# XunshanMan/Object-oriented-SLAM

Measured on AMD Instinct MI355X. Metric: LM iterations/sec (cams+ellipsoids), higher is better.
Workload: dtype f64

## Files before the change

### include/esl.h

```cpp
#ifndef ESL_H_
#define ESL_H_

#include <stdint.h>

#ifdef __cplusplus
extern "C" {
#endif

#define ESL_ABI_VERSION 5
#define ESL_MAX_TRACE 32

typedef enum {
  ESL_OK = 0,
  ESL_ERR_NO_DEVICE = 1,
  ESL_ERR_INVALID = 2,
  ESL_ERR_HIP = 3,
  ESL_ERR_STATE = 4,
  ESL_ERR_ALLOC = 5
} esl_status;

typedef struct esl_ctx esl_ctx;

typedef struct {
  double fx, fy, cx, cy;
  int32_t n_cams;
  int32_t n_objs;
  const uint8_t* cam_fixed;

  int32_t n_bbox;
  const int32_t* bbox_cam;
  const int32_t* bbox_obj;
  const double* bbox_meas;
  const double* bbox_weight;

  int32_t n_e3d;
  const int32_t* e3d_cam;
  const int32_t* e3d_obj;
  const double* e3d_meas;
  const double* e3d_weight;

  int32_t n_grav;
  const int32_t* grav_obj;
  double grav_normal[4];
  double grav_weight;

  int32_t n_odom;
  const int32_t* odom_i;
  const int32_t* odom_j;
  const double* odom_meas;
  const double* odom_info;

  int32_t check_visibility;
  int32_t image_rows, image_cols;
} esl_graph;

typedef enum {
  ESL_JAC_NUMERIC = 0,
  ESL_JAC_ANALYTIC = 1
} esl_jacobian_mode;

typedef enum {
  ESL_SOLVER_AUTO = 0,
  ESL_SOLVER_REDUCED_CAMERA = 1,
  ESL_SOLVER_REDUCED_ELLIPSOID = 2,
  ESL_SOLVER_CAMERA_CHAIN = 3,
  ESL_SOLVER_PCG = 4
} esl_linear_solver;

typedef enum {
  ESL_BBOX_REPROJECTION = 0,
  ESL_BBOX_TANGENCY = 1
} esl_bbox_residual;

typedef struct {
  int32_t max_iters;
  int32_t max_trials;
  double tau;
  int32_t jacobian_mode;
  double numeric_delta;
  int32_t linear_solver;
  int32_t drop_nan_bbox;
  int32_t bbox_residual;
  int32_t e3d_half_turn;
} esl_lm_params;

typedef struct {
  int32_t iterations;
  int32_t total_trials;
  int32_t n_bbox_valid;
  int32_t n_bbox_dropped;
  int32_t stop_reason;
  double chi2_initial;
  double chi2_final;
  double lambda_final;
  int32_t trace_len;
  double trace_chi2[ESL_MAX_TRACE];
  double trace_lambda[ESL_MAX_TRACE];
  int32_t trace_trials[ESL_MAX_TRACE];
} esl_lm_report;

typedef struct {
  double chi2;
  double max_diag;
  double scale;
  int32_t solve_ok;
  int32_t pad;
} esl_lm_partials;

int esl_abi_version(void);
const char* esl_last_error(void);
int esl_device_count(void);
int esl_ctx_create(int device_id, esl_ctx** out);
int esl_ctx_destroy(esl_ctx* ctx);
int esl_ctx_synchronize(esl_ctx* ctx);
int esl_ctx_trim(esl_ctx* ctx);
void esl_lm_params_default(esl_lm_params* p);

typedef enum { ESL_ROBUST_NONE = 0, ESL_ROBUST_HUBER = 1, ESL_ROBUST_PSEUDO_HUBER = 2, ESL_ROBUST_CAUCHY = 3, ESL_ROBUST_TUKEY = 4 } esl_robust_kind;
typedef enum { ESL_EDGE_BBOX = 0, ESL_EDGE_E3D = 1, ESL_EDGE_GRAVITY = 2, ESL_EDGE_ODOM = 3, ESL_EDGE_CLASSES = 4 } esl_edge_class;
typedef struct {
  int32_t kind[ESL_EDGE_CLASSES];
  double delta[ESL_EDGE_CLASSES];
} esl_robust_params;
int esl_lm_set_robust(esl_ctx* ctx, const esl_robust_params* p);
typedef struct {
  int32_t max_iters;
  int32_t check_every;
  double rel_tol;
} esl_pcg_params;
void esl_pcg_params_default(esl_pcg_params* p);
int esl_lm_set_pcg(esl_ctx* ctx, const esl_pcg_params* p);
#define ESL_PCG_STATS 8
int esl_lm_pcg_stats(esl_ctx* ctx, double stats[ESL_PCG_STATS]);

int esl_edge_chi2(esl_ctx* ctx, int32_t edge_class, double* chi2, double* weight, int64_t count);

int esl_optimize(esl_ctx* ctx, const esl_graph* g, double* cams_io ,
                 double* objs_io , const esl_lm_params* p, esl_lm_report* out);

int esl_graph_upload(esl_ctx* ctx, const esl_graph* g);
int esl_graph_upload_fixed(esl_ctx* ctx, const esl_graph* g, const uint8_t* obj_fixed);
int esl_optimize_fixed(esl_ctx* ctx, const esl_graph* g, const uint8_t* obj_fixed, double* cams_io, double* objs_io,
                       const esl_lm_params* p, esl_lm_report* out);
int esl_graph_obj_fixed(esl_ctx* ctx, uint8_t* flags_out, int32_t count);
int esl_states_upload(esl_ctx* ctx, const double* cams, const double* objs);
int esl_states_download(esl_ctx* ctx, double* cams, double* objs);
int esl_optimize_resident(esl_ctx* ctx, const esl_lm_params* p, esl_lm_report* out);
int esl_states_snapshot(esl_ctx* ctx);
int esl_states_restore(esl_ctx* ctx);

typedef struct {
  int32_t n_new_cams; const double* new_cams;
  int32_t n_new_objs; const double* new_objs;
  int32_t n_bbox; const int32_t* bbox_cam; const int32_t* bbox_obj; const double* bbox_meas; const double* bbox_weight;
  int32_t n_e3d; const int32_t* e3d_cam; const int32_t* e3d_obj; const double* e3d_meas; const double* e3d_weight;
  int32_t n_grav; const int32_t* grav_obj;
  const uint8_t* new_cam_fixed;
  int32_t n_odom; const int32_t* odom_i; const int32_t* odom_j;
  const double* odom_meas;
  const double* odom_info;
} esl_graph_delta;
int esl_graph_append(esl_ctx* ctx, const esl_graph_delta* d);
int esl_graph_sizes(esl_ctx* ctx, int32_t* n_cams, int32_t* n_objs, int32_t* n_bbox, int32_t* n_e3d, int32_t* relayouts);

#define ESL_PROF_KINDS 10
int esl_profile_enable(esl_ctx* ctx, int enable);
int esl_profile_get(esl_ctx* ctx, int64_t count[ESL_PROF_KINDS], double total_ms[ESL_PROF_KINDS]);

int esl_lm_begin(esl_ctx* ctx, const esl_lm_params* p, int32_t* n_valid, int32_t* n_dropped);
int esl_lm_linearize(esl_ctx* ctx, esl_lm_partials* out);
int esl_lm_reduced_system(esl_ctx* ctx, double lambda, void** dev_ptr, int64_t* n, int64_t* lda);
int esl_lm_reduced_residual(esl_ctx* ctx, double* rel_residual_out);
int esl_lm_try_step(esl_ctx* ctx, double lambda, esl_lm_partials* out);
int esl_lm_commit(esl_ctx* ctx, int accept);
int esl_lm_solver_used(esl_ctx* ctx, int32_t* solver_out);
#define ESL_SOLVER_STATS 10
int esl_lm_solver_stats(esl_ctx* ctx, double stats[ESL_SOLVER_STATS]);

int esl_lm_download(esl_ctx* ctx, int32_t which, double* dst, int64_t count);

int esl_comm_unique_id(char out[128]);
int esl_comm_init(esl_ctx* ctx, int32_t n_ranks, int32_t rank, const char id[128]);
typedef int (*esl_host_allreduce_fn)(void* user, double* host_buf, int64_t count);
int esl_comm_init_host(esl_ctx* ctx, int32_t n_ranks, int32_t rank, esl_host_allreduce_fn fn, void* user);
int esl_comm_set_replicated(esl_ctx* ctx, int replicated);
int esl_comm_destroy(esl_ctx* ctx);

int esl_partition_objects(const esl_graph* g, int32_t n_parts, int32_t* part_of_obj);

typedef struct {
  int32_t stride;
  double depth_scale;
  double depth_min, depth_max;
  double voxel_leaf;
  double plane_dist;
  double cluster_tolerance;
  int32_t min_cluster_size;
  double center_dis;
  int32_t symmetry_open;
  double symmetry_grid;
  double symmetry_sigma;
  int32_t symmetry_lm_iters;
} esl_fit_params;

void esl_fit_params_default(esl_fit_params* p);

int esl_fit_frame(esl_ctx* ctx, const uint16_t* depth, int32_t width, int32_t height,
                  const double* bboxes , const int32_t* labels , int32_t n_boxes,
                  const double Twc[7], const double intr[5] ,
                  const double ground[4], const esl_fit_params* p,
                  double* ellipsoids_out , double* prob_out ,
                  int32_t* status_out );

int esl_fit_frame_debug(esl_ctx* ctx, const uint16_t* depth, int32_t width, int32_t height, const double* bboxes,
                        const int32_t* labels, int32_t n_boxes, const double Twc[7], const double intr[5],
                        const double ground[4], const esl_fit_params* p, double* ellipsoids_out, double* prob_out,
                        int32_t* status_out, double* debug_out);

typedef struct {
  int32_t result;
  int32_t symmetry_type;
  double plane[4];
  double plane2[4];
  double prob;
  double center[3];
} esl_fit_symmetry;

int esl_fit_frame_ex(esl_ctx* ctx, const uint16_t* depth, int32_t width, int32_t height, const double* bboxes,
                     const int32_t* labels, int32_t n_boxes, const double Twc[7], const double intr[5],
                     const double ground[4], const esl_fit_params* p, double* ellipsoids_out, double* prob_out,
                     int32_t* status_out, esl_fit_symmetry* symmetry_out, double* debug_out);

typedef struct esl_plane_params {
  int32_t min_size;
  double angle_threshold_deg;
  double distance_threshold;
  int32_t normal_smoothing;
  double max_depth_change_factor;
  int32_t min_inliers;
  int32_t refine;
  double refine_distance;
  double max_curvature;
} esl_plane_params;
void esl_plane_params_default(esl_plane_params* p);
int esl_extract_ground_plane(esl_ctx* ctx, const uint16_t* depth, int32_t width, int32_t height, const double intr[5],
                             const esl_plane_params* p, double plane_out[4], int32_t* ok, int32_t* n_planes, int32_t* n_pixels);

int esl_extract_planes(esl_ctx* ctx, const uint16_t* depth, int32_t width, int32_t height, const double intr[5],
                       const esl_plane_params* p, int32_t max_planes, double* planes_out, int32_t* sizes_out,
                       int32_t* n_planes, int32_t* labels_out);

int esl_init_quadric(esl_ctx* ctx, const double* poses_Twc , const double* bboxes ,
                     int32_t n, const double K[4], int32_t rows, int32_t cols, int32_t faithful,
                     double ellipsoid_out[10], double qstar_out[16], int32_t* ok);

int esl_init_from_qstar(esl_ctx* ctx, const double qstar[16], int32_t faithful, double ellipsoid_out[10], int32_t* ok);
int esl_init_plane_error(esl_ctx* ctx, const double* poses_Twc , const double* bboxes , int32_t n,
                         const double K[4], int32_t rows, int32_t cols, const double ellipsoid[10], double* error_out);

int esl_init_quadrics(esl_ctx* ctx,
                      const double* cams , int32_t F,
                      int32_t N ,
                      const int32_t* obs_cam , const int32_t* obs_obj ,
                      const double* obs_boxes , int64_t n_obs,
                      const double K[4], int32_t rows, int32_t cols, int32_t faithful, int32_t min_observations,
                      double* ellipsoids_out , double* qstar_out ,
                      double* plane_error_out , int32_t* stats_out );

typedef struct {
  int32_t sample_size;
  int32_t n_hypotheses;
  double  inlier_px;
  int32_t min_inliers;
  int32_t refine;
  uint64_t seed;
} esl_init_robust_params;
void esl_init_robust_params_default(esl_init_robust_params* p);

int esl_init_quadrics_robust(esl_ctx* ctx, const double* cams , int32_t F, int32_t N,
                             const int32_t* obs_cam, const int32_t* obs_obj, const double* obs_boxes, int64_t n_obs,
                             const double K[4], int32_t rows, int32_t cols, int32_t faithful, int32_t min_observations,
                             const esl_init_robust_params* p ,
                             double* ellipsoids_out , double* qstar_out , double* plane_error_out ,
                             int32_t* stats_out , int32_t* inlier_out , double* residual_out ,
                             double* hyp_out );

typedef struct {
  double center_tol;
  double height_tol;
  double size_ratio;
  double min_baseline;
  int32_t min_inliers;
  int32_t max_candidates;
  int32_t match_labels;
  int32_t refine;
} esl_reloc_params;
void esl_reloc_params_default(esl_reloc_params* p);

int esl_reloc_set_map(esl_ctx* ctx, const double* objs, const int32_t* labels, int32_t M, const double ground_world[4]);

typedef struct {
  int32_t status;
  int32_t n_candidates;
  int64_t n_hypotheses;
  int64_t best_key;
  int32_t n_inliers;
  int32_t refined;
  double cost;
  double yaw, tx, ty;
  double Twc[7];
} esl_reloc_result;

int esl_relocalize(esl_ctx* ctx, const double* det_objs , const int32_t* det_labels, int32_t D,
                   const double ground_cam[4], const esl_reloc_params* p ,
                   esl_reloc_result* out, int32_t* assoc_out );

typedef struct {
  double min_iou;
  double occl_ratio;
  double min_box_px;
  int32_t match_labels;
  int32_t occlusion;
} esl_assoc_params;
void esl_assoc_params_default(esl_assoc_params* p);

int esl_predict_boxes(esl_ctx* ctx, const double Tcw[7], const double* objs ,
                      int32_t M, const double K[4], int32_t rows, int32_t cols, const esl_assoc_params* p ,
                      double* boxes_out , double* depth_out , int32_t* flags_out );

int esl_associate_boxes(esl_ctx* ctx, const double* cams , int32_t F,
// ... 104 lines not shown
```

### object-oriented-slam_amd/abi.py

```python
import ctypes as C

import numpy as np

ESL_MAX_TRACE = 32

c_double_p = C.POINTER(C.c_double)
c_int32_p = C.POINTER(C.c_int32)
c_uint8_p = C.POINTER(C.c_uint8)


class EslGraph(C.Structure):
    _fields_ = [
        ("fx", C.c_double), ("fy", C.c_double), ("cx", C.c_double), ("cy", C.c_double),
        ("n_cams", C.c_int32), ("n_objs", C.c_int32),
        ("cam_fixed", c_uint8_p),
        ("n_bbox", C.c_int32), ("bbox_cam", c_int32_p), ("bbox_obj", c_int32_p),
        ("bbox_meas", c_double_p), ("bbox_weight", c_double_p),
        ("n_e3d", C.c_int32), ("e3d_cam", c_int32_p), ("e3d_obj", c_int32_p),
        ("e3d_meas", c_double_p), ("e3d_weight", c_double_p),
        ("n_grav", C.c_int32), ("grav_obj", c_int32_p),
        ("grav_normal", C.c_double * 4), ("grav_weight", C.c_double),
        ("n_odom", C.c_int32), ("odom_i", c_int32_p), ("odom_j", c_int32_p),
        ("odom_meas", c_double_p), ("odom_info", c_double_p),
        ("check_visibility", C.c_int32), ("image_rows", C.c_int32), ("image_cols", C.c_int32),
    ]


class EslGraphDelta(C.Structure):
    _fields_ = [
        ("n_new_cams", C.c_int32), ("new_cams", c_double_p), ("n_new_objs", C.c_int32), ("new_objs", c_double_p),
        ("n_bbox", C.c_int32), ("bbox_cam", c_int32_p), ("bbox_obj", c_int32_p), ("bbox_meas", c_double_p), ("bbox_weight", c_double_p),
        ("n_e3d", C.c_int32), ("e3d_cam", c_int32_p), ("e3d_obj", c_int32_p), ("e3d_meas", c_double_p), ("e3d_weight", c_double_p),
        ("n_grav", C.c_int32), ("grav_obj", c_int32_p),
        ("new_cam_fixed", C.POINTER(C.c_uint8)), ("n_odom", C.c_int32), ("odom_i", c_int32_p), ("odom_j", c_int32_p),
        ("odom_meas", c_double_p), ("odom_info", c_double_p),
    ]


class EslLmParams(C.Structure):
    _fields_ = [
        ("max_iters", C.c_int32), ("max_trials", C.c_int32), ("tau", C.c_double),
        ("jacobian_mode", C.c_int32), ("numeric_delta", C.c_double),
        ("linear_solver", C.c_int32), ("drop_nan_bbox", C.c_int32), ("bbox_residual", C.c_int32), ("e3d_half_turn", C.c_int32),
    ]


class EslLmReport(C.Structure):
    _fields_ = [
        ("iterations", C.c_int32), ("total_trials", C.c_int32),
        ("n_bbox_valid", C.c_int32), ("n_bbox_dropped", C.c_int32), ("stop_reason", C.c_int32),
        ("chi2_initial", C.c_double), ("chi2_final", C.c_double), ("lambda_final", C.c_double),
        ("trace_len", C.c_int32),
        ("trace_chi2", C.c_double * ESL_MAX_TRACE), ("trace_lambda", C.c_double * ESL_MAX_TRACE),
        ("trace_trials", C.c_int32 * ESL_MAX_TRACE),
    ]

    def as_dict(self):
        n = self.trace_len
        return dict(iterations=self.iterations, total_trials=self.total_trials,
                    n_bbox_valid=self.n_bbox_valid, n_bbox_dropped=self.n_bbox_dropped,
                    stop_reason=self.stop_reason, chi2_initial=self.chi2_initial,
                    chi2_final=self.chi2_final, lambda_final=self.lambda_final,
                    trace_chi2=list(self.trace_chi2[:n]), trace_lambda=list(self.trace_lambda[:n]),
                    trace_trials=list(self.trace_trials[:n]))


class EslLmPartials(C.Structure):
    _fields_ = [("chi2", C.c_double), ("max_diag", C.c_double), ("scale", C.c_double),
                ("solve_ok", C.c_int32), ("pad", C.c_int32)]


class EslFitParams(C.Structure):
    _fields_ = [
        ("stride", C.c_int32), ("depth_scale", C.c_double), ("depth_min", C.c_double),
        ("depth_max", C.c_double), ("voxel_leaf", C.c_double), ("plane_dist", C.c_double),
        ("cluster_tolerance", C.c_double), ("min_cluster_size", C.c_int32), ("center_dis", C.c_double),
        ("symmetry_open", C.c_int32), ("symmetry_grid", C.c_double), ("symmetry_sigma", C.c_double),
        ("symmetry_lm_iters", C.c_int32),
    ]


class EslFitSymmetry(C.Structure):
    _fields_ = [("result", C.c_int32), ("symmetry_type", C.c_int32), ("plane", C.c_double * 4),
                ("plane2", C.c_double * 4), ("prob", C.c_double), ("center", C.c_double * 3)]


class EslPlaneParams(C.Structure):
    _fields_ = [("min_size", C.c_int32), ("angle_threshold_deg", C.c_double), ("distance_threshold", C.c_double),
                ("normal_smoothing", C.c_int32), ("max_depth_change_factor", C.c_double), ("min_inliers", C.c_int32),
                ("refine", C.c_int32), ("refine_distance", C.c_double), ("max_curvature", C.c_double)]


def default_plane_params(**kw):
    p = EslPlaneParams(min_size=200, angle_threshold_deg=5.0, distance_threshold=0.1, normal_smoothing=10,
                       max_depth_change_factor=0.05, min_inliers=100, refine=1, refine_distance=0.02, max_curvature=0.001)
    for k, v in kw.items():
        if not hasattr(p, k):
            raise AttributeError(k)
        setattr(p, k, v)
    return p


SOLVER_AUTO, SOLVER_REDUCED_CAMERA, SOLVER_REDUCED_ELLIPSOID, SOLVER_CAMERA_CHAIN, SOLVER_PCG = 0, 1, 2, 3, 4


class EslPcgParams(C.Structure):
    _fields_ = [("max_iters", C.c_int32), ("check_every", C.c_int32), ("rel_tol", C.c_double)]


def default_pcg_params():
    return EslPcgParams(max_iters=1000, check_every=8, rel_tol=1e-10)


class EslRelocParams(C.Structure):
    _fields_ = [("center_tol", C.c_double), ("height_tol", C.c_double), ("size_ratio", C.c_double), ("min_baseline", C.c_double),
                ("min_inliers", C.c_int32), ("max_candidates", C.c_int32), ("match_labels", C.c_int32), ("refine", C.c_int32)]


class EslRelocResult(C.Structure):
    _fields_ = [("status", C.c_int32), ("n_candidates", C.c_int32), ("n_hypotheses", C.c_int64), ("best_key", C.c_int64),
                ("n_inliers", C.c_int32), ("refined", C.c_int32), ("cost", C.c_double), ("yaw", C.c_double), ("tx", C.c_double),
                ("ty", C.c_double), ("Twc", C.c_double * 7)]

    def as_dict(self):
        return dict(status=self.status, n_candidates=self.n_candidates, n_hypotheses=self.n_hypotheses, best_key=self.best_key,
                    n_inliers=self.n_inliers, refined=self.refined, cost=self.cost, yaw=self.yaw, tx=self.tx, ty=self.ty,
                    Twc=np.array(list(self.Twc)))


def default_reloc_params(**kw):
    p = EslRelocParams(center_tol=0.25, height_tol=0.25, size_ratio=1.5, min_baseline=0.5, min_inliers=3, max_candidates=4096,
                       match_labels=1, refine=1)
    for k, v in kw.items():
        if not hasattr(p, k):
            raise AttributeError(k)
        setattr(p, k, v)
    return p


class EslAssocParams(C.Structure):
    _fields_ = [("min_iou", C.c_double), ("occl_ratio", C.c_double), ("min_box_px", C.c_double), ("match_labels", C.c_int32),
                ("occlusion", C.c_int32)]


def default_assoc_params(**kw):
    p = EslAssocParams(min_iou=0.3, occl_ratio=0.7, min_box_px=10.0, match_labels=1, occlusion=1)
    for k, v in kw.items():
        if not hasattr(p, k):
            raise AttributeError(k)
        setattr(p, k, v)
    return p


class EslInitRobustParams(C.Structure):
    _fields_ = [("sample_size", C.c_int32), ("n_hypotheses", C.c_int32), ("inlier_px", C.c_double), ("min_inliers", C.c_int32),
                ("refine", C.c_int32), ("seed", C.c_uint64)]

# ... 222 lines not shown
```

### object-oriented-slam_amd/csrc/esl_capi.hip

```cpp
#include <algorithm>
#include <cfloat>
#include <cmath>
#include <cstdio>
#include <cstdlib>
#include <cstring>
#include <numeric>

#include "esl_graph_int.hpp"
#include "esl_graph_layout.hpp"
#include "esl_kernels_map.hpp"
#include "esl_kernels_chunk.hpp"
#include "esl_slam.hpp"
#include "esl_fixed.hpp"

namespace esl {
static thread_local std::string g_err;
void set_error(const std::string& s) { g_err = s; }
}

using namespace esl;

namespace esl {
ProfScope::ProfScope(esl_ctx* ctx, int kind) : c(ctx), slot(-1) {
  if (!c || !c->prof_on) return;
  if (c->prof_level < 2 && (kind != 0 || !c->prof_gate)) return;
  if (c->prof_used + 2 > c->prof_ev.size()) {
    if (c->prof_ev.size() >= 16384) { prof_drain(c); }
    else {
      for (int i = 0; i < 512; ++i) { hipEvent_t e; if (hipEventCreate(&e) != hipSuccess) return; c->prof_ev.push_back(e); }
      c->prof_kind.resize(c->prof_ev.size() / 2);
    }
  }
  slot = (int)c->prof_used;
  c->prof_kind[slot / 2] = kind;
  c->prof_used += 2;
  (void)hipEventRecord(c->prof_ev[slot], c->stream);
}
ProfScope::~ProfScope() {
  if (slot >= 0) (void)hipEventRecord(c->prof_ev[slot + 1], c->stream);
}
int prof_drain(esl_ctx* c) {
  if (hipStreamSynchronize(c->stream) != hipSuccess) return ESL_ERR_HIP;
  for (size_t s = 0; s + 1 < c->prof_used; s += 2) {
    float ms = 0;
    if (hipEventElapsedTime(&ms, c->prof_ev[s], c->prof_ev[s + 1]) == hipSuccess) {
      const int k = c->prof_kind[s / 2];
      c->prof_count[k]++;
      c->prof_ms[k] += ms;
    }
  }
  c->prof_used = 0;
  return ESL_OK;
}
}

struct WorkStage {
  struct Fix { void** dst; size_t off; };
  size_t total = 0;
  std::vector<Fix> fixes;
  template <class T>
  void add(T** dst, size_t n) {
    const size_t off = layout::align_up(total, 256);
    total = off + std::max<size_t>(n, 1) * sizeof(T);
    fixes.push_back({(void**)dst, off});
  }
  int commit(esl_ctx* c) {
    int rc = arena_reserve(&c->arena_work, &c->arena_work_cap, std::max<size_t>(total, 256));
    if (rc) return rc;
    for (const Fix& f : fixes) *f.dst = c->arena_work + f.off;
    return ESL_OK;
  }
};
int esl::work_buffers(esl_ctx* c, size_t cap_objs, size_t cap_cams, size_t cap_chunks) {
  WorkStage wk;
  wk.add(&c->chunk_out, cap_chunks * kChunkOut); wk.add(&c->chunk_out2, cap_chunks * kChunkOut);
  wk.add(&c->chunk_chi, cap_chunks);
  wk.add(&c->blk_part, ((cap_objs + kStepWaves - 1) / kStepWaves + 2) * 2);
  wk.add(&c->solve_part, ((cap_objs + kStepWaves - 1) / kStepWaves + (cap_objs + 63) / 64 + 2) * 4 * 2);
  wk.add(&c->blk_chi, cap_chunks + 2);
  wk.add(&c->cams, cap_cams * 7); wk.add(&c->cams_trial, cap_cams * 7);
  wk.add(&c->objs, cap_objs * 10); wk.add(&c->objs_trial, cap_objs * 10);
  wk.add(&c->Hoo, cap_objs * 45); wk.add(&c->bo, cap_objs * 9); wk.add(&c->xo, cap_objs * 9); wk.add(&c->obj_part, cap_objs * 4);
  int rc = wk.commit(c);
  if (rc) return rc;
  ESL_HIP_TRY(hipMemsetAsync(c->obj_part, 0, std::max<size_t>(cap_objs, 1) * 4 * sizeof(double), c->stream));
  return ESL_OK;
}

extern "C" {

int esl_abi_version(void) { return ESL_ABI_VERSION; }
const char* esl_last_error(void) { return g_err.c_str(); }

int esl_device_count(void) {
  int n = 0;
  if (hipGetDeviceCount(&n) != hipSuccess) return 0;
  return n;
}

void esl_lm_params_default(esl_lm_params* p) {
  p->max_iters = 10;
  p->max_trials = 10;
  p->tau = 1e-5;
  p->jacobian_mode = ESL_JAC_NUMERIC;
  p->numeric_delta = 1e-9;
  p->linear_solver = ESL_SOLVER_AUTO;
  p->drop_nan_bbox = 1;
  p->bbox_residual = ESL_BBOX_REPROJECTION;
  p->e3d_half_turn = 0;
}

int esl_ctx_create(int device_id, esl_ctx** out) {
  if (!out) return ESL_ERR_INVALID;
  *out = nullptr;
  int n = 0;
  if (hipGetDeviceCount(&n) != hipSuccess || n <= 0) {
    set_error("no HIP device visible: libesl_hip has no CPU fallback");
    return ESL_ERR_NO_DEVICE;
  }
  if (device_id < 0 || device_id >= n) { set_error("device id out of range"); return ESL_ERR_INVALID; }
  ESL_HIP_TRY(hipSetDevice(device_id));
  esl_ctx* c = new esl_ctx();
  c->device = device_id;
  { const char* ov = std::getenv("ESL_CF_OVERLAP"); c->sw_cf_overlap = (ov && ov[0] >= '0' && ov[0] <= '4') ? ov[0] - '0' : 4; }
  { const char* ok = std::getenv("ESL_CF_OS_KERNEL"); c->sw_cf_os_kernel = (ok && ok[0] == '0') ? 0 : 1; }
  { const char* sd = std::getenv("ESL_CF_STRIDE"); const int v = sd ? std::atoi(sd) : 0; c->sw_cf_stride = (v == 16 || v == 32 || v == 48) ? v : 0; }
  auto init = [&]() -> int {
    ESL_HIP_TRY(hipStreamCreateWithFlags(&c->stream, hipStreamNonBlocking));
    ESL_HIP_TRY(hipHostMalloc((void**)&c->host_part, 16 * sizeof(double), hipHostMallocDefault));
    ESL_HIP_TRY(hipMalloc((void**)&c->dev_part, 16 * sizeof(double)));
    ESL_HIP_TRY(hipMalloc((void**)&c->chol_info, 4 * sizeof(int)));
    ESL_HIP_TRY(hipMemset(c->chol_info, 0, 4 * sizeof(int)));
    ESL_HIP_TRY(hipMalloc((void**)&c->tickets, 4 * sizeof(unsigned int)));
    ESL_HIP_TRY(hipMemset(c->tickets, 0, 4 * sizeof(unsigned int)));
    ESL_HIP_TRY(hipMalloc((void**)&c->dev_scal, 8 * sizeof(double)));
    ESL_HIP_TRY(hipEventCreateWithFlags(&c->ev_try, hipEventDisableTiming));
    ESL_HIP_TRY(hipHostMalloc(&c->host_scal, sizeof(LmScalars), hipHostMallocMapped));
    ESL_HIP_TRY(hipHostGetDevicePointer(&c->host_scal_dev, c->host_scal, 0));
    std::memset(c->host_scal, 0, sizeof(LmScalars));
    ESL_HIP_TRY(hipMalloc(&c->lm_dev, 2 * sizeof(LmCore)));
    ESL_HIP_TRY(hipMemset(c->lm_dev, 0, 2 * sizeof(LmCore)));
    ESL_HIP_TRY(hipHostMalloc(&c->lm_host, sizeof(LmHostView), hipHostMallocMapped));
    ESL_HIP_TRY(hipHostGetDevicePointer(&c->lm_host_dev, c->lm_host, 0));
    std::memset(c->lm_host, 0, sizeof(LmHostView));
    return ESL_OK;
  };
  const int rc = init();
  if (rc) { const std::string msg = g_err; esl_ctx_destroy(c); set_error(msg); return rc; }
  *out = c;
  return ESL_OK;
}

int esl_ctx_destroy(esl_ctx* c) {
  if (!c) return ESL_OK;
  (void)hipSetDevice(c->device);
  if (c->stream) (void)hipStreamSynchronize(c->stream);
  slam_sync_side(c);
  free_graph(c);
  slam_release(c);
  if (c->arena_graph) (void)hipFree(c->arena_graph);
  if (c->arena_work) (void)hipFree(c->arena_work);
  if (c->stage_host) (void)hipHostFree(c->stage_host);
  if (c->append_dev) (void)hipFree(c->append_dev);
  if (c->slam_tab_dev) (void)hipFree(c->slam_tab_dev);
  c->eq_buf.release();
  if (c->fx_blob) (void)hipFree(c->fx_blob);
  c->chain_ws.release();
  fit_release(c);
  plane_release(c);
  reloc_release(c);
  assoc_release(c);
  merge_release(c);
  render_release(c);
  dense_release(c);
  init_batch_release(c);
  for (hipEvent_t e : c->prof_ev) (void)hipEventDestroy(e);
  if (c->host_part) (void)hipHostFree(c->host_part);
  dev_free(&c->dev_part);
  dev_free(&c->chol_info);
  dev_free(&c->tickets); dev_free(&c->dev_scal);
  if (c->host_scal) (void)hipHostFree(c->host_scal);
  if (c->lm_host) (void)hipHostFree(c->lm_host);
  if (c->lm_dev) (void)hipFree(c->lm_dev);
  if (c->ev_try) (void)hipEventDestroy(c->ev_try);
  esl_comm_destroy(c);
  slam_release_runtime(c);
  if (c->stream) (void)hipStreamDestroy(c->stream);
  delete c;
  return ESL_OK;
}

int esl_ctx_trim(esl_ctx* c) {
  if (!c) return ESL_ERR_INVALID;
  ESL_HIP_TRY(hipSetDevice(c->device));
  ESL_HIP_TRY(hipStreamSynchronize(c->stream));
  slam_trim(c, c->graph_loaded && c->g.n_free_cams > 0);
  return ESL_OK;
}

int esl_debug_scratch_allocs(esl_ctx* c, int32_t owner, int64_t* allocs_out, int64_t* bytes_out) {
  if (!c || !allocs_out || !bytes_out || owner < ESL_SCRATCH_RELOC || owner > ESL_SCRATCH_INIT_ROBUST) {
    set_error("esl_debug_scratch_allocs: null pointer or unknown owner");
    return ESL_ERR_INVALID;
  }
  *allocs_out = 0; *bytes_out = 0;
  switch (owner) {
    case ESL_SCRATCH_RELOC: reloc_scratch_stats(c, allocs_out, bytes_out); break;
    case ESL_SCRATCH_ASSOC: assoc_scratch_stats(c, allocs_out, bytes_out); break;
    case ESL_SCRATCH_MERGE: merge_scratch_stats(c, allocs_out, bytes_out); break;
    case ESL_SCRATCH_RENDER: render_scratch_stats(c, allocs_out, bytes_out); break;
    default: init_scratch_stats(c, owner == ESL_SCRATCH_INIT_ROBUST, allocs_out, bytes_out);
  }
  return ESL_OK;
}

int esl_ctx_synchronize(esl_ctx* c) {
  if (!c) return ESL_ERR_INVALID;
  ESL_HIP_TRY(hipStreamSynchronize(c->stream));
  return ESL_OK;
}

static ChunkTable chunk_table(const esl_ctx* c) {
  ChunkTable t;
  t.n_chunks = c->n_chunks; t.obj = c->ck_obj; t.type = c->ck_type; t.begin = c->ck_begin; t.end = c->ck_end; t.ostart = c->ck_ostart;
  return t;
}
static int map_launch_linearize(esl_ctx* c, bool finalize, const double* src_objs = nullptr, double* dst_chunk = nullptr,
                                const LmCore* st = nullptr, bool validate = false) {
  const DevGraph& g = c->g;
  if (!src_objs) src_objs = c->objs;
  if (!dst_chunk) dst_chunk = c->chunk_out;
  const double* objs_b = st ? c->objs_trial : nullptr;
  double* chunk_b = st ? c->chunk_out2 : nullptr;
  if (st) { src_objs = c->objs; dst_chunk = c->chunk_out; }
  const ChunkTable ct = chunk_table(c);
  const bool an = c->lm.p.jacobian_mode == ESL_JAC_ANALYTIC;
  const int nb_e3 = (c->n_ids_e3 + 2 * kLinWaves - 1) / (2 * kLinWaves);
  const int nb_bb = (c->n_ids_bb + kLinWaves - 1) / kLinWaves;
  robust_dispatch(c->robust_on, [&](auto robust) {
    constexpr bool R = decltype(robust)::value;
    if (ct.n_chunks > 0) {
      ProfScope ps(c, 0);
      const dim3 block(64 * kLinWaves);
      int* cnt = c->chol_info + 2;
      if (an && g.bbox_mode) {
        if (validate && g.check_vis)
          hipLaunchKernelGGL((k_chunk_linearize_both<ESL_JAC_ANALYTIC, 2, true, R>), dim3(nb_e3 + nb_bb), block, 0, c->stream, g, ct, c->ck_ids_e3,
                             c->n_ids_e3, nb_e3, c->ck_ids_bb, c->n_ids_bb, c->cams, src_objs, objs_b, c->lm.p.numeric_delta, dst_chunk,
                             chunk_b, c->blk_chi, st, cnt);
        else if (validate)
          hipLaunchKernelGGL((k_chunk_linearize_both<ESL_JAC_ANALYTIC, 1, true, R>), dim3(nb_e3 + nb_bb), block, 0, c->stream, g, ct, c->ck_ids_e3,
                             c->n_ids_e3, nb_e3, c->ck_ids_bb, c->n_ids_bb, c->cams, src_objs, objs_b, c->lm.p.numeric_delta, dst_chunk,
                             chunk_b, c->blk_chi, st, cnt);
        else
          hipLaunchKernelGGL((k_chunk_linearize_both<ESL_JAC_ANALYTIC, 0, true, R>), dim3(nb_e3 + nb_bb), block, 0, c->stream, g, ct, c->ck_ids_e3,
                             c->n_ids_e3, nb_e3, c->ck_ids_bb, c->n_ids_bb, c->cams, src_objs, objs_b, c->lm.p.numeric_delta, dst_chunk,
                             chunk_b, c->blk_chi, st, cnt);
      } else if (an) {
        if (validate && g.check_vis)
          hipLaunchKernelGGL((k_chunk_linearize_both<ESL_JAC_ANALYTIC, 2, false, R>), dim3(nb_e3 + nb_bb), block, 0, c->stream, g, ct, c->ck_ids_e3,
                             c->n_ids_e3, nb_e3, c->ck_ids_bb, c->n_ids_bb, c->cams, src_objs, objs_b, c->lm.p.numeric_delta, dst_chunk,
                             chunk_b, c->blk_chi, st, cnt);
        else if (validate)
          hipLaunchKernelGGL((k_chunk_linearize_both<ESL_JAC_ANALYTIC, 1, false, R>), dim3(nb_e3 + nb_bb), block, 0, c->stream, g, ct, c->ck_ids_e3,
                             c->n_ids_e3, nb_e3, c->ck_ids_bb, c->n_ids_bb, c->cams, src_objs, objs_b, c->lm.p.numeric_delta, dst_chunk,
                             chunk_b, c->blk_chi, st, cnt);
        else
          hipLaunchKernelGGL((k_chunk_linearize_both<ESL_JAC_ANALYTIC, 0, false, R>), dim3(nb_e3 + nb_bb), block, 0, c->stream, g, ct, c->ck_ids_e3,
                             c->n_ids_e3, nb_e3, c->ck_ids_bb, c->n_ids_bb, c->cams, src_objs, objs_b, c->lm.p.numeric_delta, dst_chunk,
                             chunk_b, c->blk_chi, st, cnt);
      } else {
        if (nb_e3 > 0)
          hipLaunchKernelGGL((k_chunk_linearize<ESL_JAC_NUMERIC, 1, 0, false, R>), dim3(nb_e3), block, 0, c->stream, g, ct, c->ck_ids_e3,
                             c->n_ids_e3, c->cams, src_objs, objs_b, c->lm.p.numeric_delta, dst_chunk, chunk_b, c->blk_chi, 0, st, cnt);
        if (nb_bb > 0) {
          auto launch_bb = [&](auto kern) {
            hipLaunchKernelGGL(kern, dim3(nb_bb), block, 0, c->stream, g, ct, c->ck_ids_bb, c->n_ids_bb, c->cams, src_objs, objs_b,
                               c->lm.p.numeric_delta, dst_chunk, chunk_b, c->blk_chi, nb_e3, st, cnt);
// ... 642 lines not shown
```

### object-oriented-slam_amd/csrc/esl_cf.hpp

```cpp
#pragma once
#include "esl_cf_plan.hpp"
#include "esl_kernels_map.hpp"

namespace esl {

__device__ __forceinline__ double cf_readlane(double v, int src) {
  const int lo = __builtin_amdgcn_readlane(__double2loint(v), src), hi = __builtin_amdgcn_readlane(__double2hiint(v), src);
  return __hiloint2double(hi, lo);
}

static __global__ __launch_bounds__(256) void k_cf_gather_B(int nf, const double* __restrict__ Aod, const int* __restrict__ od_start,
                                                            const int* __restrict__ od_edge, double* __restrict__ B) {
  const long t = (long)blockIdx.x * 256 + threadIdx.x;
  const long i = t / 36;
  if (i >= nf) return;
  const int e = (int)(t - i * 36), r = e / 6, c = e - 6 * r;
  double s = 0;
  if (i + 1 < nf)
    for (int q = od_start[i]; q < od_start[i + 1]; ++q) {
      const int es = od_edge[q];
      const double* Hij = Aod + (size_t)(es >> 1) * 90 + 54;
      s += (es & 1) ? Hij[c * 6 + r] : Hij[r * 6 + c];
    }
  B[t] = s;
// ... 45 lines not shown
          double v = sH[ii * 36 + r * 6 + c] + ((r == c) ? lambda : 0.0);
#pragma unroll
          for (int k = 0; k < 6; ++k) v -= g[k * 6 + r] * g[k * 6 + c];
          d[CF_LT(r, c)] = v;
        }
#pragma unroll
      for (int k = 0; k < 36; ++k) b[k] = sB[ii * 36 + k];
      double is[6];
#pragma unroll
      for (int j = 0; j < 6; ++j) {
        const double p = d[CF_LT(j, j)];
        ok = ok && (p > 0);
        double q = __builtin_amdgcn_rsq(p);
        q = q * (1.5 - 0.5 * p * q * q);
        q = q * (1.5 - 0.5 * p * q * q);
        is[j] = q;
        d[CF_LT(j, j)] = p * q;
#pragma unroll
        for (int r = j + 1; r < 6; ++r) d[CF_LT(r, j)] *= q;
#pragma unroll
        for (int r = j + 1; r < 6; ++r)
#pragma unroll
          for (int c = j + 1; c <= r; ++c) d[CF_LT(r, c)] -= d[CF_LT(r, j)] * d[CF_LT(c, j)];
      }
#pragma unroll
      for (int c = 0; c < 6; ++c)
#pragma unroll
        for (int r = 0; r < 6; ++r) {
          double v = b[c * 6 + r];
#pragma unroll
          for (int k = 0; k < r; ++k) v -= d[CF_LT(r, k)] * g[k * 6 + c];
          g[r * 6 + c] = v * is[r];
        }
      if (lane == 0) {
#pragma unroll
        for (int k = 0; k < 21; ++k) sL[ii * 21 + k] = d[k];
#pragma unroll
        for (int k = 0; k < 36; ++k) sG[ii * 36 + k] = g[k];
      }
    }
    __builtin_amdgcn_wave_barrier();
    if (more) lstore();
    for (int idx = lane; idx < len * 21; idx += 64) Lfac[(size_t)i0 * 21 + idx] = sL[idx];
    for (int idx = lane; idx < len * 36; idx += 64) Gfac[(size_t)i0 * 36 + idx] = sG[idx];
    __builtin_amdgcn_wave_barrier();
  }
  if (!ok && lane == 0) atomicOr(info, 1);
}

static __global__ __launch_bounds__(64) void k_cf_factor_blocks(int nf, const double* __restrict__ Lfac, const double* __restrict__ Gfac,
                                                                double* __restrict__ Linv, double* __restrict__ Mm, double* __restrict__ Nn,
                                                                int stride, double* __restrict__ scat = nullptr, int scat_stride = 0) {
  const int i = blockIdx.x * 64 + threadIdx.x;
  if (i >= nf) return;
  const int pos = stride > 0 ? i % stride : i;
  if (stride > 0 && pos == stride - 1) return;
  const bool first = pos == 0, last = (i == nf - 1) || (stride > 0 && pos == stride - 2);
  double L[21], Li[36];
#pragma unroll
  for (int k = 0; k < 21; ++k) L[k] = Lfac[(size_t)i * 21 + k];
#pragma unroll
  for (int c = 0; c < 6; ++c)
#pragma unroll
    for (int r = 0; r < 6; ++r) {
      if (r < c) { Li[r * 6 + c] = 0; continue; }
      double v = (r == c) ? 1.0 : 0.0;
#pragma unroll
      for (int k = c; k < r; ++k) v -= L[CF_LT(r, k)] * Li[k * 6 + c];
      Li[r * 6 + c] = v / L[CF_LT(r, r)];
    }
#pragma unroll
  for (int k = 0; k < 36; ++k) Linv[(size_t)i * 36 + k] = Li[k];
  if (scat) {
#pragma unroll
    for (int k = 0; k < 36; ++k) scat[(size_t)(i * scat_stride + scat_stride - 1) * 36 + k] = Li[k];
  }
  double Lo[36];
#pragma unroll
  for (int r = 0; r < 6; ++r)
#pragma unroll
    for (int c = 0; c < 6; ++c) Lo[r * 6 + c] = first ? 0.0 : Gfac[(size_t)(i - 1) * 36 + c * 6 + r];
#pragma unroll
  for (int r = 0; r < 6; ++r)
#pragma unroll
    for (int c = 0; c < 6; ++c) {
      double m = 0;
#pragma unroll
      for (int k = 0; k <= r; ++k) m += Li[r * 6 + k] * Lo[k * 6 + c];
      Mm[(size_t)i * 36 + r * 6 + c] = m;
    }
#pragma unroll
  for (int r = 0; r < 6; ++r)
#pragma unroll
    for (int c = 0; c < 6; ++c) {
      double nv = 0;
#pragma unroll
      for (int k = r; k < 6; ++k) nv += Li[k * 6 + r] * Gfac[(size_t)i * 36 + k * 6 + c];
      Nn[(size_t)i * 36 + r * 6 + c] = last ? 0.0 : nv;
    }
}
#undef CF_LT

__device__ __forceinline__ void cf_edge_scale_one(const DevGraph& g, int n_list, const int* __restrict__ oe_u, const int* __restrict__ oe_slot,
                                                  const double* __restrict__ W, const double* __restrict__ Linv,
                                                  const double* __restrict__ bc, double* __restrict__ V,
                                                  double* __restrict__ vy, long t, int cls = 0, int stride = 0) {
  const long EU = (long)g.n_bbox + g.n_e3d;
  if (t < (long)n_list * 9) {
    const long k = t / 9;
    const int b = (int)(t - k * 9);
    const int slot = oe_slot[k];
    if (cls != 0 && (slot % stride == stride - 1) != (cls == 2)) return;
    const long u = oe_u[k];
    const bool valid = !(u < g.n_bbox) || g.bb_valid[u];
    double w[6];
#pragma unroll
    for (int q = 0; q < 6; ++q) w[q] = valid ? W[(long)(q * 9 + b) * EU + u] : 0.0;
    const double* Li = Linv + (size_t)slot * 36;
#pragma unroll
    for (int a = 0; a < 6; ++a) {
      double s = 0;
#pragma unroll
      for (int q = 0; q <= a; ++q) s += Li[a * 6 + q] * w[q];
      V[t * 6 + a] = s;
    }
  } else {
    const long s = t - (long)n_list * 9;
    if (s >= g.n_free_cams) return;
    if (cls != 0 && (s % stride == stride - 1) != (cls == 2)) return;
    const double* Li = Linv + (size_t)s * 36;
    double w[6];
#pragma unroll
    for (int q = 0; q < 6; ++q) w[q] = bc[(size_t)s * 6 + q];
#pragma unroll
    for (int a = 0; a < 6; ++a) {
      double v = 0;
#pragma unroll
      for (int q = 0; q <= a; ++q) v += Li[a * 6 + q] * w[q];
      vy[(size_t)s * 6 + a] = v;
    }
  }
}
static __global__ __launch_bounds__(256) void k_cf_edge_scale(DevGraph g, int n_list, const int* __restrict__ oe_u, const int* __restrict__ oe_slot,
                                                              const double* __restrict__ W, const double* __restrict__ Linv,
                                                              const double* __restrict__ bc, double* __restrict__ V,
                                                              double* __restrict__ vy, int cls, int stride) {
  cf_edge_scale_one(g, n_list, oe_u, oe_slot, W, Linv, bc, V, vy, (long)blockIdx.x * 256 + threadIdx.x, cls, stride);
}

struct CfSegs {
  const int* fwork; const int* seg_start; const int* seg_obj; const long long* xoff; const int* xld;
  const int* rank; const int* unrank;
};
template <int MODE>
static __global__ __launch_bounds__(64) void k_cf_forward(int nf_all, int n_o, int n_chunks, const int* __restrict__ oe_cst ,
                                                          const int* __restrict__ oe_slot, const double* __restrict__ V,
                                                          const double* __restrict__ vy, const double* __restrict__ Mm,
                                                          double* __restrict__ Xt, long ldx, int stride, int seglen,
                                                          const double* __restrict__ Zt, double* __restrict__ R, int sep_stride, CfSegs sg) {
  constexpr bool SEP = MODE == 1;
  __shared__ double sM[kCfFwdCh * 36];
  __shared__ double sZ[kCfFwdCh * 36];
  constexpr int CH = MODE == 2 ? kCfFwdCh / 2 : kCfFwdCh;
  __shared__ double sv[CH * 6 * 64];
  __shared__ double svy[kCfFwdCh * 6];
  const int lane = threadIdx.x;
  const int seg = SEP ? 0 : (MODE == 2 ? sg.fwork[2 * blockIdx.x] : (int)blockIdx.y);
  const int j = (MODE == 2 ? sg.fwork[2 * blockIdx.x + 1] : (int)blockIdx.x) * 64 + lane;
  const int ob = MODE == 2 ? sg.seg_start[seg] : 0;
  const int jr = MODE == 2 ? 9 * (sg.seg_start[seg + 1] - ob) : n_o;
  const bool on = j <= jr, rhs = j == jr, col = on && !rhs;
  const int oi = col ? j / 9 : 0, b = j - 9 * oi;
  const int o = (MODE == 2 && col) ? sg.seg_obj[ob + oi] : oi;
  const long tcol = MODE == 2 ? (rhs ? (long)n_o : 9L * (sg.rank ? sg.rank[o] : o) + b) : (long)j;
  const int beg = SEP ? 0 : seg * stride;
  const int nf = SEP ? nf_all : ((beg + seglen < nf_all) ? beg + seglen : nf_all);
  if (beg >= nf) return;
  const bool use_z = !SEP && Zt != nullptr && seg >= 1;
  const int* cst = oe_cst + (size_t)o * (n_chunks + 1);
  double x[6] = {0, 0, 0, 0, 0, 0}, acc[6] = {0, 0, 0, 0, 0, 0};
  for (int i0 = beg; i0 < nf; i0 += kCfFwdCh) {
    const int ch = i0 / kCfFwdCh;
    const int len = (nf - i0 < kCfFwdCh) ? nf - i0 : kCfFwdCh;
    {
      double tm[kCfFwdCh * 36 / 64], tz[kCfFwdCh * 36 / 64], ty[2];
#pragma unroll
      for (int q = 0; q < kCfFwdCh * 36 / 64; ++q) {
        const int idx = q * 64 + lane, cl = idx < len * 36 ? idx : 0;
        tm[q] = Mm[(size_t)i0 * 36 + cl];
        tz[q] = use_z ? Zt[(size_t)i0 * 36 + cl] : 0.0;
      }
#pragma unroll
      for (int q = 0; q < 2; ++q) { const int idx = q * 64 + lane; ty[q] = SEP ? 0.0 : vy[(size_t)i0 * 6 + (idx < len * 6 ? idx : 0)]; }
#pragma unroll
      for (int q = 0; q < kCfFwdCh * 36 / 64; ++q) { sM[q * 64 + lane] = tm[q]; sZ[q * 64 + lane] = tz[q]; }
#pragma unroll
      for (int q = 0; q < 2; ++q) if (q * 64 + lane < kCfFwdCh * 6) svy[q * 64 + lane] = ty[q];
    }
    for (int h0 = 0; h0 < (MODE == 2 ? len : 1); h0 += CH) {
      const int hl = MODE == 2 ? ((len - h0 < CH) ? len - h0 : CH) : len;
      if (SEP) {
        const size_t jc = on ? (size_t)j : 0;
        {
          constexpr int kQ = kCfFwdCh * 6;
          double t[kQ];
#pragma unroll
          for (int q = 0; q < kQ; ++q) t[q] = R[jc + (size_t)(6 * i0 + (q < len * 6 ? q : 0)) * (size_t)ldx];
#pragma unroll
          for (int q = 0; q < kQ; ++q) sv[q * 64 + lane] = (on && q < len * 6) ? t[q] : 0.0;
        }
        __builtin_amdgcn_wave_barrier();
      } else {
#pragma unroll
        for (int q = 0; q < CH * 6; ++q) sv[q * 64 + lane] = 0.0;
        __builtin_amdgcn_wave_barrier();
        if (rhs) {
#pragma unroll
          for (int q = 0; q < CH * 6; ++q) sv[q * 64 + lane] = (q < hl * 6) ? svy[h0 * 6 + q] : 0.0;
        } else if (col) {
          const int ka = cst[ch], kb = cst[ch + 1];
          for (int k = ka; k < kb; k += 4) {
            int sl[4];
            double rec[4][6];
#pragma unroll
            for (int e = 0; e < 4; ++e) {
              const int kk = (k + e < kb) ? k + e : ka;
              sl[e] = oe_slot[kk];
              const double* src = V + ((size_t)kk * 9 + b) * 6;
#pragma unroll
              for (int a = 0; a < 6; ++a) rec[e][a] = src[a];
            }
#pragma unroll
            for (int e = 0; e < 4; ++e)
              if (k + e < kb && sl[e] - i0 >= h0 && sl[e] - i0 - h0 < hl) {
#pragma unroll
                for (int a = 0; a < 6; ++a) sv[((sl[e] - i0 - h0) * 6 + a) * 64 + lane] += rec[e][a];
              }
          }
        }
        __builtin_amdgcn_wave_barrier();
      }
      for (int ii = 0; ii < hl; ++ii) {
        const double* M = sM + (h0 + ii) * 36;
        double xn[6];
#pragma unroll
        for (int a = 0; a < 6; ++a) {
          double t = sv[(ii * 6 + a) * 64 + lane];
#pragma unroll
          for (int q = 0; q < 6; ++q) t -= M[a * 6 + q] * x[q];
          xn[a] = t;
        }
#pragma unroll
        for (int a = 0; a < 6; ++a) { x[a] = xn[a]; sv[(ii * 6 + a) * 64 + lane] = xn[a]; }
        if (use_z) {
          const double* Z = sZ + (h0 + ii) * 36;
#pragma unroll
          for (int a = 0; a < 6; ++a)
#pragma unroll
            for (int q = 0; q < 6; ++q) acc[a] += Z[q * 6 + a] * xn[q];
        }
      }
      if (on) {
#pragma unroll
        for (int q0 = 0; q0 < CH * 6; q0 += 8) {
          double t[8];
#pragma unroll
          for (int e = 0; e < 8; ++e) t[e] = sv[((q0 + e < hl * 6) ? q0 + e : 0) * 64 + lane];
#pragma unroll
          for (int e = 0; e < 8; ++e)
            if (q0 + e < hl * 6) {
              const int q = q0 + e;
              if (MODE == 2) {
                Xt[(size_t)sg.xoff[seg] + (size_t)(6 * (i0 - beg + h0) + q) * (size_t)sg.xld[seg] + (size_t)j] = t[e];
              } else {
                const size_t row = (SEP && sep_stride > 0) ? (size_t)(6 * ((i0 + q / 6) * sep_stride + sep_stride - 1) + q % 6) : (size_t)(6 * i0 + q);
                Xt[(size_t)j + row * (size_t)ldx] = t[e];
              }
            }
        }
      }
      __builtin_amdgcn_wave_barrier();
    }
  }
  if (use_z && on) {
#pragma unroll
    for (int a = 0; a < 6; ++a) R[(size_t)tcol + (size_t)(6 * (seg - 1) + a) * (size_t)ldx] = acc[a];
  }
}

static __global__ __launch_bounds__(64) void k_cf_zt(int nf, int stride, const double* __restrict__ Linv, const double* __restrict__ Mm,
                                                     const double* __restrict__ B, double* __restrict__ Zt) {
  __shared__ double sM[kCfMaxStride * 36];
  const int p = blockIdx.x + 1, lane = threadIdx.x;
  const int beg = p * stride, end = (beg + stride - 1 < nf) ? beg + stride - 1 : nf;
  if (beg >= end) return;
  const int len = end - beg;
  {
    constexpr int kQ = kCfMaxStride * 36 / 64;
    double t[kQ];
#pragma unroll
    for (int q = 0; q < kQ; ++q) { const int idx = q * 64 + lane; t[q] = Mm[(size_t)beg * 36 + (idx < len * 36 ? idx : 0)]; }
#pragma unroll
    for (int q = 0; q < kQ; ++q) sM[q * 64 + lane] = t[q];
  }
  __builtin_amdgcn_wave_barrier();
  const int c = lane < 6 ? lane : 5;
  double z[6];
  {
    const double* Li = Linv + (size_t)beg * 36;
    const double* Bs = B + (size_t)(beg - 1) * 36;
#pragma unroll
    for (int r = 0; r < 6; ++r) {
      double v = 0;
#pragma unroll
      for (int k = 0; k <= r; ++k) v += Li[r * 6 + k] * Bs[k * 6 + c];
      z[r] = v;
// ... 403 lines not shown
  const double* X = Xc + xoff[p];
  const int cc = c < m ? c : 0;
  double s = 0;
#pragma unroll 6
  for (int row = 0; row < 6 * (kCfFwdCh - 1); ++row) s += X[(long)row * ld + cc] * X[(long)row * ld + m];
  if (c < m) Prhs[roff[p] + c] = s;
}

static __global__ __launch_bounds__(256) void k_cf_T_gather(int N, int nw, const unsigned long long* __restrict__ mask, const int* __restrict__ cmap,
                                                            const long long* __restrict__ boff, const long long* __restrict__ roff,
                                                            const double* __restrict__ P, const double* __restrict__ Prhs,
                                                            const double* __restrict__ Hoo, const double* __restrict__ bo, double lambda,
                                                            double* __restrict__ T, long ldt, int o2_begin, int o2_end, const int* __restrict__ unrank,
                                                            int accumulate = 0) {
  const int lane = threadIdx.x & 63, wave = __builtin_amdgcn_readfirstlane(threadIdx.x >> 6);
  const int t1 = blockIdx.x;
  const int o1 = (t1 == N || !unrank) ? t1 : unrank[t1];
  const int N1 = N + 1;
  const long n_o = 9L * N;
  const bool rhs = o1 == N;
  for (int q = wave; q < kCfTPer; q += 4) {
    const int t2 = o2_begin + (int)blockIdx.y * kCfTPer + q;
    if (t2 >= o2_end || t2 > t1 || t2 >= N) continue;
    const int o2 = unrank ? unrank[t2] : t2;
    double s0 = 0, s1 = 0;
    const int eT0 = (lane % 9) * 9 + lane / 9, eT1 = lane < 17 ? ((64 + lane) % 9) * 9 + (64 + lane) / 9 : 0;
    for (int wd = 0; wd < nw; ++wd) {
      unsigned long long mk = mask[(size_t)o1 * nw + wd] & mask[(size_t)o2 * nw + wd];
      if (!mk) continue;
      const int pl = wd * 64 + lane;
      long long offl = 0;
      int swl = 0;
      if ((mk >> lane) & 1ull) {
        const long long i2 = cmap[(size_t)pl * N1 + o2] & 0xFFFFFF;
        if (rhs) offl = roff[pl] + 9 * i2;
        else {
          const long long i1 = cmap[(size_t)pl * N1 + o1] & 0xFFFFFF;
          swl = i2 > i1;
          offl = (boff[pl] + (swl ? i2 * (i2 + 1) / 2 + i1 : i1 * (i1 + 1) / 2 + i2)) * 81;
        }
      }
      while (mk) {
        long long off[4];
        bool have[4], sw[4];
#pragma unroll
        for (int u = 0; u < 4; ++u) {
          have[u] = mk != 0;
          const int bit = have[u] ? __builtin_ctzll(mk) : 0;
          if (have[u]) mk &= mk - 1;
          off[u] = ((long long)__builtin_amdgcn_readlane((int)(offl >> 32), bit) << 32) | (unsigned)__builtin_amdgcn_readlane((int)offl, bit);
          sw[u] = __builtin_amdgcn_readlane(swl, bit) != 0;
        }
        double v0[4], v1[4];
#pragma unroll
        for (int u = 0; u < 4; ++u) {
          const double* src = (rhs ? Prhs : P) + off[u];
          v0[u] = (have[u] && (!rhs || lane < 9)) ? src[sw[u] ? eT0 : lane] : 0.0;
          v1[u] = (have[u] && !rhs && lane < 17) ? src[sw[u] ? eT1 : 64 + lane] : 0.0;
        }
#pragma unroll
        for (int u = 0; u < 4; ++u) { s0 += v0[u]; s1 += v1[u]; }
      }
    }
    if (rhs) {
      if (lane < 9) { double* tp = &T[n_o + (9L * t2 + lane) * ldt]; const double v = bo[(size_t)o2 * 9 + lane] - s0; *tp = accumulate ? v + *tp : v; }
    } else {
#pragma unroll
      for (int h = 0; h < 2; ++h) {
        const int e = h * 64 + lane;
        if (e >= 81) continue;
        const int j = e / 9, i = e - 9 * j;
        if (o1 == o2 && i < j) continue;
        double base = 0;
        if (o1 == o2) base = Hoo[(size_t)o1 * 45 + j * 9 - (j * (j - 1)) / 2 + (i - j)] + ((i == j) ? lambda : 0.0);
        double* tp = &T[(9L * t1 + i) + (9L * t2 + j) * ldt];
        const double v = base - (h ? s1 : s0);
        *tp = accumulate ? v + *tp : v;
      }
    }
  }
}

template <int M>
static __global__ __launch_bounds__(64) void k_cf_seg_back(int nf_all, const int* __restrict__ fwork, const int* __restrict__ seg_start,
                                                           const long long* __restrict__ xoff, const int* __restrict__ xld,
                                                           const double* __restrict__ Xc, const double* __restrict__ Linv,
                                                           const double* __restrict__ Gfac, double* __restrict__ Y, double* __restrict__ Yr) {
  constexpr int SI = M * kCfFwdCh - 1;
  constexpr int CL = M == 1 ? SI : kCfFwdCh;
  __shared__ double sLi[SI * 36], sG[SI * 36];
  const int lane = threadIdx.x;
  const int p = fwork[2 * blockIdx.x], j = fwork[2 * blockIdx.x + 1] * 64 + lane;
  const int ob = seg_start[p], m = 9 * (seg_start[p + 1] - ob);
  const int beg = p * (M * kCfFwdCh);
  const int len = (beg + SI < nf_all ? beg + SI : nf_all) - beg;
  if (len <= 0) return;
  {
    constexpr int kQ = (SI * 36 + 63) / 64;
    double tl[kQ], tg[kQ];
#pragma unroll
    for (int q = 0; q < kQ; ++q) {
      const int idx = q * 64 + lane, cl = idx < len * 36 ? idx : 0;
      tl[q] = Linv[(size_t)beg * 36 + cl]; tg[q] = Gfac[(size_t)beg * 36 + cl];
    }
#pragma unroll
    for (int q = 0; q < kQ; ++q) if (q * 64 + lane < SI * 36) { sLi[q * 64 + lane] = tl[q]; sG[q * 64 + lane] = tg[q]; }
  }
  const bool on = j <= m, rhs = j == m;
  const size_t ld = (size_t)xld[p];
  const double* X = Xc + (size_t)xoff[p] + (on ? j : 0);
  const int oi = rhs ? 0 : (on ? j / 9 : 0), b = on ? j - 9 * oi : 0;
  double* dst = rhs ? Yr + (size_t)beg * 6 : Y + ((size_t)(ob + oi) * SI) * 54 + b * 6;
  const int dstep = rhs ? 6 : 54;
  double z[6] = {0, 0, 0, 0, 0, 0};
#pragma unroll
  for (int c = M - 1; c >= 0; --c) {
    const int s0 = c * kCfFwdCh;
    if (s0 >= len && c < M - 1) continue;
    double x[CL * 6];
#pragma unroll
    for (int q = 0; q < CL * 6; ++q) x[q] = X[(size_t)(s0 * 6 + q < len * 6 ? s0 * 6 + q : 0) * ld];
    if (c == M - 1) __builtin_amdgcn_wave_barrier();
#pragma unroll
    for (int ii = CL - 1; ii >= 0; --ii) {
      if (s0 + ii >= len) continue;
      double y[6];
#pragma unroll
      for (int a = 0; a < 6; ++a) {
        double t = x[ii * 6 + a];
#pragma unroll
        for (int q = 0; q < 6; ++q) t -= sG[(s0 + ii) * 36 + a * 6 + q] * z[q];
        y[a] = t;
      }
#pragma unroll
      for (int a = 0; a < 6; ++a) {
        double t = 0;
#pragma unroll
        for (int q = a; q < 6; ++q) t += sLi[(s0 + ii) * 36 + q * 6 + a] * y[q];
        z[a] = t;
      }
      if (on) {
#pragma unroll
        for (int a = 0; a < 6; ++a) dst[(size_t)(s0 + ii) * dstep + a] = y[a];
      }
    }
  }
}

template <bool FILL>
static __global__ __launch_bounds__(256) void k_cf_os_list(int N, int nw, int n_chunks, int seg_chunks, const unsigned long long* __restrict__ mask,
                                                           const int* __restrict__ cmap, const int* __restrict__ seg_start,
                                                           const int* __restrict__ oe_cst, const int* __restrict__ oe_slot,
                                                           const int* __restrict__ unrank, const long long* __restrict__ bstart,
                                                           int* __restrict__ bcnt, int2* __restrict__ pairs, int offsets) {
  const int lane = threadIdx.x & 63, wave = __builtin_amdgcn_readfirstlane(threadIdx.x >> 6);
  const int t1 = blockIdx.x;
  const int o1 = (t1 == N || !unrank) ? t1 : unrank[t1];
  const int N1 = N + 1;
  const bool rhs = o1 == N;
  const int m54 = offsets ? 54 : 1, m6 = offsets ? 6 : 1;
  const int stride = seg_chunks * kCfFwdCh;
  for (int q = wave; q < kCfTPer; q += 4) {
    const int t2 = (int)blockIdx.y * kCfTPer + q;
    if (t2 > t1 || t2 >= N) continue;
    const int o2 = unrank ? unrank[t2] : t2;
    const long b = rhs ? (long)N * (N + 1) / 2 + t2 : (long)t1 * (t1 + 1) / 2 + t2;
    const int* cst = oe_cst + (size_t)(rhs ? o2 : o1) * (n_chunks + 1);
    const long long w0 = FILL ? bstart[b] : 0;
    int cnt = 0;
    for (int wd = 0; wd < nw; ++wd) {
      unsigned long long mk = mask[(size_t)o1 * nw + wd] & mask[(size_t)o2 * nw + wd];
      if (!mk) continue;
      const int pl = wd * 64 + lane;
      const bool mine = (mk >> lane) & 1ull;
      const int che = seg_chunks * (pl + 1) < n_chunks ? seg_chunks * (pl + 1) : n_chunks;
      const int kal = mine ? cst[seg_chunks * pl] : 0, kbl = mine ? cst[che] : 0;
      const int yrl = (mine && !rhs) ? (seg_start[pl] + (cmap[(size_t)pl * N1 + o2] & 0xFFFFFF)) * (stride - 1) : 0;
      while (mk) {
        const int bit = __builtin_ctzll(mk);
        mk &= mk - 1;
        const int p = wd * 64 + bit;
        const int ka = __builtin_amdgcn_readlane(kal, bit), kb = __builtin_amdgcn_readlane(kbl, bit), yr = __builtin_amdgcn_readlane(yrl, bit);
        for (int k0 = ka; k0 < kb; k0 += 64) {
          const int ent = k0 + lane;
          const int pos = ent < kb ? oe_slot[ent] - p * stride : stride - 1;
          const bool valid = pos != stride - 1;
          const unsigned long long vb = __ballot(valid);
          if (FILL && valid) {
            const int at = cnt + __builtin_popcountll(vb & ((1ull << lane) - 1ull));
            pairs[w0 + at] = rhs ? make_int2((p * stride + pos) * m6, ent * m54) : make_int2(ent * m54, (yr + pos) * m54);
          }
          cnt += __builtin_popcountll(vb);
        }
      }
    }
    if (!FILL && lane == 0) bcnt[b] = cnt;
  }
}

constexpr int kCfOsBatch = 12;
static __global__ __launch_bounds__(256) void k_cf_T_onesided(int N, const int2* __restrict__ pairs, const long long* __restrict__ bstart,
                                                              const int* __restrict__ bcnt, const double* __restrict__ V,
                                                              const double* __restrict__ Y, const double* __restrict__ Yr,
                                                              const double* __restrict__ Hoo, const double* __restrict__ bo, double lambda,
                                                              double* __restrict__ T, long ldt, int o2_begin, int o2_end,
                                                              const int* __restrict__ unrank, int accumulate) {
  const int lane = threadIdx.x & 63, wave = __builtin_amdgcn_readfirstlane(threadIdx.x >> 6);
  const int t1 = blockIdx.x;
  const int o1 = (t1 == N || !unrank) ? t1 : unrank[t1];
  const int r = lane & 15, kq = lane >> 4;
  const long n_o = 9L * N;
  const bool rhs = o1 == N;
  const double* Asrc = rhs ? Yr : V;
  const double* Bsrc = rhs ? V : Y;
  const int astep = rhs ? 6 : 54, aoff = rhs ? 0 : r * 6;
  const bool alane = rhs ? r == 0 : r < 9, blane = r < 9;
  constexpr int kPerWave = kCfTPer / 4;
  long long stl = 0;
  int cnl = 0;
  {
    const int t2l = o2_begin + (int)blockIdx.y * kCfTPer + wave + 4 * (lane < kPerWave ? lane : 0);
    if (lane < kPerWave && t2l < o2_end && t2l <= t1 && t2l < N) {
      const long bl = rhs ? (long)N * (N + 1) / 2 + t2l : (long)t1 * (t1 + 1) / 2 + t2l;
      stl = bstart[bl]; cnl = bcnt[bl];
    }
  }
  auto first_pairs = [&](int u, int& px, int& py) {
    px = 0; py = 0;
    if (u >= kPerWave) return;
    const long long st = ((long long)__builtin_amdgcn_readlane((int)(stl >> 32), u) << 32) | (unsigned)__builtin_amdgcn_readlane((int)stl, u);
    if (lane < __builtin_amdgcn_readlane(cnl, u)) { const int2 pr = pairs[st + lane]; px = pr.x; py = pr.y; }
  };
  int nx = 0, ny = 0;
  first_pairs(0, nx, ny);
#pragma unroll
  for (int u = 0; u < kPerWave; ++u) {
    const int q = wave + 4 * u;
    const int t2 = o2_begin + (int)blockIdx.y * kCfTPer + q;
    const int px0 = nx, py0 = ny;
    first_pairs(u + 1, nx, ny);
    if (t2 >= o2_end || t2 > t1 || t2 >= N) continue;
    const int o2 = unrank ? unrank[t2] : t2;
    const long long start = ((long long)__builtin_amdgcn_readlane((int)(stl >> 32), u) << 32) | (unsigned)__builtin_amdgcn_readlane((int)stl, u);
    const int n = __builtin_amdgcn_readlane(cnl, u);
    cf_d4 acc = {0, 0, 0, 0};
    for (int c0 = 0; c0 < n; c0 += 64) {
      const int m = n - c0 < 64 ? n - c0 : 64;
      int px = px0, py = py0;
      if (c0 > 0) { px = 0; py = 0; if (lane < m) { const int2 pr = pairs[start + c0 + lane]; px = pr.x; py = pr.y; } }
      const int nst = (6 * m + 3) / 4;
      for (int s0 = 0; s0 < nst; s0 += kCfOsBatch) {
        double av[kCfOsBatch], bv[kCfOsBatch];
#pragma unroll
        for (int j = 0; j < kCfOsBatch; ++j) {
          const int s = s0 + j;
          const int e0 = (4 * s) / 6 < 63 ? (4 * s) / 6 : 63, e1 = (4 * s + 3) / 6 < 63 ? (4 * s + 3) / 6 : 63;
          const int x0 = __builtin_amdgcn_readlane(px, e0), x1 = __builtin_amdgcn_readlane(px, e1);
          const int y0 = __builtin_amdgcn_readlane(py, e0), y1 = __builtin_amdgcn_readlane(py, e1);
          const int kidx = 4 * s + kq;
          const bool hi = kidx >= 6 * e1 && e1 != e0;
          const int a = kidx - 6 * (hi ? e1 : e0);
          const bool ok = (hi ? e1 : e0) < m && kidx < 6 * m;
          const bool oka = ok && alane, okb = ok && blane;
          const size_t ia = oka ? (size_t)(hi ? x1 : x0) * astep + aoff + a : 0, ib = okb ? (size_t)(hi ? y1 : y0) * 54 + r * 6 + a : 0;
          const double va = Asrc[ia], vb = Bsrc[ib];
          av[j] = oka ? va : 0.0; bv[j] = okb ? vb : 0.0;
        }
#pragma unroll
        for (int j = 0; j < kCfOsBatch; ++j)
          if (s0 + j < nst) acc = __builtin_amdgcn_mfma_f64_16x16x4f64(av[j], bv[j], acc, 0, 0, 0);
      }
    }
    if (r < 9) {
#pragma unroll
      for (int g = 0; g < 4; ++g) {
        const int i = kq + 4 * g;
        if (rhs) {
          if (i == 0) { double* tp = &T[n_o + (9L * t2 + r) * ldt]; const double v = bo[(size_t)o2 * 9 + r] - acc[g]; *tp = accumulate ? v + *tp : v; }
        } else if (i < 9 && !(o1 == o2 && i < r)) {
          double base = 0;
          if (o1 == o2) base = Hoo[(size_t)o1 * 45 + r * 9 - (r * (r - 1)) / 2 + (i - r)] + ((i == r) ? lambda : 0.0);
          double* tp = &T[(9L * t1 + i) + (9L * t2 + r) * ldt];
          const double v = base - acc[g];
          *tp = accumulate ? v + *tp : v;
        }
      }
    }
  }
}

constexpr bool cf_og_ldk_ok(int ldk, int mod) {
  for (int i = 0; i < 20; ++i)
    for (int j = 0; j < i; ++j)
      if (((i / 2) * ldk + i % 2) % mod == ((j / 2) * ldk + j % 2) % mod) return false;
  return true;
}
constexpr bool cf_og_ldk_wr_ok(int ldk) {
  for (int g = 0; g < 4; ++g) {
    int cnt[16] = {};
    for (int l = 16 * g; l < 16 * g + 16 && l < 54; ++l)
      if (++cnt[((l / 6) * ldk + l % 6) % 16] > 2) return false;
  }
  return true;
}
constexpr int cf_og_ldk(int E) { int k = 6 * E + 1; while (!cf_og_ldk_ok(k, 32) || !cf_og_ldk_wr_ok(k)) k += 2; return k; }
#if defined(__HIP_DEVICE_COMPILE__)
typedef __attribute__((address_space(1))) double cf_gdouble;
#else
typedef double cf_gdouble;
#endif
constexpr int kCfOgBatch = 8;
static __global__ __launch_bounds__(256) __attribute__((amdgpu_waves_per_eu(4, 4))) void k_cf_T_onesided_lds(int N, const int2* __restrict__ pairs, const long long* __restrict__ bstart,
                                                                  const int* __restrict__ bcnt, const double* __restrict__ V,
                                                                  const double* __restrict__ Y, const double* __restrict__ Yr,
                                                                  const double* __restrict__ Hoo, const double* __restrict__ bo, double lambda,
                                                                  double* __restrict__ T, long ldt, int o2_begin, int o2_end,
                                                                  const int* __restrict__ unrank, int accumulate) {
  constexpr int E = kCfOgBatch, LDK = cf_og_ldk(E), NST = 6 * E / 4, IMG = 10 * LDK;
  static_assert(64 % E == 0 && (6 * E) % 4 == 0, "whole batches per 64 pairs, whole K-steps per batch");
  __shared__ double sImg[4 * 2 * IMG];
  const int lane = threadIdx.x & 63, wave = __builtin_amdgcn_readfirstlane(threadIdx.x >> 6);
  const int t1 = blockIdx.x;
  const int o1 = (t1 == N || !unrank) ? t1 : unrank[t1];
  const int r = lane & 15, kq = lane >> 4;
  const long n_o = 9L * N;
  const bool rhs = o1 == N;
  const double* Asrc = rhs ? Yr : V;
  const double* Bsrc = rhs ? V : Y;
  double* sA = sImg + wave * 2 * IMG;
  double* sB = sA + IMG;
  for (int i = lane; i < LDK; i += 64) { sA[9 * LDK + i] = 0.0; sB[9 * LDK + i] = 0.0; }
  const bool wa = lane < (rhs ? 6 : 54), wb = lane < 54;
  const unsigned la8 = wa ? 8u * lane : 0u, lb8 = wb ? 8u * lane : 0u;
  double* wA = sA + (lane / 6) * LDK + lane % 6;
  double* wB = sB + (lane / 6) * LDK + lane % 6;
  const double* rA = sA + (rhs ? (r == 0 ? 0 : 9) : (r < 9 ? r : 9)) * LDK + kq;
  const double* rB = sB + (r < 9 ? r : 9) * LDK + kq;
  constexpr int kPerWave = kCfTPer / 4;
  long long stl = 0;
  int cnl = 0;
  {
    const int t2l = o2_begin + (int)blockIdx.y * kCfTPer + wave + 4 * (lane < kPerWave ? lane : 0);
    if (lane < kPerWave && t2l < o2_end && t2l <= t1 && t2l < N) {
      const long bl = rhs ? (long)N * (N + 1) / 2 + t2l : (long)t1 * (t1 + 1) / 2 + t2l;
      stl = bstart[bl]; cnl = bcnt[bl];
    }
  }
  auto first_pairs = [&](int u, int& px, int& py) {
    px = 0; py = 0;
    if (u >= kPerWave) return;
    const long long st = ((long long)__builtin_amdgcn_readlane((int)(stl >> 32), u) << 32) | (unsigned)__builtin_amdgcn_readlane((int)stl, u);
    if (lane < __builtin_amdgcn_readlane(cnl, u)) { const int2 pr = pairs[st + lane]; px = pr.x; py = pr.y; }
  };
  double ga[E], gb[E];
  auto load = [&](const bool full, const int px, const int py, int e0, int m) __attribute__((always_inline)) {
#pragma unroll
    for (int e = 0; e < E; ++e)
      if (full || e < m) {
        const unsigned x = (unsigned)__builtin_amdgcn_readlane(px, e0 + e), y = (unsigned)__builtin_amdgcn_readlane(py, e0 + e);
        unsigned long long pa = (unsigned long long)(Asrc + x), pb = (unsigned long long)(Bsrc + y);
        unsigned oa = la8, ob = lb8;
#if defined(__HIP_DEVICE_COMPILE__)
        asm("" : "+s"(pa)); asm("" : "+s"(pb)); asm("" : "+v"(oa)); asm("" : "+v"(ob));
#endif
        ga[e] = *(const cf_gdouble*)(pa + oa);
        gb[e] = *(const cf_gdouble*)(pb + ob);
      }
  };
  int nx = 0, ny = 0;
  first_pairs(0, nx, ny);
#pragma unroll
  for (int u = 0; u < kPerWave; ++u) {
    const int q = wave + 4 * u;
    const int t2 = o2_begin + (int)blockIdx.y * kCfTPer + q;
    const int px0 = nx, py0 = ny;
    first_pairs(u + 1, nx, ny);
    if (t2 >= o2_end || t2 > t1 || t2 >= N) continue;
    const int o2 = unrank ? unrank[t2] : t2;
    const long long start = ((long long)__builtin_amdgcn_readlane((int)(stl >> 32), u) << 32) | (unsigned)__builtin_amdgcn_readlane((int)stl, u);
    const int n = __builtin_amdgcn_readlane(cnl, u);
    cf_d4 acc = {0, 0, 0, 0};
    for (int c0 = 0; c0 < n; c0 += 64) {
      const int m64 = n - c0 < 64 ? n - c0 : 64;
      int px = px0, py = py0;
      if (c0 > 0) { px = 0; py = 0; if (lane < m64) { const int2 pr = pairs[start + c0 + lane]; px = pr.x; py = pr.y; } }
      auto store = [&](const bool full, int m) __attribute__((always_inline)) {
        if (wa) {
#pragma unroll
          for (int e = 0; e < E; ++e)
            if (full || e < m) wA[6 * e] = ga[e];
          if (!full) wA[6 * m] = 0.0;
        }
        if (wb) {
#pragma unroll
          for (int e = 0; e < E; ++e)
            if (full || e < m) wB[6 * e] = gb[e];
          if (!full) wB[6 * m] = 0.0;
        }
      };
      auto steps = [&](const bool full, int m) __attribute__((always_inline)) {
        const int nst = (6 * m + 3) / 4;
        if (full) {
          double av[NST], bv[NST];
#pragma unroll
          for (int j = 0; j < NST; ++j) { av[j] = rA[4 * j]; bv[j] = rB[4 * j]; }
          __builtin_amdgcn_sched_barrier(0);
#pragma unroll
          for (int j = 0; j < NST; ++j) acc = __builtin_amdgcn_mfma_f64_16x16x4f64(av[j], bv[j], acc, 0, 0, 0);
        } else {
#pragma unroll
          for (int j = 0; j < NST; ++j)
            if (j < nst) acc = __builtin_amdgcn_mfma_f64_16x16x4f64(rA[4 * j], rB[4 * j], acc, 0, 0, 0);
        }
      };
      int mb = m64 < E ? m64 : E;
      if (mb == E) load(true, px, py, 0, E); else load(false, px, py, 0, mb);
      for (int e0 = 0; e0 < m64; e0 += E) {
        const int m = mb;
        __builtin_amdgcn_wave_barrier();
        if (m == E) store(true, E); else store(false, m);
        __builtin_amdgcn_fence(__ATOMIC_RELEASE, "wavefront");
        __builtin_amdgcn_wave_barrier();
        __builtin_amdgcn_fence(__ATOMIC_ACQUIRE, "wavefront");
        const int e1 = e0 + E;
        mb = m64 - e1 < E ? m64 - e1 : E;
        if (mb == E) load(true, px, py, e1, E); else if (mb > 0) load(false, px, py, e1, mb);
        if (m == E) steps(true, E); else steps(false, m);
      }
    }
    if (r < 9) {
#pragma unroll
      for (int g = 0; g < 4; ++g) {
        const int i = kq + 4 * g;
        if (rhs) {
          if (i == 0) { double* tp = &T[n_o + (9L * t2 + r) * ldt]; const double v = bo[(size_t)o2 * 9 + r] - acc[g]; *tp = accumulate ? v + *tp : v; }
        } else if (i < 9 && !(o1 == o2 && i < r)) {
          double base = 0;
          if (o1 == o2) base = Hoo[(size_t)o1 * 45 + r * 9 - (r * (r - 1)) / 2 + (i - r)] + ((i == r) ? lambda : 0.0);
          double* tp = &T[(9L * t1 + i) + (9L * t2 + r) * ldt];
          const double v = base - acc[g];
          *tp = accumulate ? v + *tp : v;
        }
      }
    }
  }
}

static __global__ __launch_bounds__(256) void k_cf_xo_unpermute(int N, const int* __restrict__ rank, const double* __restrict__ xo_t,
                                                                double* __restrict__ xo) {
  const int t = blockIdx.x * 256 + threadIdx.x;
  if (t >= 9 * N) return;
  const int o = t / 9, i = t - 9 * o;
  xo[t] = xo_t[9 * rank[o] + i];
}

static __global__ __launch_bounds__(256) void k_cf_make_cst(int N, int n_chunks, const int* __restrict__ oe_start, const int* __restrict__ oe_slot,
                                                            int* __restrict__ cst) {
  const long t = (long)blockIdx.x * 256 + threadIdx.x;
  if (t >= (long)N * (n_chunks + 1)) return;
  const int o = (int)(t / (n_chunks + 1)), chk = (int)(t - (long)o * (n_chunks + 1));
  int lo = oe_start[o], hi = oe_start[o + 1];
  const int want = chk * kCfFwdCh;
  while (lo < hi) { const int mid = (lo + hi) >> 1; if (oe_slot[mid] < want) lo = mid + 1; else hi = mid; }
  cst[t] = lo;
}
static __global__ __launch_bounds__(256) void k_cf_make_cmap(int n_inc, const int* __restrict__ inc , int N1, int nw,
                                                             const int* __restrict__ seg_start, int* __restrict__ cmap, unsigned long long* __restrict__ mask,
                                                             int* __restrict__ seg_obj, int* __restrict__ seg_first) {
  const int q = blockIdx.x * 256 + threadIdx.x;
  if (q >= n_inc) return;
  const int p = inc[q], o = inc[n_inc + q], f = inc[2 * n_inc + q], at = inc[3 * n_inc + q];
  cmap[(long)p * N1 + o] = (f << 24) | (at - seg_start[p]);
  seg_obj[at] = o; seg_first[at] = f;
  atomicOr(&mask[(long)o * nw + p / 64], 1ull << (p & 63));
}
static __global__ __launch_bounds__(64) void k_cf_make_work(int nseg, int N, int nw, const int* __restrict__ seg_start, const int* __restrict__ fw_off,
                                                            const long long* __restrict__ tw_off, int* __restrict__ cmap, unsigned long long* __restrict__ mask,
                                                            int* __restrict__ fwork, int* __restrict__ twork) {
  const int p = blockIdx.x;
  if (p >= nseg) return;
  const int cnt = seg_start[p + 1] - seg_start[p];
  if (threadIdx.x == 0) {
    cmap[(long)p * (N + 1) + N] = cnt;
    atomicOr(&mask[(long)N * nw + p / 64], 1ull << (p & 63));
  }
  const int nq = fw_off[p + 1] - fw_off[p];
  for (int q = threadIdx.x; q < nq; q += 64) { fwork[2 * (fw_off[p] + q)] = p; fwork[2 * (fw_off[p] + q) + 1] = q; }
  const int nt = (9 * cnt + kCfSyT - 1) / kCfSyT;
  const long long base = tw_off[p];
  for (int t = threadIdx.x; t < nt * (nt + 1) / 2; t += 64) {
    int ti = (int)((sqrt(8.0 * t + 1.0) - 1.0) * 0.5);
    while ((ti + 1) * (ti + 2) / 2 <= t) ++ti;
    while (ti * (ti + 1) / 2 > t) --ti;
    const int tj = t - ti * (ti + 1) / 2;
    twork[3 * (base + t)] = p; twork[3 * (base + t) + 1] = ti; twork[3 * (base + t) + 2] = tj;
  }
}
}
```

### object-oriented-slam_amd/csrc/esl_cf_plan.hpp

```cpp
#pragma once
#include <algorithm>
#include <array>
#include <cmath>
#include <cstddef>
#include <cstdint>
#include <vector>

namespace esl {

constexpr int kCfFwdCh = 16;
constexpr int kCfSyT = 128;
constexpr int kCfSegRows = 96;
constexpr int kCfMaxStride = 128;
constexpr int kCfKC = 16;
constexpr int kCfSparseMinCams = 256;

constexpr double kCfUpdFlopsPerMs = 0.83 * 79.0e9;
constexpr double kCfPairMs = (7.82 - 4.21) / (77.35e6 - 31.05e6);
constexpr double kCfSlabMs = 1.30 / 1.35e8;
constexpr double kCfStrideMargin = 0.05;
inline double cf_stride_cost(double upd_flops, double pairs, double slab) {
  return upd_flops / kCfUpdFlopsPerMs + pairs * kCfPairMs + slab * kCfSlabMs;
}
inline int cf_stride_choose(long n_o, const double* upd_flops, const double* pairs, const double* slab) {
  if (n_o < 8192) return kCfFwdCh;
  const double base = cf_stride_cost(upd_flops[0], pairs[0], slab[0]);
  int best = 1;
  double best_ms = base * (1.0 - kCfStrideMargin);
  for (int m = 2; m <= 3; ++m) {
    const double ms = cf_stride_cost(upd_flops[m - 1], pairs[m - 1], slab[m - 1]);
    if (ms < best_ms) { best = m; best_ms = ms; }
  }
  return best * kCfFwdCh;
}

struct CfSwitches {
  int sparse = -1;
  bool tperm_off = false;
  bool no_nd = false;
  int nd_min = 48;
  int stride = 0;
  int os_kernel = 1;
};

struct CfSegTables {
  int S = kCfFwdCh, nseg = 0, nw = 0;
  std::vector<int> p, o, first;
  std::vector<int> seg_start, xld, fw_off;
  std::vector<long long> xoff, boff, roff, tw_off;
  int n_fwork = 0, n_twork = 0;
  size_t xc_len = 0, p_blocks = 0, prhs_len = 0;
  double sp_flops = 0;
};
struct CfPlan : CfSegTables {
  int n_list = 0, n_chunks = 0;
  int64_t ldx = 0, ldt = 0, kpad = 0, kpad_s = 0;
  bool nd = false;
  int stride = 0, n_sep = 0, n_seg = 1;
  bool sparse = false;
  int form = 0;
  std::vector<int> os, ou;
  size_t y_len = 0;
  size_t os_npairs = 0;
  bool os_offsets = false;
  double os_flops = 0;
  bool tperm = false;
  std::vector<int> rank, unrank, kfirst;
  double upd_flops = 0;
};

inline void cf_entry_lists(int N, int nf, const std::vector<int>& start, const int* cu_start, const int* cu_obj, const int* cu_id,
                           std::vector<int>& os, std::vector<int>& ou) {
  std::vector<int> cur(start.begin(), start.end() - 1);
  os.assign((size_t)start[(size_t)N], 0); ou.assign((size_t)start[(size_t)N], 0);
  for (int sl = 0; sl < nf; ++sl)
    for (int q = cu_start[sl]; q < cu_start[sl + 1]; ++q) { const int at = cur[cu_obj[q]]++; os[(size_t)at] = sl; ou[(size_t)at] = cu_id[q]; }
}
inline CfSegTables cf_walk(int S, int N, int nf, const int* cu_start, const int* cu_obj) {
  CfSegTables t;
  const int nseg = (nf + S - 1) / S;
  t.S = S; t.nseg = nseg; t.nw = (nseg + 63) / 64;
  std::vector<int> last_seg((size_t)N, -1);
  for (int sl = 0; sl < nf; ++sl) {
    const int p = sl / S, pos = sl - p * S;
    if (pos == S - 1) continue;
    for (int q = cu_start[sl]; q < cu_start[sl + 1]; ++q) {
      const int o = cu_obj[q];
      if (last_seg[(size_t)o] != p) { last_seg[(size_t)o] = p; t.p.push_back(p); t.o.push_back(o); t.first.push_back(pos); }
    }
  }
  const size_t n_inc = t.p.size();
  const long long rows = S == kCfFwdCh ? kCfSegRows : 6 * (S - 1);
  t.seg_start.assign((size_t)nseg + 1, 0); t.xld.assign((size_t)nseg, 0); t.fw_off.assign((size_t)nseg + 1, 0);
  t.xoff.assign((size_t)nseg + 1, 0); t.boff.assign((size_t)nseg + 1, 0); t.roff.assign((size_t)nseg + 1, 0); t.tw_off.assign((size_t)nseg + 1, 0);
  for (size_t q = 0; q < n_inc; ++q) ++t.seg_start[(size_t)t.p[q] + 1];
  for (int p = 0; p < nseg; ++p) t.seg_start[(size_t)p + 1] += t.seg_start[(size_t)p];
  for (size_t q = 0; q < n_inc; ++q)
    t.sp_flops += 81.0 * (double)(q - (size_t)t.seg_start[(size_t)t.p[q]] + 1) * (6.0 * (S - 1 - t.first[q]));
  for (int p = 0; p < nseg; ++p) {
    const int cnt = t.seg_start[(size_t)p + 1] - t.seg_start[(size_t)p];
    const int m = 9 * cnt + 1;
    t.xld[(size_t)p] = (m + 15) / 16 * 16 + 16;
    t.xoff[(size_t)p + 1] = t.xoff[(size_t)p] + rows * t.xld[(size_t)p];
    t.fw_off[(size_t)p + 1] = t.fw_off[(size_t)p] + (m + 63) / 64;
    t.boff[(size_t)p + 1] = t.boff[(size_t)p] + (long long)cnt * (cnt + 1) / 2;
    t.roff[(size_t)p + 1] = t.roff[(size_t)p] + 9LL * cnt;
    const long long nt = (9 * cnt + kCfSyT - 1) / kCfSyT;
    t.tw_off[(size_t)p + 1] = t.tw_off[(size_t)p] + nt * (nt + 1) / 2;
  }
  t.n_fwork = t.fw_off[(size_t)nseg]; t.n_twork = (int)t.tw_off[(size_t)nseg];
  t.xc_len = (size_t)t.xoff[(size_t)nseg] + 2 * kCfSyT;
  t.p_blocks = (size_t)t.boff[(size_t)nseg]; t.prhs_len = (size_t)t.roff[(size_t)nseg];
  return t;
}
inline double cf_staircase(int S, int N, int nf, const std::vector<int>& unrank, const std::vector<int>& first_cam, std::vector<int>& kfirst) {
  const size_t n_o = (size_t)9 * N;
  double upd_flops = 0;
  const int Ks = (int)((6 * ((size_t)nf / (size_t)S) + kCfKC - 1) / kCfKC * kCfKC);
  kfirst.assign((n_o + 1 + 256) / 64 + 8, Ks);
  for (size_t col = 0; col < n_o; ++col) {
    const int k0 = std::max(0, first_cam[(size_t)unrank[col / 9]] / S - 1);
    kfirst[col / 64] = std::min(kfirst[col / 64], std::min(6 * k0, Ks));
  }
  kfirst[n_o / 64] = 0;
  const long nti = ((long)n_o + 1 + 127) / 128;
  for (long ti = 0; ti < nti; ++ti) {
    const int ka = std::min(kfirst[(size_t)(ti * 2)], kfirst[(size_t)(ti * 2 + 1)]);
    for (long tj = 0; tj <= ti && tj * 128 < (long)n_o; ++tj) {
      const int kb = std::min(kfirst[(size_t)(tj * 2)], kfirst[(size_t)(tj * 2 + 1)]);
      int ks = std::min(std::max(ka, kb), Ks) & ~(kCfKC - 1);
      if (((Ks - ks) & kCfKC) != 0 && ks >= kCfKC) ks -= kCfKC;
      const double rows_t = (double)std::min<long>(128, (long)n_o + 1 - ti * 128), cols_t = (double)std::min<long>(128, (long)n_o - tj * 128);
      const double in_triangle = tj < ti ? 1.0 : 0.5 * (cols_t + 1.0) / cols_t;
      upd_flops += 2.0 * rows_t * cols_t * (double)(Ks - ks) * in_triangle;
    }
  }
  return upd_flops;
}
struct CfOsCounts { double prod = 0, rhs_entries = 0; };
inline CfOsCounts cf_os_counts(int S, int N, const std::vector<int>& start, const std::vector<int>& os, const std::vector<int>& rank) {
  std::vector<std::array<int, 3>> inc3;
  CfOsCounts n;
  for (int o = 0; o < N; ++o) {
    int last_p = -1;
    for (int k = start[(size_t)o]; k < start[(size_t)o + 1]; ++k) {
      const int sl = os[(size_t)k];
      if (sl % S == S - 1) continue;
      const int p = sl / S;
      if (p != last_p) { inc3.push_back({p, rank.empty() ? o : rank[(size_t)o], 0}); last_p = p; }
      ++inc3.back()[2]; n.rhs_entries += 1;
    }
  }
  std::sort(inc3.begin(), inc3.end());
  for (size_t q = 0, q0 = 0; q < inc3.size(); ++q) {
    if (inc3[q][0] != inc3[q0][0]) q0 = q;
    n.prod += (double)inc3[q][2] * (double)(q - q0 + 1);
  }
  return n;
}

inline bool cf_plan_build(int N, int nf, size_t EU, const std::vector<int>& start, const int* cu_start, const int* cu_obj, const int* cu_id, bool chain_ok,
                          bool comm, size_t total_mem, const CfSwitches& sw, CfPlan& pl) {
  pl = CfPlan{};
  const size_t nfz = (size_t)nf, n_o = (size_t)9 * N;
  const int nch = (nf + kCfFwdCh - 1) / kCfFwdCh;
  pl.ldx = (int64_t)((n_o + 1 + 127) / 128 * 128);
  pl.kpad = (int64_t)((6 * nfz + kCfKC - 1) / kCfKC * kCfKC);
  pl.ldt = pl.ldx;
  pl.n_list = start[(size_t)N]; pl.n_chunks = nch;
  pl.nseg = nch; pl.nw = (nch + 63) / 64;
  if ((size_t)std::max(N, 1) * (size_t)(nch + 1) > ((size_t)1 << 28)) return false;
  cf_entry_lists(N, nf, start, cu_start, cu_obj, cu_id, pl.os, pl.ou);
  CfSegTables& seg = pl;
  if (chain_ok && nf >= kCfSparseMinCams && N > 0 && (size_t)nch * (size_t)(N + 1) <= ((size_t)1 << 28) && !sw.no_nd) {
    seg = cf_walk(kCfFwdCh, N, nf, cu_start, cu_obj);
    const double dense = (double)n_o * (double)n_o * 6.0 * (double)nfz;
    const double sparse = (double)n_o * (double)n_o * 6.0 * (double)(nfz / kCfFwdCh) + 24.0 * pl.sp_flops;
    pl.sparse = sw.sparse >= 0 ? sw.sparse != '0' : (n_o >= 2048 && sparse < 0.5 * dense);
    const double need = 8.0 * (81.0 * (double)pl.p_blocks + (double)pl.xc_len + 2.0 * (double)pl.ldt * (double)n_o +
                               2.0 * 6.0 * (double)(nfz / kCfFwdCh) * (double)pl.ldx  + 54.0 * (double)EU );
    pl.form = sw.sparse == '2' || need > 0.4 * (double)total_mem ? 2 : 1;
    if ((sw.sparse < 0 || sw.sparse == '3') && !comm) pl.form = 3;
  }
  const bool sp = pl.sparse;
  std::vector<int> first_cam;
  pl.tperm = sp && N > 0 && !sw.tperm_off;
  if (pl.tperm) {
    std::vector<int> cnt(nfz + 2, 0);
    first_cam.assign((size_t)N, nf);
    for (int o = 0; o < N; ++o) if (start[(size_t)o + 1] > start[(size_t)o]) first_cam[(size_t)o] = pl.os[(size_t)start[(size_t)o]];
    for (int o = 0; o < N; ++o) ++cnt[(size_t)first_cam[(size_t)o] + 1];
    for (int s = 0; s <= nf; ++s) cnt[(size_t)s + 1] += cnt[(size_t)s];
    pl.rank.assign((size_t)N, 0); pl.unrank.assign((size_t)N, 0);
    for (int o = 0; o < N; ++o) { const int t = cnt[(size_t)first_cam[(size_t)o]]++; pl.rank[(size_t)o] = t; pl.unrank[(size_t)t] = o; }
  }
  if (sp && pl.form == 3 && !comm) {
    int want = sw.stride;
    CfSegTables cand[3];
    if (!want && pl.tperm && n_o >= 8192) {
      double upd[3], pairs[3], slab[3];
      for (int m = 1; m <= 3; ++m) {
        const int S = m * kCfFwdCh;
        cand[m - 1] = cf_walk(S, N, nf, cu_start, cu_obj);
        const CfOsCounts n = cf_os_counts(S, N, start, pl.os, pl.rank);
        long long cols = 0;
        for (int x : cand[m - 1].xld) cols += x;
        upd[m - 1] = cf_staircase(S, N, nf, pl.unrank, first_cam, pl.kfirst); pairs[m - 1] = n.prod + n.rhs_entries; slab[m - 1] = 6.0 * (S - 1) * (double)cols;
      }
      want = cf_stride_choose((long)n_o, upd, pairs, slab);
      seg = std::move(cand[want / kCfFwdCh - 1]);
    }
    if (!want) want = kCfFwdCh;
    if (want != pl.S) seg = cf_walk(want, N, nf, cu_start, cu_obj);
  }
  pl.nd = nfz >= (size_t)std::max(sw.nd_min, 2 * kCfFwdCh) && !sw.no_nd;
  if (pl.nd) {
    int sd = 16 * (int)std::max(1.0, std::floor(std::sqrt((double)nfz) / 16.0 + 0.5));
    sd = std::min(sd, kCfMaxStride);
    if (sp) sd = pl.S;
    pl.stride = sd; pl.n_sep = nf / sd; pl.n_seg = (nf + sd - 1) / sd;
  }
  if (sp) pl.kpad_s = (int64_t)((6 * (size_t)pl.n_sep + kCfKC - 1) / kCfKC * kCfKC);
  if (pl.tperm) pl.upd_flops = cf_staircase(pl.S, N, nf, pl.unrank, first_cam, pl.kfirst);
  if (sp && pl.form == 3) {
    const CfOsCounts n = cf_os_counts(pl.S, N, start, pl.os, pl.rank);
    const size_t y_recs = std::max<size_t>(pl.p.size(), 1) * (size_t)(pl.S - 1);
    pl.os_flops = 2.0 * 6.0 * (81.0 * n.prod + 9.0 * n.rhs_entries);
    pl.os_npairs = (size_t)(n.prod + n.rhs_entries);
    pl.y_len = y_recs * 54 + std::max<size_t>(nfz, 1) * 6;
    pl.os_offsets = sw.os_kernel != 0 && 54 * std::max(EU, y_recs) <= (size_t)INT32_MAX;
  }
  return true;
}

}
```

### object-oriented-slam_amd/csrc/esl_ctx.hpp

```cpp
#pragma once
#include <hip/hip_runtime.h>

#include <cstdint>
#include <string>
#include <type_traits>
#include <vector>

#include "../../include/esl.h"
#include "esl_cf_plan.hpp"
#include "esl_math.hpp"

namespace esl {

void set_error(const std::string& s);
#define ESL_HIP_TRY(expr)                                                                         \
  do {                                                                                            \
    hipError_t _e = (expr);                                                                       \
    if (_e != hipSuccess) {                                                                       \
      esl::set_error(std::string(#expr) + ": " + hipGetErrorString(_e));                          \
      return ESL_ERR_HIP;                                                                         \
    }                                                                                             \
  } while (0)

struct DevGraph {
// ... 72 lines not shown
  double lambda_used = 0;
  bool have_trial = false;
};

}

#include "esl_scratch.hpp"

struct BlobArena { char* dev = nullptr; size_t cap = 0; char* host = nullptr; size_t host_cap = 0; hipEvent_t ev = nullptr; };
struct esl_ctx;
namespace esl {
struct ProfScope {
  esl_ctx* c; int slot;
  ProfScope(esl_ctx* ctx, int kind);
  ~ProfScope();
};
int prof_drain(esl_ctx* c);
void fit_graphs_clear(esl_ctx* c);
void fit_release(esl_ctx* c);
void plane_release(esl_ctx* c);
void reloc_release(esl_ctx* c);
void assoc_release(esl_ctx* c);
void merge_release(esl_ctx* c);
void render_release(esl_ctx* c);
void dense_release(esl_ctx* c);
void init_batch_release(esl_ctx* c);
void reloc_scratch_stats(const esl_ctx* c, int64_t* allocs, int64_t* bytes);
void assoc_scratch_stats(const esl_ctx* c, int64_t* allocs, int64_t* bytes);
void merge_scratch_stats(const esl_ctx* c, int64_t* allocs, int64_t* bytes);
void render_scratch_stats(const esl_ctx* c, int64_t* allocs, int64_t* bytes);
void init_scratch_stats(const esl_ctx* c, bool robust, int64_t* allocs, int64_t* bytes);
void dense_scratch_stats(const esl_ctx* c, int64_t* allocs, int64_t* bytes);
int comm_gather_scalars_device(esl_ctx* c);
int comm_allreduce_sum(esl_ctx* c, double* dev_buf, size_t count, hipStream_t st = nullptr);
int comm_reduce_sum_root(esl_ctx* c, double* dev_buf, size_t count, int root);
int comm_bcast(esl_ctx* c, double* dev_buf, size_t count, int root, hipStream_t st = nullptr);
int comm_check_replicated(esl_ctx* c);
int comm_reduce4(esl_ctx* c, const double* dev_src4, double out[4]);
}

struct esl_ctx {
  int device = 0;
  hipStream_t stream = nullptr;
  esl::DevGraph g;
  bool graph_loaded = false;
  bool states_loaded = false;
  double* cams = nullptr; double* cams_trial = nullptr;
  double* objs = nullptr; double* objs_trial = nullptr;
  double* Hoo = nullptr;
  double* bo = nullptr;
  double* xo = nullptr;
  double* obj_part = nullptr;
  double* Hcc = nullptr;
  double* bc = nullptr;
  double* xc = nullptr;
  double* Wbb = nullptr;
  double* Abb = nullptr;
  double* Aod = nullptr;
  double* Dinv = nullptr;
  double* Yb = nullptr;
  double* Wt = nullptr;
  double* Tb = nullptr;
  double* S = nullptr;
  int64_t S_n = 0;
  double* cam_part = nullptr;
  double* od_part = nullptr;
  int* chol_info = nullptr;
  double* host_part = nullptr;
  double* dev_part = nullptr;
  esl::LmState lm;
  esl_robust_params robust = {{0, 0, 0, 0}, {1, 1, 1, 1}};
  bool robust_on = false;
  std::vector<int> h_bb_slot_of, h_e3_slot_of, h_grav_obj;
  esl::Scratch eq_buf;
  double* cams_snap = nullptr; double* objs_snap = nullptr;
  bool prof_on = false;
  int prof_level = 0;
  unsigned prof_runs = 0;
  bool prof_gate = true;
  std::vector<hipEvent_t> prof_ev;
  std::vector<int> prof_kind;
  size_t prof_used = 0;
  int64_t prof_count[ESL_PROF_KINDS] = {0};
  double prof_ms[ESL_PROF_KINDS] = {0};
  std::vector<int> h_bb_cam, h_bb_obj, h_e3_cam, h_e3_obj, h_cam_slot, h_od_i, h_od_j;
  int n_chunks = 0;
  int *ck_obj = nullptr, *ck_type = nullptr, *ck_begin = nullptr, *ck_end = nullptr, *ck_ostart = nullptr;
  int *ck_ids_bb = nullptr, *ck_ids_e3 = nullptr; int n_ids_bb = 0, n_ids_e3 = 0;
  double* chunk_out = nullptr;
  double* chunk_out2 = nullptr;
  hipEvent_t ev_try = nullptr;
  double* chunk_chi = nullptr;
  double* blk_part = nullptr;
  double* solve_part = nullptr;
  double* blk_chi = nullptr;
  unsigned int* tickets = nullptr;
  double* dev_scal = nullptr;
  esl::HostImage* append_img = nullptr;
  char* append_dev = nullptr; size_t append_dev_cap = 0;
  char* slam_tab_dev = nullptr; size_t slam_tab_cap = 0;
  char* arena_graph = nullptr; size_t arena_graph_cap = 0;
  char* arena_work = nullptr;  size_t arena_work_cap = 0;
  char* stage_host = nullptr;  size_t stage_host_cap = 0;
  BlobArena arena_slam, arena_solve, arena_S;
  const int *h_cu_start = nullptr, *h_cu_obj = nullptr, *h_cu_id = nullptr;
  std::vector<int> h_ue_start, h_ue_id, h_ue_slot;
  char* fit_slab = nullptr; size_t fit_slab_cap = 0;
  char* fit_in = nullptr;  size_t fit_in_cap = 0;
  char* fit_out = nullptr; size_t fit_out_cap = 0;
  esl::Scratch plane_slab;
  esl::RelocState* reloc = nullptr;
  esl::AssocState* assoc = nullptr;
  esl::MergeState* merge = nullptr;
  esl::RenderState* render = nullptr;
  esl::DenseState* dense = nullptr;
  esl::InitBatchState* init_batch = nullptr;
  void* fit_graph_cache = nullptr;
  bool parts_fresh = false;
  bool cams_match_snap = false;
  int n_grav_edges = 0;
  void* lm_dev = nullptr;
  void* lm_host = nullptr;
  void* lm_host_dev = nullptr;
  void* host_scal = nullptr;
  void* host_scal_dev = nullptr;
  bool sys_combined = false;
  void* comm = nullptr;
  int comm_ranks = 1, comm_rank = 0;
  bool comm_replicated = false;
  esl_host_allreduce_fn host_allreduce = nullptr;
  void* host_user = nullptr;
  double* host_stage = nullptr;
  double* dev_gather = nullptr;
  double* host_gather = nullptr;
  double* Linv_ws = nullptr;
  double* z_ws = nullptr;
  int64_t S_lda = 0;
  bool cf_chain_ok = false;
  bool cf_ready = false;
  bool cf_unavailable = false;
  esl::CfPlan cf_plan;
  int *cf_oe_start = nullptr, *cf_oe_u = nullptr, *cf_oe_slot = nullptr, *cf_od_start = nullptr, *cf_od_edge = nullptr, *cf_oe_cst = nullptr;
  double *cf_Linv = nullptr, *cf_M = nullptr, *cf_N = nullptr, *cf_V = nullptr, *cf_vy = nullptr, *cf_z = nullptr;
  double *cf_B = nullptr, *cf_Lfac = nullptr, *cf_G = nullptr;
  double *cf_Zt = nullptr, *cf_Hs = nullptr, *cf_Bs = nullptr, *cf_LfacS = nullptr, *cf_GS = nullptr, *cf_LiS = nullptr, *cf_MS = nullptr,
         *cf_NS = nullptr, *cf_R = nullptr;
  double *cf_Xt = nullptr, *cf_T = nullptr, *cf_Linv_ws = nullptr, *cf_part = nullptr;
  int *cf_seg_start = nullptr, *cf_seg_obj = nullptr, *cf_seg_first = nullptr, *cf_cmap = nullptr, *cf_xld = nullptr, *cf_fwork = nullptr, *cf_twork = nullptr;
  unsigned long long* cf_mask = nullptr;
  long long *cf_xoff = nullptr, *cf_boff = nullptr, *cf_roff = nullptr;
  double *cf_Xc = nullptr, *cf_Xs = nullptr, *cf_P = nullptr, *cf_Prhs = nullptr, *cf_Y = nullptr, *cf_Yr = nullptr;
  long long* cf_os_start = nullptr;
  int *cf_os_cnt = nullptr, *cf_os_pairs = nullptr;
  int *cf_rank = nullptr, *cf_unrank = nullptr, *cf_kfirst = nullptr;
  double* cf_xo_t = nullptr;
  int lm_solver_used = 0;
  bool fx_on = false;
  std::vector<uint8_t> fx_flags;
  esl::AnchGraph fx;
  char* fx_blob = nullptr; size_t fx_blob_cap = 0;
  double* fx_A = nullptr; double* fx_chi = nullptr;
  std::vector<int> fx_bb_map, fx_e3_map;
  std::vector<int> fx_grav_obj;
  bool chain_ok = false;
  esl::Scratch chain_ws;
  esl_pcg_params pcg = {1000, 8, 1e-10};
  esl_pcg_params pcg_run = {1000, 8, 1e-10};
  double* pcg_ws = nullptr; size_t pcg_ws_cap = 0;
  double* pcg_st = nullptr; double* pcg_M = nullptr;
  double* pcg_host = nullptr;
  bool pcg_ran = false;
  bool pcg_reset = true;
  void* chol_rt = nullptr;
  void* chol_prof_scope = nullptr;
  unsigned long long graph_fp = 0;
  bool repl_checked = false;
  double *chol_pack = nullptr, *chol_pack2 = nullptr;
  size_t chol_pack_len = 0;
  bool schur_attr_set = false;
  int sw_chol_dist = -1;
  bool sw_chol_overlap = true;
  int sw_cf_overlap = 4;
  int sw_cf_os_kernel = 1;
  int sw_cf_stride = 0;
};
```

### object-oriented-slam_amd/csrc/esl_slam.hip

```cpp
#include "esl_slam.hpp"

#include <algorithm>
#include <array>
#include <chrono>
#include <cmath>
#include <cstdio>
#include <cstdlib>
#include <cstring>

#include "esl_cf.hpp"
#include "esl_chol.hpp"
#include "esl_fixed.hpp"
#include "esl_kernels_slam.hpp"
#include "esl_pcg.hpp"

namespace esl {

static __global__ __launch_bounds__(256) void k_cf_updates(DevGraph g, int nb_obj, double lambda, const double* __restrict__ objs, const double* __restrict__ bo,
                                                           const double* __restrict__ xo, double* __restrict__ objs_trial, double* __restrict__ obj_part,
                                                           const double* __restrict__ cams, const double* __restrict__ xc, const double* __restrict__ bc,
                                                           double* __restrict__ cams_trial, double* __restrict__ cam_part) {
  if ((int)blockIdx.x < nb_obj) cf_obj_update_one(g, lambda, objs, bo, xo, objs_trial, obj_part, blockIdx.x * 256 + threadIdx.x);
  else slam_cam_update_one(g, lambda, cams, xc, bc, cams_trial, cam_part, ((int)blockIdx.x - nb_obj) * 256 + threadIdx.x);
}
// ... 86 lines not shown
int slam_alloc(esl_ctx* c) {
  DevGraph& g = c->g;
  const int N = g.n_objs, F = g.n_cams, nf = g.n_free_cams;
  const bool timing = std::getenv("ESL_UPLOAD_HOST_TIMING") != nullptr;
  const double t0 = timing ? now_us() : 0;
  std::vector<int>& start = c->h_ue_start;
  std::vector<int>& id = c->h_ue_id;
  std::vector<int>& slot = c->h_ue_slot;
  start.assign((size_t)N + 1, 0);
  for (int i = 0; i < g.n_bbox; ++i) if (c->h_bb_obj[i] >= 0 && c->h_cam_slot[c->h_bb_cam[i]] >= 0) ++start[(size_t)c->h_bb_obj[i] + 1];
  for (int i = 0; i < g.n_e3d; ++i) if (c->h_e3_obj[i] >= 0 && c->h_cam_slot[c->h_e3_cam[i]] >= 0) ++start[(size_t)c->h_e3_obj[i] + 1];
  for (int o = 0; o < N; ++o) start[(size_t)o + 1] += start[o];
  const size_t nue = (size_t)start[N];
  id.resize(nue); slot.resize(nue);
  {
    std::vector<int> cur(start.begin(), start.end() - 1);
    for (int i = 0; i < g.n_bbox; ++i) {
      if (c->h_bb_obj[i] < 0) continue;
      const int s = c->h_cam_slot[c->h_bb_cam[i]];
      if (s >= 0) { const int at = cur[c->h_bb_obj[i]]++; id[at] = i; slot[at] = s; }
    }
    for (int i = 0; i < g.n_e3d; ++i) {
      if (c->h_e3_obj[i] < 0) continue;
      const int s = c->h_cam_slot[c->h_e3_cam[i]];
      if (s >= 0) { const int at = cur[c->h_e3_obj[i]]++; id[at] = g.n_bbox + i; slot[at] = s; }
    }
  }
  g.n_ue = (int)nue;
  std::vector<int> ods((size_t)std::max(nf, 1) + 1, 0), ode;
  bool chain = true;
  {
    std::vector<std::pair<int, int>> pe;
    for (int e = 0; e < g.n_odom; ++e) {
      const int si = c->h_cam_slot[c->h_od_i[e]], sj = c->h_cam_slot[c->h_od_j[e]];
      if (si < 0 || sj < 0) continue;
      if (si == sj + 1) pe.push_back({sj, e * 2});
      else if (sj == si + 1) pe.push_back({si, e * 2 + 1});
      else chain = false;
    }
    for (auto& p : pe) ++ods[(size_t)p.first + 1];
    for (int k = 0; k < nf; ++k) ods[(size_t)k + 1] += ods[k];
    ode.resize(pe.size());
    std::vector<int> cur(ods.begin(), ods.end() - 1);
    for (auto& p : pe) ode[(size_t)cur[p.first]++] = p.second;
  }
  c->cf_chain_ok = chain && nf > 0 && N > 0;
  c->chain_ok = chain && nf > 0;
  const double t1 = timing ? now_us() : 0;
  const size_t EU = (size_t)g.n_bbox + g.n_e3d;
  const int64_t n = 6 * (int64_t)nf;
  c->S_n = n;
  c->S_lda = ((n + 1 + 127) / 128) * 128;
  BlobStage st;
  const int i_ust = st.up(&g.ue_start, start.size()), i_uid = st.up(&g.ue_id, nue), i_usl = st.up(&g.ue_slot, nue);
  const int i_cst = st.up(&g.cu_start, (size_t)nf + 1), i_cob = st.up(&g.cu_obj, nue), i_cid = st.up(&g.cu_id, nue);
  const int i_ods = st.up(&c->cf_od_start, ods.size()), i_ode = st.up(&c->cf_od_edge, ode.size());
  st.work(&c->Hcc, (size_t)nf * 36); st.work(&c->bc, (size_t)nf * 6);
  st.work(&c->Wbb, EU * 54);
  st.work(&c->Abb, EU * 27);
  st.work(&c->Yb, EU * 54);
  st.work(&c->Wt, EU * 54);
  st.work(&c->Tb, EU * 6);
  st.work(&c->Aod, (size_t)g.n_odom * 90); st.work(&c->Dinv, (size_t)N * 81);
  st.work(&c->cam_part, (size_t)F * 4); st.work(&c->od_part, (size_t)g.n_odom);
  st.work(&c->xc, (size_t)n); st.work(&c->z_ws, (size_t)kNB);
  if (int rc = st.reserve(c->arena_slam)) return rc;
  std::memcpy(st.host<int>(i_ust), start.data(), start.size() * sizeof(int));
  if (nue) { std::memcpy(st.host<int>(i_uid), id.data(), nue * sizeof(int)); std::memcpy(st.host<int>(i_usl), slot.data(), nue * sizeof(int)); }
  std::memcpy(st.host<int>(i_ods), ods.data(), ods.size() * sizeof(int));
  if (!ode.empty()) std::memcpy(st.host<int>(i_ode), ode.data(), ode.size() * sizeof(int));
  {
    int* cstart = st.host<int>(i_cst); int* cobj = st.host<int>(i_cob); int* cid = st.host<int>(i_cid);
    c->h_cu_start = cstart; c->h_cu_obj = cobj; c->h_cu_id = cid;
    std::fill(cstart, cstart + nf + 1, 0);
    for (size_t k = 0; k < nue; ++k) ++cstart[(size_t)slot[k] + 1];
    g.cu_max = 0;
    for (int s = 0; s < nf; ++s) { g.cu_max = std::max(g.cu_max, cstart[(size_t)s + 1]); cstart[(size_t)s + 1] += cstart[s]; }
    std::vector<int> cur(cstart, cstart + nf);
    for (int o = 0; o < N; ++o)
      for (int k = start[o]; k < start[(size_t)o + 1]; ++k) { const int at = cur[slot[k]]++; cobj[at] = o; cid[at] = id[k]; }
  }
  if (int rc = st.ship(c->stream)) return rc;
  ESL_HIP_TRY(hipMemsetAsync(c->Abb, 0, std::max<size_t>(EU, 1) * 27 * sizeof(double), c->stream));
  ESL_HIP_TRY(hipMemsetAsync(c->Wbb, 0, std::max<size_t>(EU, 1) * 54 * sizeof(double), c->stream));
  if (timing) {
    const double t2 = now_us();
    ESL_HIP_TRY(hipStreamSynchronize(c->stream));
    fprintf(stderr, "[slam_alloc host, us] lists %.0f  layout + per-camera lists + enqueue %.0f  wait %.0f  (blob %.1f MB uploaded, %.1f MB in all)\n",
            t1 - t0, t2 - t1, now_us() - t2, st.up_end / 1e6, st.total / 1e6);
  }
  return ESL_OK;
}

static CholRuntime& chol_rt(esl_ctx* c);
static __global__ void k_info_to_double(const int* __restrict__ info, double* __restrict__ d) { d[0] = info[0] ? 1.0 : 0.0; }
static __global__ void k_double_to_info(const double* __restrict__ d, int* __restrict__ info) { if (d[0] > 0.5) info[0] |= 1; }
static int slam_ensure_S(esl_ctx* c) {
  if (c->S) return ESL_OK;
  const size_t n = (size_t)c->S_n, np = (n + kNB - 1) / kNB;
  BlobStage st;
  st.work(&c->S, (size_t)c->S_lda * n); st.work(&c->Linv_ws, np * kNB * kNB);
  const int rc = st.reserve(c->arena_S);
  if (rc) { c->S = c->Linv_ws = nullptr; return rc; }
  return st.ship(c->stream);
}

static int chol_pack_ensure(esl_ctx* c, int n) {
  const size_t need = chol_pack_len(n);
  if (c->chol_pack && c->chol_pack2 && c->chol_pack_len >= need) return ESL_OK;
  int rc = al(&c->chol_pack, need);
  if (rc) return rc;
  if ((rc = al(&c->chol_pack2, need))) return rc;
  c->chol_pack_len = need;
  return ESL_OK;
}
static int chol_dist_fill(esl_ctx* c, int n, CholDist& d) {
  d.rank = c->comm_rank; d.n_ranks = c->comm_ranks; d.user = c;
  d.bcast = [](void* u, double* dev, size_t count, int root) { return comm_bcast((esl_ctx*)u, dev, count, root); };
  const int rc = chol_pack_ensure(c, n);
  if (rc) return rc;
  d.pack = c->chol_pack;
  if (c->sw_chol_overlap) {
    d.pack2 = c->chol_pack2;
    d.bcast_on = [](void* u, double* dev, size_t count, int root, hipStream_t st) { return comm_bcast((esl_ctx*)u, dev, count, root, st); };
  }
  return ESL_OK;
}
static bool cf_applicable(const esl_ctx* c) { return c->cf_chain_ok && (!c->comm || c->comm_replicated); }
static bool cf_dist(const esl_ctx* c) {
  if (!c->comm || !c->comm_replicated || c->comm_ranks < 2) return false;
  if (c->sw_chol_dist >= 0) return c->sw_chol_dist == 1;
  return 9L * c->g.n_objs >= 8192;
}
static bool chain_applicable(const esl_ctx* c) { return c->chain_ok && c->g.n_ue == 0 && !c->comm; }
static int slam_pick_solver(const esl_ctx* c) {
  const int want = c->lm.p.linear_solver;
  if (want == ESL_SOLVER_PCG) return c->comm ? -3 : ESL_SOLVER_PCG;
  if (want == ESL_SOLVER_CAMERA_CHAIN) return chain_applicable(c) ? ESL_SOLVER_CAMERA_CHAIN : -2;
  if (want == ESL_SOLVER_AUTO && c->fx_on && chain_applicable(c)) return ESL_SOLVER_CAMERA_CHAIN;
  if (want == ESL_SOLVER_REDUCED_CAMERA) return ESL_SOLVER_REDUCED_CAMERA;
  if (want == ESL_SOLVER_REDUCED_ELLIPSOID) return cf_applicable(c) ? ESL_SOLVER_REDUCED_ELLIPSOID : -1;
  if (!cf_applicable(c) || c->cf_unavailable) return ESL_SOLVER_REDUCED_CAMERA;
  const double nc = (double)c->S_n, no = 9.0 * c->g.n_objs;
  return (no * no * nc + no * no * no / 3.0 < nc * nc * nc / 3.0) ? ESL_SOLVER_REDUCED_ELLIPSOID : ESL_SOLVER_REDUCED_CAMERA;
}
static void cf_forget(esl_ctx* c) {
  c->cf_oe_start = c->cf_oe_u = c->cf_oe_slot = c->cf_oe_cst = nullptr;
  c->cf_seg_start = c->cf_seg_obj = c->cf_seg_first = c->cf_cmap = c->cf_xld = c->cf_fwork = c->cf_twork = nullptr;
  c->cf_mask = nullptr; c->cf_xoff = c->cf_boff = c->cf_roff = nullptr;
  c->cf_Linv = c->cf_M = c->cf_N = c->cf_V = c->cf_B = c->cf_Lfac = c->cf_G = c->cf_vy = c->cf_z = nullptr;
  c->cf_T = c->cf_Linv_ws = c->cf_part = nullptr;
  c->cf_Zt = c->cf_Hs = c->cf_Bs = c->cf_LfacS = c->cf_GS = c->cf_LiS = c->cf_MS = c->cf_NS = c->cf_R = nullptr;
  c->cf_Xc = c->cf_Xs = c->cf_P = c->cf_Prhs = c->cf_Xt = c->cf_Y = c->cf_Yr = nullptr;
  c->cf_os_start = nullptr; c->cf_os_cnt = c->cf_os_pairs = nullptr;
  c->cf_rank = c->cf_unrank = c->cf_kfirst = nullptr; c->cf_xo_t = nullptr;
  c->cf_plan = CfPlan{};
  c->cf_ready = false;
}
static int cf_ensure_impl(esl_ctx* c);
static int cf_ensure(esl_ctx* c) {
  if (c->cf_ready) return ESL_OK;
  const int rc = cf_ensure_impl(c);
  if (rc) { cf_forget(c); (void)hipGetLastError(); return rc; }
  c->cf_ready = true;
  return ESL_OK;
}
static_assert(kCfKC == kKC, "esl_cf_plan.hpp pads K to the rank-K update's chunk");
static int cf_ensure_impl(esl_ctx* c) {
  const DevGraph& g = c->g;
  const int N = g.n_objs, nfi = g.n_free_cams;
  const size_t nf = (size_t)nfi, EU = (size_t)g.n_bbox + g.n_e3d, n_o = (size_t)9 * N;
  const bool timing = std::getenv("ESL_UPLOAD_HOST_TIMING") != nullptr;
  const double t0 = timing ? now_us() : 0;
  CfSwitches sw;
  { const char* e = std::getenv("ESL_CF_SPARSE"); sw.sparse = e ? (int)(unsigned char)e[0] : -1; }
  { const char* e = std::getenv("ESL_CF_TPERM"); sw.tperm_off = e && e[0] == '0'; }
  sw.no_nd = std::getenv("ESL_CF_NO_ND") != nullptr;
  static const int nd_min = [] { const char* e = std::getenv("ESL_CF_ND_MIN"); return e ? std::atoi(e) : 48; }();
  sw.nd_min = nd_min; sw.stride = c->sw_cf_stride; sw.os_kernel = c->sw_cf_os_kernel;
  size_t free_b = 0, total_b = 0;
  if (nfi >= kCfSparseMinCams) ESL_HIP_TRY(hipMemGetInfo(&free_b, &total_b));
  CfPlan& pl = c->cf_plan;
  if (!cf_plan_build(N, nfi, EU, c->h_ue_start, c->h_cu_start, c->h_cu_obj, c->h_cu_id, c->cf_chain_ok, c->comm != nullptr, total_b, sw, pl)) {
    set_error("camera-first elimination: the (ellipsoid, camera chunk) range table of this graph exceeds 1 GB");
    return ESL_ERR_ALLOC;
  }
  const bool sp = pl.sparse, os3 = sp && pl.form == 3;
  const int nch = pl.n_chunks, nseg = pl.nseg, nw = pl.nw, N1 = N + 1;
  const size_t n_inc = pl.p.size();
  const size_t y_recs = std::max<size_t>(n_inc, 1) * (size_t)(pl.S - 1), nb = (size_t)N * (N + 1) / 2 + N;
  const double t1 = timing ? now_us() : 0;
  BlobStage st;
  struct Up { int item; const void* src; size_t bytes; };
  std::vector<Up> ups;
  auto ship = [&](auto** dst, const auto& v) { ups.push_back({st.up(dst, v.size()), v.data(), v.size() * sizeof(v[0])}); };
  ship(&c->cf_oe_start, c->h_ue_start); ship(&c->cf_oe_u, pl.ou); ship(&c->cf_oe_slot, pl.os);
  int* d_inc = nullptr; int* d_fw_off = nullptr; long long* d_tw_off = nullptr;
  int i_inc = -1;
  if (pl.tperm) { ship(&c->cf_rank, pl.rank); ship(&c->cf_unrank, pl.unrank); ship(&c->cf_kfirst, pl.kfirst); }
  if (sp) {
    i_inc = st.up(&d_inc, 4 * n_inc); ship(&c->cf_seg_start, pl.seg_start); ship(&c->cf_xld, pl.xld);
    ship(&c->cf_xoff, pl.xoff); ship(&c->cf_boff, pl.boff); ship(&c->cf_roff, pl.roff); ship(&d_fw_off, pl.fw_off); ship(&d_tw_off, pl.tw_off);
  }
  st.work(&c->cf_oe_cst, (size_t)std::max(N, 1) * (nch + 1));
  if (sp) {
    st.work(&c->cf_cmap, (size_t)nseg * N1); st.work(&c->cf_mask, (size_t)N1 * nw); st.work(&c->cf_seg_obj, n_inc); st.work(&c->cf_seg_first, n_inc);
    st.work(&c->cf_fwork, 2 * (size_t)pl.n_fwork); st.work(&c->cf_twork, 3 * (size_t)pl.n_twork);
  }
  st.work(&c->cf_Linv, nf * 36); st.work(&c->cf_M, nf * 36); st.work(&c->cf_N, nf * 36); st.work(&c->cf_V, EU * 54);
  st.work(&c->cf_B, nf * 36); st.work(&c->cf_Lfac, nf * 21); st.work(&c->cf_G, nf * 36); st.work(&c->cf_vy, nf * 6); st.work(&c->cf_z, nf * 6);
  st.work(&c->cf_T, (size_t)pl.ldt * n_o); st.work(&c->cf_Linv_ws, ((n_o + kNB - 1) / kNB) * kNB * kNB);
  if (pl.tperm) st.work(&c->cf_xo_t, n_o);
  if (n_o <= 1024) st.work(&c->cf_part, (size_t)kCholMaxSplit * (size_t)pl.ldt * n_o);
  if (pl.nd) {
    const size_t ns = (size_t)std::max(pl.n_sep, 1);
    st.work(&c->cf_Zt, nf * 36); st.work(&c->cf_Hs, ns * 36); st.work(&c->cf_Bs, ns * 36); st.work(&c->cf_LfacS, ns * 21);
    st.work(&c->cf_GS, ns * 36); st.work(&c->cf_LiS, ns * 36); st.work(&c->cf_MS, ns * 36); st.work(&c->cf_NS, ns * 36);
    st.work(&c->cf_R, ns * 6 * (size_t)pl.ldx);
  }
  if (sp) {
    st.work(&c->cf_Xc, pl.xc_len); st.work(&c->cf_Xs, (size_t)pl.ldx * (size_t)pl.kpad_s);
    if (pl.form == 1) { st.work(&c->cf_P, pl.p_blocks * 81); st.work(&c->cf_Prhs, pl.prhs_len); }
    if (pl.form == 3) {
      st.work(&c->cf_Y, y_recs * 54); st.work(&c->cf_Yr, std::max<size_t>(nf, 1) * 6);
      st.work(&c->cf_os_start, nb + 1); st.work(&c->cf_os_cnt, nb); st.work(&c->cf_os_pairs, 2 * std::max<size_t>(pl.os_npairs, 1));
    }
  } else {
    st.work(&c->cf_Xt, (size_t)pl.ldx * (size_t)pl.kpad);
  }
  if (int rc = st.reserve(c->arena_solve)) return rc;
  for (const Up& u : ups) if (u.bytes) std::memcpy(st.host<char>(u.item), u.src, u.bytes);
  if (sp && n_inc) {
    int* inc = st.host<int>(i_inc);
    std::memcpy(inc, pl.p.data(), n_inc * sizeof(int)); std::memcpy(inc + n_inc, pl.o.data(), n_inc * sizeof(int));
    std::memcpy(inc + 2 * n_inc, pl.first.data(), n_inc * sizeof(int));
    for (size_t q = 0; q < n_inc; ++q) inc[3 * n_inc + q] = (int)q;
  }
  if (int rc = st.ship(c->stream)) return rc;
  if (N > 0) {
    const long nt = (long)N * (nch + 1);
    hipLaunchKernelGGL(k_cf_make_cst, dim3((unsigned)((nt + 255) / 256)), dim3(256), 0, c->stream, N, nch, c->cf_oe_start, c->cf_oe_slot, c->cf_oe_cst);
  }
  if (sp) {
    ESL_HIP_TRY(hipMemsetAsync(c->cf_cmap, 0xFF, (size_t)nseg * N1 * sizeof(int), c->stream));
    ESL_HIP_TRY(hipMemsetAsync(c->cf_mask, 0, (size_t)N1 * nw * sizeof(unsigned long long), c->stream));
    if (n_inc)
      hipLaunchKernelGGL(k_cf_make_cmap, dim3((unsigned)((n_inc + 255) / 256)), dim3(256), 0, c->stream, (int)n_inc, d_inc, N1, nw, c->cf_seg_start, c->cf_cmap,
                         c->cf_mask, c->cf_seg_obj, c->cf_seg_first);
    hipLaunchKernelGGL(k_cf_make_work, dim3((unsigned)nseg), dim3(64), 0, c->stream, nseg, N, nw, c->cf_seg_start, d_fw_off, d_tw_off, c->cf_cmap, c->cf_mask,
                       c->cf_fwork, c->cf_twork);
  }
  if (os3) {
    const dim3 grid((unsigned)(N + 1), (unsigned)((N + kCfTPer - 1) / kCfTPer));
    ESL_HIP_TRY(hipMemsetAsync(c->cf_os_cnt, 0, nb * sizeof(int), c->stream));
    hipLaunchKernelGGL(k_cf_os_list<false>, grid, dim3(256), 0, c->stream, N, nw, nch, pl.S / kCfFwdCh, c->cf_mask, c->cf_cmap, c->cf_seg_start, c->cf_oe_cst, c->cf_oe_slot,
                       (const int*)c->cf_unrank, (const long long*)nullptr, c->cf_os_cnt, (int2*)nullptr, 0);
    std::vector<int> h_cnt(nb);
    std::vector<long long> h_start(nb + 1);
    ESL_HIP_TRY(hipMemcpyAsync(h_cnt.data(), c->cf_os_cnt, nb * sizeof(int), hipMemcpyDeviceToHost, c->stream));
    ESL_HIP_TRY(hipStreamSynchronize(c->stream));
    h_start[0] = 0;
    for (size_t b = 0; b < nb; ++b) h_start[b + 1] = h_start[b] + h_cnt[b];
    if ((size_t)h_start[nb] != pl.os_npairs) {
      set_error("camera-first elimination: the one-sided assembly's pair list does not have the length the host counted");
      return ESL_ERR_STATE;
    }
    ESL_HIP_TRY(hipMemcpyAsync(c->cf_os_start, h_start.data(), (nb + 1) * sizeof(long long), hipMemcpyHostToDevice, c->stream));
    hipLaunchKernelGGL(k_cf_os_list<true>, grid, dim3(256), 0, c->stream, N, nw, nch, pl.S / kCfFwdCh, c->cf_mask, c->cf_cmap, c->cf_seg_start, c->cf_oe_cst, c->cf_oe_slot,
                       (const int*)c->cf_unrank, (const long long*)c->cf_os_start, c->cf_os_cnt, (int2*)c->cf_os_pairs, pl.os_offsets ? 1 : 0);
    ESL_HIP_TRY(hipStreamSynchronize(c->stream));
  }
  if (pl.nd) ESL_HIP_TRY(hipMemsetAsync(c->cf_Zt, 0, nf * 36 * sizeof(double), c->stream));
  if (sp) {
    ESL_HIP_TRY(hipMemsetAsync(c->cf_Xc, 0, std::max<size_t>(pl.xc_len, 1) * sizeof(double), c->stream));
    ESL_HIP_TRY(hipMemsetAsync(c->cf_Xs, 0, (size_t)pl.ldx * (size_t)pl.kpad_s * sizeof(double), c->stream));
    ESL_HIP_TRY(hipMemsetAsync(c->cf_T, 0, (size_t)pl.ldt * n_o * sizeof(double), c->stream));
    if (pl.form == 3) {
      ESL_HIP_TRY(hipMemsetAsync(c->cf_Y, 0, y_recs * 54 * sizeof(double), c->stream));
      ESL_HIP_TRY(hipMemsetAsync(c->cf_Yr, 0, std::max<size_t>(nf, 1) * 6 * sizeof(double), c->stream));
    }
  } else {
    ESL_HIP_TRY(hipMemsetAsync(c->cf_Xt, 0, (size_t)pl.ldx * (size_t)pl.kpad * sizeof(double), c->stream));
  }
  ESL_HIP_TRY(hipMemsetAsync(c->cf_V, 0, std::max<size_t>(EU, 1) * 54 * sizeof(double), c->stream));
  if (timing)
    fprintf(stderr, "[cf_ensure host, us] sorts + structure %.0f  layout + tables + enqueue %.0f  (blob %.1f MB uploaded, %.1f MB in all; sparse %d form %d)\n",
            t1 - t0, now_us() - t1, st.up_end / 1e6, st.total / 1e6, (int)sp, pl.form);
  return ESL_OK;
}

namespace {
struct CfSideJoin {
  CholRuntime& rt; hipStream_t main; bool armed;
  hipError_t wait(hipEvent_t ev) { const hipError_t e = hipStreamWaitEvent(main, ev, 0); armed = e != hipSuccess; return e; }
  ~CfSideJoin() {
    if (!armed) return;
    if (hipEventRecord(rt.cf_ev_p, rt.cf_side) != hipSuccess || hipStreamWaitEvent(main, rt.cf_ev_p, 0) != hipSuccess) (void)hipStreamSynchronize(rt.cf_side);
  }
};
struct CfTrial {
  esl_ctx* c; CholRuntime& rt; const CfPlan& pl; const DevGraph& g; const double lambda;
  const int N, nf, n_o; const long ldx, ldt;
  const int st, ns, nseg;
  const bool nd, dist;
  const unsigned cg;
  const hipStream_t main;
  CfSideJoin join;
  CfTrial(esl_ctx* c_, CholRuntime& rt_, double lambda_)
      : c(c_), rt(rt_), pl(c_->cf_plan), g(c_->g), lambda(lambda_), N(g.n_objs), nf(g.n_free_cams), n_o(9 * N), ldx((long)pl.ldx), ldt((long)pl.ldt),
        st(pl.stride), ns(pl.n_sep), nseg(pl.n_seg), nd(st > 0 && ns > 0), dist(cf_dist(c_)), cg((unsigned)((n_o + 1 + 63) / 64)), main(c_->stream),
        join{rt_, c_->stream, false} {}
  CfSegs segs() const { return CfSegs{c->cf_fwork, c->cf_seg_start, c->cf_seg_obj, c->cf_xoff, c->cf_xld, c->cf_rank, c->cf_unrank}; }
  int edge_blocks() const { return (int)(((long)pl.n_list * 9 + nf + 255) / 256); }
  template <class F> void my_columns(F f) const {
    if (!dist) { f(0L, (long)n_o); return; }
    const int Wp = chol_outer_panels(n_o), n_outer = ((n_o + kNB - 1) / kNB + Wp - 1) / Wp;
    for (int op = c->comm_rank; op < n_outer; op += c->comm_ranks) f((long)op * Wp * kNB, std::min<long>((long)(op + 1) * Wp * kNB, (long)n_o));
  }
  dim3 block_grid(long c_begin, long c_end, int& o2b, int& o2e) const {
    o2b = (int)(c_begin / 9); o2e = (int)((c_end + 8) / 9);
    return dim3((unsigned)(N + 1), (unsigned)((o2e - o2b + kCfTPer - 1) / kCfTPer));
  }
  void edge_scale(int cls, hipStream_t s) const {
    hipLaunchKernelGGL(k_cf_edge_scale, dim3((unsigned)edge_blocks()), dim3(256), 0, s, g, pl.n_list, c->cf_oe_u, c->cf_oe_slot, c->Wbb, c->cf_Linv, c->bc,
                       c->cf_V, c->cf_vy, cls, st);
  }
  void segment_chains() const {
    hipLaunchKernelGGL(k_cf_chain, dim3((unsigned)nseg), dim3(64), 0, main, nf, c->Hcc, c->cf_B, lambda, c->cf_Lfac, c->cf_G, c->chol_info, st, st - 1);
    hipLaunchKernelGGL(k_cf_factor_blocks, dim3((unsigned)((nf + 63) / 64)), dim3(64), 0, main, nf, c->cf_Lfac, c->cf_G, c->cf_Linv, c->cf_M, c->cf_N, st);
    if (nseg > 1) hipLaunchKernelGGL(k_cf_zt, dim3((unsigned)(nseg - 1)), dim3(64), 0, main, nf, st, c->cf_Linv, c->cf_M, c->cf_B, c->cf_Zt);
    hipLaunchKernelGGL(k_cf_sep_assemble, dim3((unsigned)((ns * 36 + 255) / 256)), dim3(256), 0, main, nf, st, ns, c->Hcc, lambda, c->cf_G, c->cf_Zt,
                       c->cf_Hs, c->cf_Bs);
  }
  void sep_chain(hipStream_t s) const {
    hipLaunchKernelGGL(k_cf_chain, dim3(1), dim3(64), 0, s, ns, c->cf_Hs, c->cf_Bs, 0.0, c->cf_LfacS, c->cf_GS, c->chol_info, ns, ns);
    hipLaunchKernelGGL(k_cf_factor_blocks, dim3((unsigned)((ns + 63) / 64)), dim3(64), 0, s, ns, c->cf_LfacS, c->cf_GS, c->cf_LiS, c->cf_MS, c->cf_NS, 0,
                       c->cf_Linv, st);
  }
  int slabs(bool beside) {
    segment_chains();
    if (beside) {
      ESL_HIP_TRY(hipEventRecord(rt.cf_ev_a, main));
      ESL_HIP_TRY(hipStreamWaitEvent(rt.cf_side, rt.cf_ev_a, 0));
      join.armed = true;
    }
    sep_chain(beside ? rt.cf_side : main);
    if (beside) ESL_HIP_TRY(hipEventRecord(rt.cf_ev_s, rt.cf_side));
    edge_scale(beside ? 1 : 0, main);
    hipLaunchKernelGGL(k_cf_forward<2>, dim3((unsigned)pl.n_fwork), dim3(64), 0, main, nf, n_o, pl.n_chunks, c->cf_oe_cst, c->cf_oe_slot, c->cf_V,
                       c->cf_vy, c->cf_M, c->cf_Xc, ldx, st, st - 1, (const double*)c->cf_Zt, c->cf_R, st, segs());
    return ESL_OK;
  }
  void sep_rhs(hipStream_t s, bool sp = true) const {
    hipLaunchKernelGGL(k_cf_sep_rhs, dim3(cg, (unsigned)ns), dim3(64), 0, s, nf, n_o, st, pl.n_chunks, c->cf_oe_cst, c->cf_oe_slot, c->cf_V, c->cf_vy,
                       c->cf_G, c->cf_LiS, sp ? c->cf_Xc : c->cf_Xt, ldx, c->cf_R, sp ? (const int*)c->cf_cmap : nullptr, sp ? segs() : CfSegs{});
  }
  void sep_forward(hipStream_t s, bool sp = true) const {
    hipLaunchKernelGGL(k_cf_forward<1>, dim3(cg), dim3(64), 0, s, ns, n_o, pl.n_chunks, c->cf_oe_cst, c->cf_oe_slot, c->cf_V, c->cf_vy,
                       c->cf_MS, sp ? c->cf_Xs : c->cf_Xt, ldx, ns, ns, (const double*)nullptr, c->cf_R, sp ? 0 : st, CfSegs{});
  }
  void products(hipStream_t s) const {
    hipLaunchKernelGGL(k_cf_seg_syrk, dim3((unsigned)pl.n_twork), dim3(256), 0, s, c->cf_twork, c->cf_seg_start, c->cf_seg_first, c->cf_xoff,
                       c->cf_xld, c->cf_Xc, c->cf_boff, c->cf_P);
    hipLaunchKernelGGL(k_cf_seg_rhs, dim3((unsigned)pl.n_fwork), dim3(64), 0, s, c->cf_fwork, c->cf_seg_start, c->cf_xoff, c->cf_xld, c->cf_Xc,
                       c->cf_roff, c->cf_Prhs);
  }
  void gather_products(long c_begin, long c_end, int accumulate) const {
    int o2b, o2e;
    const dim3 grid = block_grid(c_begin, c_end, o2b, o2e);
    hipLaunchKernelGGL(k_cf_T_gather, grid, dim3(256), 0, main, N, pl.nw, c->cf_mask, c->cf_cmap, c->cf_boff, c->cf_roff, c->cf_P, c->cf_Prhs,
                       c->Hoo, c->bo, lambda, c->cf_T, ldt, o2b, o2e, (const int*)c->cf_unrank, accumulate);
  }
  void update() const {
    ProfScope pk(c, 7);
    const double* Xf = pl.sparse ? c->cf_Xs : c->cf_Xt;
    const int K = (int)(pl.sparse ? pl.kpad_s : pl.kpad);
    if (!dist && K <= 0) return;
    my_columns([&](long c_begin, long c_end) {
      chol_launch_update(rt.sw, c->cf_T, ldt, (long)n_o + 1, main, 0, K, c_begin, c_end, Xf, ldx, dist ? nullptr : c->cf_part, pl.sparse ? c->cf_kfirst : nullptr);
    });
  }

  int build_dense() {
    auto edge_scale_T = [&] {
      const int nb_es = edge_blocks();
      hipLaunchKernelGGL(k_cf_edge_scale_T, dim3((unsigned)(nb_es + (int)((ldt * (long)n_o + 255) / 256))), dim3(256), 0, main, g, nb_es, pl.n_list, c->cf_oe_u,
                         c->cf_oe_slot, c->Wbb, c->cf_Linv, c->bc, c->cf_V, c->cf_vy, c->Hoo, c->bo, lambda, c->cf_T, ldt, (long)n_o);
    };
    if (!nd) {
      hipLaunchKernelGGL(k_cf_chain, dim3(1), dim3(64), 0, main, nf, c->Hcc, c->cf_B, lambda, c->cf_Lfac, c->cf_G, c->chol_info, nf, nf);
      hipLaunchKernelGGL(k_cf_factor_blocks, dim3((unsigned)((nf + 63) / 64)), dim3(64), 0, main, nf, c->cf_Lfac, c->cf_G, c->cf_Linv, c->cf_M, c->cf_N, 0);
      edge_scale_T();
      hipLaunchKernelGGL(k_cf_forward<0>, dim3(cg), dim3(64), 0, main, nf, n_o, pl.n_chunks, c->cf_oe_cst, c->cf_oe_slot, c->cf_V, c->cf_vy,
                         c->cf_M, c->cf_Xt, ldx, nf, nf, (const double*)nullptr, (double*)nullptr, 0, CfSegs{});
    } else {
      segment_chains();
      sep_chain(main);
      edge_scale_T();
      hipLaunchKernelGGL(k_cf_forward<0>, dim3(cg, (unsigned)nseg), dim3(64), 0, main, nf, n_o, pl.n_chunks, c->cf_oe_cst, c->cf_oe_slot, c->cf_V,
                         c->cf_vy, c->cf_M, c->cf_Xt, ldx, st, st - 1, (const double*)c->cf_Zt, c->cf_R, st, CfSegs{});
      sep_rhs(main, false);
      sep_forward(main, false);
    }
    ESL_HIP_TRY(hipGetLastError());
    update();
    return ESL_OK;
  }

  int build_stored_serial() {
    if (int rc = slabs(false)) return rc;
    sep_rhs(main);
    sep_forward(main);
    {
      ProfScope pk(c, 8);
      if (pl.form == 1) products(main);
      my_columns([&](long c_begin, long c_end) {
        if (pl.form == 1) { gather_products(c_begin, c_end, 0); return; }
        int o2b, o2e;
        const dim3 grid = block_grid(c_begin, c_end, o2b, o2e);
        hipLaunchKernelGGL(k_cf_T_sparse, grid, dim3(256), 0, main, N, pl.nw, c->cf_mask, c->cf_cmap, c->cf_xoff, c->cf_xld, c->cf_Xc, c->Hoo, c->bo,
                           lambda, c->cf_T, ldt, o2b, o2e, (const int*)c->cf_unrank);
      });
    }
    ESL_HIP_TRY(hipGetLastError());
    update();
    return ESL_OK;
  }

  int build_stored_side(int ov) {
    const bool side_chain = ov != 3, early_products = ov != 2;
    if (int rc = slabs(side_chain)) return rc;
    if (side_chain) {
      ESL_HIP_TRY(join.wait(rt.cf_ev_s));
      edge_scale(2, main);
    }
    sep_rhs(main);
    if (early_products) ESL_HIP_TRY(hipEventRecord(rt.cf_ev_x, main));
    sep_forward(main);
    if (!early_products) ESL_HIP_TRY(hipEventRecord(rt.cf_ev_x, main));
    ESL_HIP_TRY(hipStreamWaitEvent(rt.cf_side, rt.cf_ev_x, 0));
    join.armed = true;
    products(rt.cf_side);
    ESL_HIP_TRY(hipEventRecord(rt.cf_ev_p, rt.cf_side));
    if (chol_update_v_applies(rt.sw, ldt, (long)n_o + 1, 0, (long)n_o, true, ldx)) {
      {
        ProfScope pk(c, 7);
        chol_launch_update(rt.sw, c->cf_T, ldt, (long)n_o + 1, main, 0, (int)pl.kpad_s, 0, (long)n_o, c->cf_Xs, ldx, nullptr, c->cf_kfirst, true, ov == 4);
      }
      ESL_HIP_TRY(join.wait(rt.cf_ev_p));
      ProfScope pk(c, 8);
      gather_products(0, (long)n_o, 1);
    } else {
      ESL_HIP_TRY(join.wait(rt.cf_ev_p));
      {
        ProfScope pk(c, 8);
        gather_products(0, (long)n_o, 0);
      }
      ESL_HIP_TRY(hipGetLastError());
      update();
    }
    return ESL_OK;
  }

  int build_onesided(bool beside) {
    const hipStream_t sst = beside ? rt.cf_side : main;
    if (int rc = slabs(beside)) return rc;
    if (beside) {
      ESL_HIP_TRY(hipEventRecord(rt.cf_ev_x, main));
      ESL_HIP_TRY(hipStreamWaitEvent(rt.cf_side, rt.cf_ev_x, 0));
      edge_scale(2, rt.cf_side);
    }
    sep_rhs(sst);
    sep_forward(sst);
    if (beside) ESL_HIP_TRY(hipEventRecord(rt.cf_ev_p, rt.cf_side));
    {
      ProfScope pk(c, 8);
      auto seg_back = [&](auto mch) {
        hipLaunchKernelGGL(k_cf_seg_back<decltype(mch)::value>, dim3((unsigned)pl.n_fwork), dim3(64), 0, main, nf, c->cf_fwork, c->cf_seg_start, c->cf_xoff,
                           c->cf_xld, c->cf_Xc, c->cf_Linv, c->cf_G, c->cf_Y, c->cf_Yr);
      };
      if (st == 3 * kCfFwdCh) seg_back(std::integral_constant<int, 3>{});
      else if (st == 2 * kCfFwdCh) seg_back(std::integral_constant<int, 2>{});
      else seg_back(std::integral_constant<int, 1>{});
      const dim3 grid((unsigned)(N + 1), (unsigned)((N + kCfTPer - 1) / kCfTPer));
      hipLaunchKernelGGL(pl.os_offsets ? k_cf_T_onesided_lds : k_cf_T_onesided, grid, dim3(256), 0, main, N, (const int2*)c->cf_os_pairs,
                         (const long long*)c->cf_os_start, (const int*)c->cf_os_cnt, c->cf_V, c->cf_Y, c->cf_Yr, c->Hoo, c->bo, lambda, c->cf_T, ldt, 0, N,
                         (const int*)c->cf_unrank, 0);
    }
    ESL_HIP_TRY(hipGetLastError());
    if (beside) ESL_HIP_TRY(join.wait(rt.cf_ev_p));
    update();
    return ESL_OK;
  }

  int back_substitute() const {
    {
      ProfScope ps(c, 3);
      double* xsol = (pl.sparse && pl.tperm) ? c->cf_xo_t : c->xo;
      if (dist) {
        CholDist d;
        if (int rc = chol_dist_fill(c, n_o, d)) return rc;
        ESL_HIP_TRY(chol_factor_solve(c->cf_T, ldt, n_o, c->cf_Linv_ws, c->z_ws, xsol, c->chol_info, main, rt, &d));
      } else {
        ESL_HIP_TRY(chol_factor_solve(c->cf_T, ldt, n_o, c->cf_Linv_ws, c->z_ws, xsol, c->chol_info, main, rt));
      }
      if (xsol != c->xo) hipLaunchKernelGGL(k_cf_xo_unpermute, dim3((unsigned)((n_o + 255) / 256)), dim3(256), 0, main, N, c->cf_rank, xsol, c->xo);
      if (pl.sparse)
        hipLaunchKernelGGL(k_cf_z_sparse, dim3((unsigned)(6 * nf)), dim3(256), 0, main, n_o, c->cf_Xs, ldx, segs(), c->cf_Xc, c->xo, xsol, c->cf_z, st);
      else
        hipLaunchKernelGGL(k_cf_z, dim3((unsigned)(6 * nf)), dim3(256), 0, main, c->cf_Xt, ldx, n_o, c->xo, c->cf_z);
      if (nd) {
        hipLaunchKernelGGL(k_cf_tridiag_back, dim3(1), dim3(64), 0, main, ns, c->cf_LiS, c->cf_NS, c->cf_z, c->xc, ns, ns, st);
        hipLaunchKernelGGL(k_cf_back_prep, dim3((unsigned)((6 * nf + 255) / 256)), dim3(256), 0, main, nf, st, ns, c->cf_Zt, c->cf_G, c->xc, c->cf_z);
        hipLaunchKernelGGL(k_cf_tridiag_back, dim3((unsigned)nseg), dim3(64), 0, main, nf, c->cf_Linv, c->cf_N, c->cf_z, c->xc, st, st - 1, 0);
      } else {
        hipLaunchKernelGGL(k_cf_tridiag_back, dim3(1), dim3(64), 0, main, nf, c->cf_Linv, c->cf_N, c->cf_z, c->xc, nf, nf, 0);
      }
      ESL_HIP_TRY(hipGetLastError());
    }
    ProfScope ps(c, 1);
    const int F = g.n_cams, nb_obj = (N + 255) / 256, nb_cam = (F + 255) / 256;
    hipLaunchKernelGGL(k_cf_updates, dim3((unsigned)(nb_obj + nb_cam)), dim3(256), 0, main, g, nb_obj, lambda, c->objs, c->bo, c->xo, c->objs_trial, c->obj_part,
                       c->cams, c->xc, c->bc, c->cams_trial, c->cam_part);
    const int nb_co = (N + kWavesPerBlock - 1) / kWavesPerBlock, nb_od = (g.n_odom + kWave * kWavesPerBlock - 1) / (kWave * kWavesPerBlock);
    robust_dispatch(c->robust_on, [&](auto robust) {
      hipLaunchKernelGGL(k_slam_chi2_all<decltype(robust)::value>, dim3((unsigned)(nb_co + nb_od)), dim3(kWave * kWavesPerBlock), 0, main, g, nb_co,
                         c->cams_trial, c->objs_trial, c->obj_part, c->od_part);
    });
    ESL_HIP_TRY(hipGetLastError());
    return ESL_OK;
  }
};
}
static int slam_try_step_cf(esl_ctx* c, double lambda) {
  int rc = cf_ensure(c);
  if (rc) return rc;
  const CfPlan& pl = c->cf_plan;
  CfTrial t(c, chol_rt(c), lambda);
  {
    ProfScope ps(c, 2);
    ESL_HIP_TRY(hipMemsetAsync(c->chol_info, 0, sizeof(int), c->stream));
    hipLaunchKernelGGL(k_cf_gather_B, dim3((unsigned)(((long)t.nf * 36 + 255) / 256)), dim3(256), 0, c->stream, t.nf, c->Aod, c->cf_od_start, c->cf_od_edge, c->cf_B);
    ESL_HIP_TRY(chol_set_attributes(t.rt));
    if (!pl.sparse) rc = t.build_dense();
    else if (!t.nd) {
      set_error("camera-first elimination: sparse X needs the dissected camera chain");
      rc = ESL_ERR_STATE;
    }
    else {
      const bool side = c->sw_cf_overlap != 0 && (pl.form == 1 || pl.form == 3) && !t.dist && pl.kpad_s > 0 && t.rt.cf_overlap_init() == hipSuccess;
      rc = pl.form == 3 ? t.build_onesided(side) : side ? t.build_stored_side(c->sw_cf_overlap) : t.build_stored_serial();
    }
    if (rc) return rc;
    ESL_HIP_TRY(hipGetLastError());
  }
  return t.back_substitute();
}

static bool slam_dist_chol(esl_ctx* c) {
  if (!c->comm || c->comm_ranks < 2) return false;
  if (c->sw_chol_dist >= 0) return c->sw_chol_dist == 1;
  return c->S_n >= 8192;
}
static void chol_prof_mark(void* user, int begin) {
  esl_ctx* c = (esl_ctx*)user;
  if (begin) { if (!c->chol_prof_scope) c->chol_prof_scope = new ProfScope(c, 9); }
  else if (c->chol_prof_scope) { delete (ProfScope*)c->chol_prof_scope; c->chol_prof_scope = nullptr; }
}
static CholRuntime& chol_rt(esl_ctx* c) {
  if (!c->chol_rt) {
    CholRuntime* rt = new CholRuntime();
    rt->prof_mark = chol_prof_mark; rt->prof_user = c;
    c->chol_rt = rt;
  }
  return *(CholRuntime*)c->chol_rt;
}
void slam_sync_side(esl_ctx* c) {
  if (c->chol_rt && ((CholRuntime*)c->chol_rt)->cf_side) (void)hipStreamSynchronize(((CholRuntime*)c->chol_rt)->cf_side);
}
void slam_release_runtime(esl_ctx* c) {
  if (c->chol_prof_scope) { delete (ProfScope*)c->chol_prof_scope; c->chol_prof_scope = nullptr; }
  if (!c->chol_rt) return;
  ((CholRuntime*)c->chol_rt)->release();
  delete (CholRuntime*)c->chol_rt;
  c->chol_rt = nullptr;
  c->schur_attr_set = false;
}

static int reduce_all(esl_ctx* c, const int* info = nullptr) {
  const DevGraph& g = c->g;
  hipLaunchKernelGGL(k_slam_reduce_all, dim3(1), dim3(256), 0, c->stream, c->obj_part, g.n_objs, c->cam_part, g.n_cams, c->od_part,
                     (g.n_odom && g.shard_rank == 0) ? g.n_odom : 0, c->dev_part, info);
  ESL_HIP_TRY(hipGetLastError());
  return ESL_OK;
}

int slam_linearize(esl_ctx* c) {
  c->parts_fresh = false;
  const DevGraph& g = c->g;
  const int N = g.n_objs, F = g.n_cams;
  const bool an = c->lm.p.jacobian_mode == ESL_JAC_ANALYTIC;
  const double delta = c->lm.p.numeric_delta;
  {
    ProfScope ps(c, 0);
    if (N > 0) {
      ChunkTable ct;
      ct.n_chunks = c->n_chunks; ct.obj = c->ck_obj; ct.type = c->ck_type; ct.begin = c->ck_begin; ct.end = c->ck_end; ct.ostart = c->ck_ostart;
      const dim3 block(64 * kLinWaves);
      const int nb_e3 = (c->n_ids_e3 + kLinWaves - 1) / kLinWaves, nb_bb = (c->n_ids_bb + kLinWaves - 1) / kLinWaves;
      robust_dispatch(c->robust_on, [&](auto robust) {
        constexpr bool R = decltype(robust)::value;
        if (an) {
          if (nb_e3) hipLaunchKernelGGL((k_slam_linearize_chunks<ESL_JAC_ANALYTIC, 1, R>), dim3(nb_e3), block, 0, c->stream, g, ct, c->ck_ids_e3, c->n_ids_e3, c->cams,
                                        c->objs, delta, c->chunk_out, c->Wbb, c->Abb);
          if (nb_bb) hipLaunchKernelGGL((k_slam_linearize_chunks<ESL_JAC_ANALYTIC, 0, R>), dim3(nb_bb), block, 0, c->stream, g, ct, c->ck_ids_bb, c->n_ids_bb, c->cams,
                                        c->objs, delta, c->chunk_out, c->Wbb, c->Abb);
          hipLaunchKernelGGL((k_slam_combine<ESL_JAC_ANALYTIC, R>), dim3((N + kWavesPerBlock - 1) / kWavesPerBlock), dim3(kWave * kWavesPerBlock), 0, c->stream, g, ct,
                             c->chunk_out, c->objs, delta, c->Hoo, c->bo, c->obj_part);
        } else {
          if (nb_e3) hipLaunchKernelGGL((k_slam_linearize_chunks<ESL_JAC_NUMERIC, 1, R>), dim3(nb_e3), block, 0, c->stream, g, ct, c->ck_ids_e3, c->n_ids_e3, c->cams,
                                        c->objs, delta, c->chunk_out, c->Wbb, c->Abb);
          if (nb_bb) hipLaunchKernelGGL((k_slam_linearize_chunks<ESL_JAC_NUMERIC, 0, R>), dim3(nb_bb), block, 0, c->stream, g, ct, c->ck_ids_bb, c->n_ids_bb, c->cams,
                                        c->objs, delta, c->chunk_out, c->Wbb, c->Abb);
          hipLaunchKernelGGL((k_slam_combine<ESL_JAC_NUMERIC, R>), dim3((N + kWavesPerBlock - 1) / kWavesPerBlock), dim3(kWave * kWavesPerBlock), 0, c->stream, g, ct,
                             c->chunk_out, c->objs, delta, c->Hoo, c->bo, c->obj_part);
        }
      });
    }
    if (g.n_odom) {
      const dim3 grid((g.n_odom + 127) / 128), block(128);
      robust_dispatch(c->robust_on, [&](auto robust) {
        constexpr bool R = decltype(robust)::value;
        if (an) hipLaunchKernelGGL((k_slam_odom<ESL_JAC_ANALYTIC, R>), grid, block, 0, c->stream, g, c->cams, delta, c->Aod, c->od_part);
        else hipLaunchKernelGGL((k_slam_odom<ESL_JAC_NUMERIC, R>), grid, block, 0, c->stream, g, c->cams, delta, c->Aod, c->od_part);
      });
    }
    hipLaunchKernelGGL(k_slam_cam_gather, dim3((F + kWavesPerBlock - 1) / kWavesPerBlock), dim3(kWave * kWavesPerBlock), 0, c->stream, g, c->Abb, c->Aod,
                       c->Hcc, c->bc, c->cam_part);
    if (c->fx_on && c->fx.n_bb + c->fx.n_e3 > 0) {
// ... 301 lines not shown
  if (i < n) {
    for (int jj = 0; jj < 64; ++jj) {
      const long j = j0 + jj;
      if (j >= n || j > i) break;
      const double a = M[i + j * lda];
      acc += a * xcol[jj];
      if (i > j) atomicAdd(&ycol[jj], a * xi);
    }
    if (acc != 0) atomicAdd(&y[i], acc);
  }
  __syncthreads();
  if (threadIdx.x < 64 && j0 + threadIdx.x < n && ycol[threadIdx.x] != 0) atomicAdd(&y[j0 + threadIdx.x], ycol[threadIdx.x]);
}
static __global__ __launch_bounds__(256) void k_resid_norms(const double* __restrict__ M, long lda, long n, const double* __restrict__ y,
                                                            double* __restrict__ out2) {
  const long j = (long)blockIdx.x * 256 + threadIdx.x;
  double r2 = 0, b2 = 0;
  if (j < n) { const double b = M[n + j * lda], r = y[j] - b; r2 = r * r; b2 = b * b; }
  r2 = wave_sum(r2); b2 = wave_sum(b2);
  if ((threadIdx.x & 63) == 0) { atomicAdd(&out2[0], r2); atomicAdd(&out2[1], b2); }
}

}

extern "C" int esl_lm_reduced_residual(esl_ctx* c, double* rel_residual_out) {
  using namespace esl;
  if (!c || !rel_residual_out) return ESL_ERR_INVALID;
  if (!c->lm.begun || !c->lm.slam || !c->xc || c->S_n <= 0) { set_error("esl_lm_reduced_residual: needs a SLAM-mode trial step"); return ESL_ERR_STATE; }
  ESL_HIP_TRY(hipSetDevice(c->device));
  const long n = (long)c->S_n, lda = (long)c->S_lda;
  int rc = slam_build_reduced(c, c->lm.lambda_used, true, nullptr, nullptr);
  if (rc) return rc;
  double* y = nullptr;
  ESL_HIP_TRY(hipMalloc((void**)&y, ((size_t)n + 2) * sizeof(double)));
  hipError_t e = hipMemsetAsync(y, 0, ((size_t)n + 2) * sizeof(double), c->stream);
  if (e == hipSuccess) {
    hipLaunchKernelGGL(k_symv_lower, dim3((unsigned)((n + 255) / 256), (unsigned)((n + 63) / 64)), dim3(256), 0, c->stream, c->S, lda, n,
                       c->xc, y);
    hipLaunchKernelGGL(k_resid_norms, dim3((unsigned)((n + 255) / 256)), dim3(256), 0, c->stream, c->S, lda, n, y, y + n);
    e = hipGetLastError();
  }
  double h2[2] = {0, 0};
  if (e == hipSuccess) e = hipMemcpyAsync(h2, y + n, sizeof(h2), hipMemcpyDeviceToHost, c->stream);
  if (e == hipSuccess) e = hipStreamSynchronize(c->stream);
  (void)hipFree(y);
  if (e != hipSuccess) { set_error(std::string("esl_lm_reduced_residual: ") + hipGetErrorString(e)); return ESL_ERR_HIP; }
  *rel_residual_out = h2[1] > 0 ? std::sqrt(h2[0] / h2[1]) : 0.0;
  return ESL_OK;
}

namespace esl {
__device__ __forceinline__ double st_entry(long i, long j, long n) {
  if (i == j) return (double)n;
  const unsigned long long a = (unsigned long long)(i < j ? i : j), b = (unsigned long long)(i < j ? j : i);
  unsigned long long h = a * 0x9E3779B97F4A7C15ull ^ (b + 0x7F4A7C15ull) * 0xC2B2AE3D27D4EB4Full;
  h ^= h >> 29; h *= 0xBF58476D1CE4E5B9ull; h ^= h >> 32;
  return (double)(h >> 11) * (2.0 / 9007199254740992.0) - 1.0;
}
__device__ __forceinline__ double st_rhs(long i) { return 1.0 + 0.001 * (double)(i % 97); }
static __global__ void k_selftest_fill(double* __restrict__ M, long lda, long n) {
  const long i = (long)blockIdx.x * blockDim.x + threadIdx.x, j = blockIdx.y;
  if (i > n || j >= n) return;
  double v = 0;
  if (i == n) v = st_rhs(j);
  else if (i >= j) v = st_entry(i, j, n);
  M[i + j * lda] = v;
}
static __global__ __launch_bounds__(256) void k_selftest_resid(const double* __restrict__ x, long n, double* __restrict__ out2) {
  __shared__ double red[256];
  const long i = blockIdx.x;
  double s = 0;
  for (long j = threadIdx.x; j < n; j += 256) s += st_entry(i, j, n) * x[j];
  red[threadIdx.x] = s;
  __syncthreads();
  for (int st = 128; st > 0; st >>= 1) { if ((int)threadIdx.x < st) red[threadIdx.x] += red[threadIdx.x + st]; __syncthreads(); }
  if (threadIdx.x == 0) {
    const double b = st_rhs(i), r = b - red[0];
    atomicAdd(&out2[0], r * r);
    atomicAdd(&out2[1], b * b);
  }
}
}

extern "C" int esl_selftest_cholesky(esl_ctx* c, int32_t n, double* ms_out, double* rel_residual_out) {
  using namespace esl;
  if (!c || n < 1 || !ms_out || !rel_residual_out) return ESL_ERR_INVALID;
  ESL_HIP_TRY(hipSetDevice(c->device));
  const long lda = (((long)n + 1 + 127) / 128) * 128;
  double *M = nullptr, *Linv = nullptr, *z = nullptr, *x = nullptr, *out2 = nullptr;
  int* info = nullptr;
  const size_t np = (size_t)((n + kNB - 1) / kNB);
  int rc = ESL_OK;
  hipEvent_t e0 = nullptr, e1 = nullptr;
  auto cleanup = [&]() {
    if (M) (void)hipFree(M); if (Linv) (void)hipFree(Linv); if (z) (void)hipFree(z); if (x) (void)hipFree(x);
    if (out2) (void)hipFree(out2); if (info) (void)hipFree(info);
    if (e0) (void)hipEventDestroy(e0); if (e1) (void)hipEventDestroy(e1);
  };
#define ST_TRY(expr) do { hipError_t e_ = (expr); if (e_ != hipSuccess) { set_error(std::string(#expr) + ": " + hipGetErrorString(e_)); cleanup(); return ESL_ERR_HIP; } } while (0)
  ST_TRY(hipMalloc((void**)&M, (size_t)lda * (size_t)n * sizeof(double)));
  ST_TRY(hipMalloc((void**)&Linv, np * kNB * kNB * sizeof(double)));
  ST_TRY(hipMalloc((void**)&z, kNB * sizeof(double)));
  ST_TRY(hipMalloc((void**)&x, (size_t)n * sizeof(double)));
  ST_TRY(hipMalloc((void**)&out2, 2 * sizeof(double)));
  ST_TRY(hipMalloc((void**)&info, sizeof(int)));
  ST_TRY(hipEventCreate(&e0)); ST_TRY(hipEventCreate(&e1));
  ST_TRY(hipMemsetAsync(out2, 0, 2 * sizeof(double), c->stream));
  ST_TRY(hipMemsetAsync(info, 0, sizeof(int), c->stream));
  hipLaunchKernelGGL(k_selftest_fill, dim3((unsigned)((n + 1 + 255) / 256), (unsigned)n), dim3(256), 0, c->stream, M, lda, (long)n);
  ST_TRY(hipEventRecord(e0, c->stream));
  ST_TRY(chol_factor_solve(M, lda, n, Linv, z, x, info, c->stream, chol_rt(c)));
  ST_TRY(hipEventRecord(e1, c->stream));
  if (chol_rt(c).sw.debug) {
    hipStream_t w2 = nullptr;
    if (hipStreamCreateWithFlags(&w2, hipStreamNonBlocking) == hipSuccess) (void)hipStreamDestroy(w2);
  }
  hipLaunchKernelGGL(k_selftest_resid, dim3((unsigned)n), dim3(256), 0, c->stream, x, (long)n, out2);
  double h2[2] = {0, 0};
  int hinfo = 0;
  ST_TRY(hipMemcpyAsync(h2, out2, sizeof(h2), hipMemcpyDeviceToHost, c->stream));
  ST_TRY(hipMemcpyAsync(&hinfo, info, sizeof(int), hipMemcpyDeviceToHost, c->stream));
  ST_TRY(hipStreamSynchronize(c->stream));
  float ms = 0;
  ST_TRY(hipEventElapsedTime(&ms, e0, e1));
#undef ST_TRY
  if (chol_rt(c).sw.timing) chol_print_timing(n);
  *ms_out = ms;
  *rel_residual_out = h2[1] > 0 ? std::sqrt(h2[0] / h2[1]) : 0.0;
  if (hinfo & 2) { set_error("self test: a device-side hand-off of the dense solver timed out"); rc = ESL_ERR_HIP; }
  else if (hinfo) { set_error("self test: non-positive pivot"); rc = ESL_ERR_STATE; }
  cleanup();
  return rc;
}


extern "C" int esl_lm_solver_stats(esl_ctx* c, double* st) {
  if (!c || !st) return ESL_ERR_INVALID;
  for (int k = 0; k < ESL_SOLVER_STATS; ++k) st[k] = 0;
  if (c->lm_solver_used != ESL_SOLVER_REDUCED_ELLIPSOID || !c->cf_ready) return ESL_OK;
  const esl::CfPlan& pl = c->cf_plan;
  st[0] = pl.sparse ? pl.form : 0;
  st[1] = pl.stride; st[2] = pl.n_sep; st[3] = pl.n_seg;
  if (pl.sparse) {
    st[4] = 2.0 * pl.sp_flops;
    st[5] = pl.form == 1 ? 8.0 * 81.0 * (double)pl.p_blocks : 0.0;
    if (pl.form == 3) { st[4] = pl.os_flops; st[5] = 8.0 * (double)pl.y_len; }
    st[6] = 8.0 * (double)pl.xc_len;
  }
  st[7] = (double)(pl.sparse ? pl.kpad_s : pl.kpad);
  st[8] = pl.tperm ? pl.upd_flops : 0.0;
  st[9] = pl.tperm ? 1.0 : 0.0;
  return ESL_OK;
}
extern "C" int esl_lm_pcg_stats(esl_ctx* c, double* st) {
  if (!c || !st) return ESL_ERR_INVALID;
  for (int k = 0; k < ESL_PCG_STATS; ++k) st[k] = 0;
  if (!c->pcg_ran || !c->pcg_st) return ESL_OK;
  ESL_HIP_TRY(hipSetDevice(c->device));
  double h[esl::kPcgState];
  ESL_HIP_TRY(hipMemcpyAsync(h, c->pcg_st, sizeof(h), hipMemcpyDeviceToHost, c->stream));
  ESL_HIP_TRY(hipStreamSynchronize(c->stream));
  st[0] = h[esl::kPcgIters];
  st[1] = h[esl::kPcgBb] > 0 ? std::sqrt(h[esl::kPcgRr] / h[esl::kPcgBb]) : 0.0;
  st[2] = h[esl::kPcgConv];
  if (!c->pcg_reset) { st[3] = h[esl::kPcgSolves]; st[4] = h[esl::kPcgIterSum]; }
  st[5] = c->pcg_run.max_iters; st[6] = c->pcg_run.rel_tol;
  return ESL_OK;
}
extern "C" int esl_lm_solver_used(esl_ctx* c, int32_t* solver_out) {
  if (!c || !solver_out) return ESL_ERR_INVALID;
  *solver_out = c->lm_solver_used;
  return ESL_OK;
}

extern "C" int esl_debug_chol_plan(int32_t n, int32_t W, int32_t filler, int32_t* tasks_out , int64_t cap_tasks,
                                   int32_t* ns_out , int64_t cap_ns, int32_t meta_out[5] ) {
  if (n < 1 || W < 1 || !meta_out) return ESL_ERR_INVALID;
  esl::CholPlan pl;
  esl::chol_plan_from_switches(esl::chol_switches_from_env(), n, W, filler, pl);
  meta_out[0] = pl.np; meta_out[1] = pl.n_outer; meta_out[2] = pl.nR; meta_out[3] = (int32_t)pl.tasks.size(); meta_out[4] = pl.W;
  if (tasks_out) {
    if ((int64_t)pl.tasks.size() > cap_tasks) return ESL_ERR_INVALID;
    for (size_t i = 0; i < pl.tasks.size(); ++i) { tasks_out[4 * i] = pl.tasks[i].type; tasks_out[4 * i + 1] = pl.tasks[i].a; tasks_out[4 * i + 2] = pl.tasks[i].b; tasks_out[4 * i + 3] = pl.tasks[i].c; }
  }
  if (ns_out) {
    if ((int64_t)pl.ns.size() > cap_ns) return ESL_ERR_INVALID;
    for (size_t i = 0; i < pl.ns.size(); ++i) ns_out[i] = pl.ns[i];
  }
  return ESL_OK;
}

extern "C" int esl_debug_update_v_applies(int64_t lda, int64_t rows, int64_t base, int64_t col_limit, int32_t ext, int64_t ldp, int32_t* applies_out) {
  if (!applies_out) return ESL_ERR_INVALID;
  *applies_out = esl::chol_update_v_applies(esl::chol_switches_from_env(), (long)lda, (long)rows, (long)base, (long)col_limit, ext != 0, (long)ldp) ? 1 : 0;
  return ESL_OK;
}

extern "C" int esl_debug_cf_stride_choose(int64_t n_o, const double upd_flops[3], const double pairs[3], const double slab[3], int32_t* stride_out,
                                          double ms_out[3]) {
  if (!upd_flops || !pairs || !slab || !stride_out) return ESL_ERR_INVALID;
  *stride_out = esl::cf_stride_choose((long)n_o, upd_flops, pairs, slab);
  if (ms_out) for (int m = 0; m < 3; ++m) ms_out[m] = esl::cf_stride_cost(upd_flops[m], pairs[m], slab[m]);
  return ESL_OK;
}
```

### object-oriented-slam_amd/lib.py

```python
import ctypes as C
import os
import subprocess
import time

import numpy as np

from . import abi

_CSRC = os.path.join(os.path.dirname(os.path.abspath(__file__)), "csrc")
LIB_PATH = os.environ.get("ESL_HIP_LIB") or os.path.join(_CSRC, "libesl_hip.so")
_lib = None

EXPORTS = [
    "esl_abi_version", "esl_last_error", "esl_device_count", "esl_ctx_create", "esl_ctx_destroy",
    "esl_ctx_synchronize", "esl_ctx_trim", "esl_lm_params_default", "esl_optimize", "esl_optimize_fixed", "esl_graph_upload", "esl_graph_upload_fixed", "esl_graph_obj_fixed", "esl_graph_append", "esl_graph_sizes", "esl_states_upload",
    "esl_states_download", "esl_optimize_resident", "esl_states_snapshot", "esl_states_restore", "esl_profile_enable", "esl_profile_get", "esl_lm_begin", "esl_lm_linearize", "esl_lm_reduced_system", "esl_lm_reduced_residual",
    "esl_lm_try_step", "esl_lm_commit", "esl_lm_solver_used", "esl_lm_solver_stats", "esl_lm_download", "esl_lm_set_robust", "esl_edge_chi2", "esl_pcg_params_default", "esl_lm_set_pcg", "esl_lm_pcg_stats", "esl_comm_unique_id", "esl_comm_init", "esl_comm_init_host", "esl_comm_set_replicated", "esl_comm_destroy", "esl_partition_objects", "esl_fit_params_default", "esl_fit_frame", "esl_fit_frame_debug", "esl_fit_frame_ex", "esl_selftest_cholesky", "esl_debug_chol_plan", "esl_debug_update_v_applies", "esl_debug_cf_stride_choose",
    "esl_init_quadric", "esl_init_from_qstar", "esl_init_plane_error", "esl_init_quadrics", "esl_plane_params_default", "esl_extract_ground_plane", "esl_extract_planes",
    "esl_reloc_params_default", "esl_reloc_set_map", "esl_relocalize",
    "esl_assoc_params_default", "esl_predict_boxes", "esl_associate_boxes",
    "esl_init_robust_params_default", "esl_init_quadrics_robust",
    "esl_merge_params_default", "esl_map_overlaps", "esl_map_merge",
    "esl_render_params_default", "esl_render_map", "esl_debug_render_allocs", "esl_debug_scratch_allocs",
    "esl_dense_params_default", "esl_dense_begin", "esl_dense_add_frames", "esl_dense_info_get", "esl_dense_extract", "esl_dense_end",
    "esl_debug_dense_allocs",
]


class EslError(RuntimeError):
    pass


def build(force=False):
    if force:
        subprocess.check_call(["make", "-s", "-C", _CSRC, "clean"])
    subprocess.check_call(["make", "-s", "-j4", "-C", _CSRC])
    return LIB_PATH


def load():
    global _lib
    if _lib is None:
        if not os.path.exists(LIB_PATH):
            raise EslError(f"{LIB_PATH} is missing: run __graft_entry__.build() (no CPU fallback exists)")
        L = C.CDLL(LIB_PATH)
        L.esl_last_error.restype = C.c_char_p
        for name in EXPORTS:
            if not hasattr(L, name):
                raise EslError(f"libesl_hip.so does not export {name}")
        abi.render_argtypes(L)
        abi.dense_argtypes(L)
        _lib = L
    return _lib


def _check(rc, what):
    if rc != 0:
        msg = load().esl_last_error().decode(errors="replace")
        raise EslError(f"{what} failed with esl_status {rc}: {msg}")


def device_count():
    return int(load().esl_device_count())


_dp = C.POINTER(C.c_double)


def _fixed_flags(obj_fixed, n_objs):
    if obj_fixed is None:
        return None
    f = np.ascontiguousarray(np.asarray(obj_fixed) != 0, dtype=np.uint8).reshape(-1)
    if f.size != n_objs:
        raise ValueError(f"obj_fixed has {f.size} entries, the graph {n_objs} ellipsoids")
    return f


def _edge_counts(graph):
    return [len(graph.bbox_cam), len(graph.e3d_cam), len(graph.grav_obj), len(graph.odom_i)]


class Context:

    def __init__(self, device=0):
        L = load()
        self._h = C.c_void_p()
        self.device = int(device)
        _check(L.esl_ctx_create(C.c_int(device), C.byref(self._h)), "esl_ctx_create")
        self._graph = None
        self._edge_counts = [0, 0, 0, 0]

    def close(self):
        if self._h:
            load().esl_ctx_destroy(self._h)
            self._h = C.c_void_p()

    def __del__(self):
        try:
            self.close()
        except Exception:
            pass

    def optimize(self, graph, cams, objs, params=None, obj_fixed=None):
        p = params if params is not None else abi.default_lm_params()
        g = graph.c_struct()
        cams = np.array(cams, dtype=np.float64, order="C").reshape(-1, 7).copy()
        objs = np.array(objs, dtype=np.float64, order="C").reshape(-1, 10).copy()
        rep = abi.EslLmReport()
        self._edge_counts = _edge_counts(graph)
        fx = _fixed_flags(obj_fixed, graph.n_objs)
        if fx is not None:
            _check(load().esl_optimize_fixed(self._h, C.byref(g), fx.ctypes.data_as(C.POINTER(C.c_uint8)), cams.ctypes.data_as(_dp),
                                             objs.ctypes.data_as(_dp), C.byref(p), C.byref(rep)), "esl_optimize_fixed")
            return cams, objs, rep.as_dict()
        _check(load().esl_optimize(self._h, C.byref(g), cams.ctypes.data_as(_dp), objs.ctypes.data_as(_dp),
                                   C.byref(p), C.byref(rep)), "esl_optimize")
        return cams, objs, rep.as_dict()

    def upload_graph(self, graph, obj_fixed=None):
        g = graph.c_struct()
        fx = _fixed_flags(obj_fixed, graph.n_objs)
        if fx is not None:
            _check(load().esl_graph_upload_fixed(self._h, C.byref(g), fx.ctypes.data_as(C.POINTER(C.c_uint8))), "esl_graph_upload_fixed")
        else:
            _check(load().esl_graph_upload(self._h, C.byref(g)), "esl_graph_upload")
        self._graph = graph
        self._edge_counts = _edge_counts(graph)

    def graph_obj_fixed(self):
        n = self.graph_sizes()["n_objs"]
        f = np.zeros(max(n, 1), dtype=np.uint8)
        _check(load().esl_graph_obj_fixed(self._h, f.ctypes.data_as(C.POINTER(C.c_uint8)), C.c_int32(n)), "esl_graph_obj_fixed")
        return f[:n]

    def append_graph(self, new_cams=(), new_objs=(), bbox=None, e3d=None, grav_obj=(), new_cam_fixed=None, odom=None):
        keep = []

        def arr(a, dt, tail=None):
            a = np.ascontiguousarray(a, dtype=dt)
            if tail is not None and a.size:
                a = a.reshape((-1,) + tail)
            keep.append(a)
            return a
        d = abi.EslGraphDelta()
        nc, no = arr(new_cams, np.float64, (7,)), arr(new_objs, np.float64, (10,))
        d.n_new_cams, d.n_new_objs = (len(nc) if nc.size else 0), (len(no) if no.size else 0)
        d.new_cams = nc.ctypes.data_as(_dp) if nc.size else _dp(); d.new_objs = no.ctypes.data_as(_dp) if no.size else _dp()
        ip = C.POINTER(C.c_int32)
        if bbox is not None and len(bbox[0]):
            bc, bo, bm, bw = arr(bbox[0], np.int32), arr(bbox[1], np.int32), arr(bbox[2], np.float64, (4,)), arr(bbox[3], np.float64)
            d.n_bbox = len(bc); d.bbox_cam = bc.ctypes.data_as(ip); d.bbox_obj = bo.ctypes.data_as(ip)
            d.bbox_meas = bm.ctypes.data_as(_dp); d.bbox_weight = bw.ctypes.data_as(_dp)
        if e3d is not None and len(e3d[0]):
            ec, eo, em, ew = arr(e3d[0], np.int32), arr(e3d[1], np.int32), arr(e3d[2], np.float64, (10,)), arr(e3d[3], np.float64)
            d.n_e3d = len(ec); d.e3d_cam = ec.ctypes.data_as(ip); d.e3d_obj = eo.ctypes.data_as(ip)
            d.e3d_meas = em.ctypes.data_as(_dp); d.e3d_weight = ew.ctypes.data_as(_dp)
        go = arr(grav_obj, np.int32)
        if go.size:
            d.n_grav = len(go); d.grav_obj = go.ctypes.data_as(ip)
        if new_cam_fixed is not None and d.n_new_cams:
            fx = arr(new_cam_fixed, np.uint8)
            assert fx.size == d.n_new_cams
            d.new_cam_fixed = fx.ctypes.data_as(C.POINTER(C.c_uint8))
        if odom is not None and len(odom[0]):
            oi, oj, om = arr(odom[0], np.int32), arr(odom[1], np.int32), arr(odom[2], np.float64, (7,))
            d.n_odom = len(oi); d.odom_i = oi.ctypes.data_as(ip); d.odom_j = oj.ctypes.data_as(ip); d.odom_meas = om.ctypes.data_as(_dp)
            if len(odom) > 3 and odom[3] is not None:
                d.odom_info = arr(odom[3], np.float64, (6,)).ctypes.data_as(_dp)
        _check(load().esl_graph_append(self._h, C.byref(d)), "esl_graph_append")
        self._edge_counts = [a + b for a, b in zip(self._edge_counts, (d.n_bbox, d.n_e3d, d.n_grav, d.n_odom))]
        if self._graph is not None:
            self._graph = _Sizes(self._graph.n_cams + d.n_new_cams, self._graph.n_objs + d.n_new_objs)

    def graph_sizes(self):
        v = [C.c_int32(0) for _ in range(5)]
        _check(load().esl_graph_sizes(self._h, *[C.byref(x) for x in v]), "esl_graph_sizes")
        return dict(zip(("n_cams", "n_objs", "n_bbox", "n_e3d", "relayouts"), [x.value for x in v]))

    def upload_states(self, cams, objs):
        cams = np.ascontiguousarray(cams, dtype=np.float64)
        objs = np.ascontiguousarray(objs, dtype=np.float64)
        _check(load().esl_states_upload(self._h, cams.ctypes.data_as(_dp), objs.ctypes.data_as(_dp)), "esl_states_upload")

    def download_states(self):
        cams = np.zeros((self._graph.n_cams, 7))
        objs = np.zeros((self._graph.n_objs, 10))
        _check(load().esl_states_download(self._h, cams.ctypes.data_as(_dp), objs.ctypes.data_as(_dp)), "esl_states_download")
        return cams, objs

    def optimize_resident(self, params=None):
        p = params if params is not None else abi.default_lm_params()
        rep = abi.EslLmReport()
        _check(load().esl_optimize_resident(self._h, C.byref(p), C.byref(rep)), "esl_optimize_resident")
        return rep.as_dict()

    def lm_begin(self, params=None):
        p = params if params is not None else abi.default_lm_params()
        nv, nd = C.c_int32(0), C.c_int32(0)
        _check(load().esl_lm_begin(self._h, C.byref(p), C.byref(nv), C.byref(nd)), "esl_lm_begin")
        return nv.value, nd.value

    def lm_linearize(self):
        out = abi.EslLmPartials()
        _check(load().esl_lm_linearize(self._h, C.byref(out)), "esl_lm_linearize")
        return out

    def lm_try_step(self, lam):
        out = abi.EslLmPartials()
        _check(load().esl_lm_try_step(self._h, C.c_double(lam), C.byref(out)), "esl_lm_try_step")
        return out

    def lm_commit(self, accept):
        _check(load().esl_lm_commit(self._h, C.c_int(1 if accept else 0)), "esl_lm_commit")

    def lm_solver_used(self):
        v = C.c_int32(0)
        _check(load().esl_lm_solver_used(self._h, C.byref(v)), "esl_lm_solver_used")
        return v.value

    def lm_solver_stats(self):
        st = (C.c_double * 10)()
        _check(load().esl_lm_solver_stats(self._h, st), "esl_lm_solver_stats")
        names = ["x_form", "stride", "separators", "segments", "product_flops", "product_bytes", "slab_bytes", "dense_update_rows",
                 "dense_update_flops_executed", "t_ordered_by_first_camera"]
        return {n: float(st[i]) for i, n in enumerate(names)}

    def lm_reduced_system(self, lam):
        ptr, n, lda = C.c_void_p(), C.c_int64(0), C.c_int64(0)
        _check(load().esl_lm_reduced_system(self._h, C.c_double(lam), C.byref(ptr), C.byref(n), C.byref(lda)),
               "esl_lm_reduced_system")
        return ptr.value, n.value, lda.value

    def lm_reduced_residual(self):
        r = C.c_double(0)
        _check(load().esl_lm_reduced_residual(self._h, C.byref(r)), "esl_lm_reduced_residual")
        return r.value

    def set_robust(self, bbox=None, e3d=None, grav=None, odom=None):
        p = abi.default_robust_params(bbox=bbox, e3d=e3d, grav=grav, odom=odom)
        _check(load().esl_lm_set_robust(self._h, C.byref(p)), "esl_lm_set_robust")

    def set_pcg(self, max_iters=None, check_every=None, rel_tol=None):
        p = abi.default_pcg_params()
        if max_iters is not None:
            p.max_iters = int(max_iters)
        if check_every is not None:
            p.check_every = int(check_every)
        if rel_tol is not None:
            p.rel_tol = float(rel_tol)
        _check(load().esl_lm_set_pcg(self._h, C.byref(p)), "esl_lm_set_pcg")

    def lm_pcg_stats(self):
        st = (C.c_double * 8)()
        _check(load().esl_lm_pcg_stats(self._h, st), "esl_lm_pcg_stats")
        names = ["iterations", "rel_residual", "converged", "solves", "iterations_total", "max_iters", "rel_tol", "reserved"]
        return {n: float(st[i]) for i, n in enumerate(names)}

    def edge_chi2(self, edge_class):
        cls = abi.EDGE_CLASSES[edge_class] if isinstance(edge_class, str) else int(edge_class)
        n = self._edge_counts[cls]
        chi, w = np.zeros(n), np.zeros(n)
        _check(load().esl_edge_chi2(self._h, C.c_int32(cls), chi.ctypes.data_as(_dp), w.ctypes.data_as(_dp), C.c_int64(n)),
               "esl_edge_chi2")
        return chi, w

    def lm_download(self, which, count):
        out = np.zeros(int(count))
        _check(load().esl_lm_download(self._h, C.c_int32(which), out.ctypes.data_as(_dp), C.c_int64(int(count))),
               "esl_lm_download")
        return out

    def snapshot_states(self):
        _check(load().esl_states_snapshot(self._h), "esl_states_snapshot")

    def restore_states(self):
        _check(load().esl_states_restore(self._h), "esl_states_restore")

    def profile_enable(self, level=2):
        lv = 2 if level is True else int(level)
        _check(load().esl_profile_enable(self._h, C.c_int(lv)), "esl_profile_enable")

    def profile_get(self):
        cnt = (C.c_int64 * 10)()
        ms = (C.c_double * 10)()
        _check(load().esl_profile_get(self._h, cnt, ms), "esl_profile_get")
        names = ["linearize", "lm_trial", "schur_build", "cholesky_solve", "reduce", "k5", "shard_allreduce", "rank_k_update", "sparse_block_products",
                 "dense_factorisation"]
        return {n: dict(count=int(cnt[i]), total_ms=float(ms[i])) for i, n in enumerate(names) if cnt[i]}

    def init_quadric(self, poses_Twc, bboxes, K, rows=480, cols=640, faithful=1):
        poses = np.ascontiguousarray(poses_Twc, dtype=np.float64).reshape(-1, 7)
        boxes = np.ascontiguousarray(bboxes, dtype=np.float64).reshape(-1, 4)
        Kd = np.ascontiguousarray(K, dtype=np.float64)
        e = np.zeros(10); Q = np.zeros(16); ok = C.c_int32(0)
        _check(load().esl_init_quadric(self._h, poses.ctypes.data_as(_dp), boxes.ctypes.data_as(_dp), C.c_int32(len(poses)),
                                       Kd.ctypes.data_as(_dp), C.c_int32(rows), C.c_int32(cols), C.c_int32(faithful),
                                       e.ctypes.data_as(_dp), Q.ctypes.data_as(_dp), C.byref(ok)), "esl_init_quadric")
        return e, Q.reshape(4, 4), bool(ok.value)

    def init_from_qstar(self, qstar, faithful=1):
        Q = np.ascontiguousarray(qstar, dtype=np.float64).reshape(16)
        e = np.zeros(10); ok = C.c_int32(0)
        _check(load().esl_init_from_qstar(self._h, Q.ctypes.data_as(_dp), C.c_int32(faithful), e.ctypes.data_as(_dp), C.byref(ok)),
               "esl_init_from_qstar")
        return e, bool(ok.value)

    def init_plane_error(self, poses_Twc, bboxes, K, ellipsoid, rows=480, cols=640):
        poses = np.ascontiguousarray(poses_Twc, dtype=np.float64).reshape(-1, 7)
        boxes = np.ascontiguousarray(bboxes, dtype=np.float64).reshape(-1, 4)
        Kd = np.ascontiguousarray(K, dtype=np.float64); e = np.ascontiguousarray(ellipsoid, dtype=np.float64)
        err = C.c_double(0)
        _check(load().esl_init_plane_error(self._h, poses.ctypes.data_as(_dp), boxes.ctypes.data_as(_dp), C.c_int32(len(poses)),
                                           Kd.ctypes.data_as(_dp), C.c_int32(rows), C.c_int32(cols), e.ctypes.data_as(_dp),
                                           C.byref(err)), "esl_init_plane_error")
        return err.value

    def init_quadrics(self, cams, N, obs_cam, obs_obj, obs_boxes, K, rows=480, cols=640, faithful=1, min_observations=0):
        _ip = C.POINTER(C.c_int32)

        def ptr(a, t):
            return a.ctypes.data_as(t) if a.size else t()
        Kc = np.ascontiguousarray(K, dtype=np.float64).reshape(4)
        oc = np.ascontiguousarray(obs_cam, dtype=np.int32).reshape(-1)
        oo = np.ascontiguousarray(obs_obj, dtype=np.int32).reshape(-1)
        ob = np.ascontiguousarray(obs_boxes, dtype=np.float64).reshape(-1, 4)
        if not len(oc) == len(oo) == len(ob):
            raise ValueError(f"{len(oc)} frame indices, {len(oo)} object indices, {len(ob)} boxes")
        if cams is None:
            F, cp = (self._graph.n_cams if self._graph is not None else 0), _dp()
        else:
            cams = np.ascontiguousarray(cams, dtype=np.float64).reshape(-1, 7)
            F, cp = len(cams), ptr(cams, _dp)
        N = int(N)
        n = max(N, 1)
        e = np.zeros((n, 10)); Q = np.zeros((n, 16)); err = np.zeros(n); stats = np.zeros((n, 4), dtype=np.int32)
        t0 = time.perf_counter()
        rc = load().esl_init_quadrics(self._h, cp, C.c_int32(F), C.c_int32(N), ptr(oc, _ip), ptr(oo, _ip), ptr(ob, _dp),
                                      C.c_int64(len(oc)), Kc.ctypes.data_as(_dp), C.c_int32(rows), C.c_int32(cols), C.c_int32(faithful),
                                      C.c_int32(min_observations), e.ctypes.data_as(_dp), Q.ctypes.data_as(_dp), err.ctypes.data_as(_dp),
                                      stats.ctypes.data_as(_ip))
        self.last_call_s = time.perf_counter() - t0
        _check(rc, "esl_init_quadrics")
        return e[:max(N, 0)], Q[:max(N, 0)].reshape(-1, 4, 4), err[:max(N, 0)], stats[:max(N, 0)]

    def init_quadrics_robust(self, cams, N, obs_cam, obs_obj, obs_boxes, K, rows=480, cols=640, faithful=1, min_observations=0,
                             params=None, want_hyp=False):
        _ip = C.POINTER(C.c_int32)

        def ptr(a, t):
            return a.ctypes.data_as(t) if a.size else t()
        p = params if params is not None else abi.default_init_robust_params()
        Kc = np.ascontiguousarray(K, dtype=np.float64).reshape(4)
        oc = np.ascontiguousarray(obs_cam, dtype=np.int32).reshape(-1)
        oo = np.ascontiguousarray(obs_obj, dtype=np.int32).reshape(-1)
        ob = np.ascontiguousarray(obs_boxes, dtype=np.float64).reshape(-1, 4)
        if not len(oc) == len(oo) == len(ob):
            raise ValueError(f"{len(oc)} frame indices, {len(oo)} object indices, {len(ob)} boxes")
        if cams is None:
            F, cp = (self._graph.n_cams if self._graph is not None else 0), _dp()
        else:
            cams = np.ascontiguousarray(cams, dtype=np.float64).reshape(-1, 7)
            F, cp = len(cams), ptr(cams, _dp)
        N = int(N)
        n, no, H = max(N, 1), max(len(oc), 1), max(int(p.n_hypotheses), 1)
        e = np.zeros((n, 10)); Q = np.zeros((n, 16)); err = np.zeros(n); stats = np.zeros((n, 8), dtype=np.int32)
        inl = np.zeros(no, dtype=np.int32); res = np.full(no, np.nan)
        hyp = np.zeros((n, H, 4)) if want_hyp else None
        t0 = time.perf_counter()
        rc = load().esl_init_quadrics_robust(self._h, cp, C.c_int32(F), C.c_int32(N), ptr(oc, _ip), ptr(oo, _ip), ptr(ob, _dp),
                                             C.c_int64(len(oc)), Kc.ctypes.data_as(_dp), C.c_int32(rows), C.c_int32(cols),
                                             C.c_int32(faithful), C.c_int32(min_observations), C.byref(p), e.ctypes.data_as(_dp),
                                             Q.ctypes.data_as(_dp), err.ctypes.data_as(_dp), stats.ctypes.data_as(_ip),
                                             inl.ctypes.data_as(_ip), res.ctypes.data_as(_dp), hyp.ctypes.data_as(_dp) if want_hyp else _dp())
        self.last_call_s = time.perf_counter() - t0
        _check(rc, "esl_init_quadrics_robust")
        N = max(N, 0)
        return dict(ellipsoids=e[:N], qstar=Q[:N].reshape(-1, 4, 4), plane_error=err[:N], stats=stats[:N], inliers=inl[:len(oc)],
                    residuals=res[:len(oc)], hyp=hyp[:N] if want_hyp else None)

# ... 442 lines not shown
```

### profiles/cf_trial_timeline.py

```python
#!/usr/bin/env python
import sqlite3
import sys

db = sqlite3.connect(sys.argv[1])
rows = db.execute("select name, grid_x, start, end from kernels order by start").fetchall()
rows = [(n.split("(")[0].replace("void ", "").replace("esl::", ""), g, s / 1e3, e / 1e3) for n, g, s, e in rows]
onesided = any(r[0].startswith("k_cf_T_onesided") for r in rows)
anchor_name, last_name = ("k_cf_T_onesided", "k_chol_update_v") if onesided else ("k_cf_seg_syrk", "k_cf_T_gather")
anchor = [i for i, r in enumerate(rows) if r[0].startswith(anchor_name)]
if not anchor:
    sys.exit("no k_cf_seg_syrk or k_cf_T_onesided launch in this trace")
longest = max(rows[i][3] - rows[i][2] for i in anchor)
live = [i for i in anchor if rows[i][3] - rows[i][2] > 0.25 * longest]
pick = live[int(sys.argv[2]) if len(sys.argv) > 2 else len(live) // 2]
b = pick
while b > 0 and not rows[b][0].startswith("k_cf_gather_B"):
    b -= 1
e = pick
while e + 1 < len(rows) and not rows[e][0].startswith(last_name):
    e += 1
t0 = rows[b][2]
print("trial %d of %d with a full-size %s; us from the start of its k_cf_gather_B\n" % (live.index(pick), len(live), anchor_name))
print("| kernel | grid (threads) | start us | end us | us |")
print("|---|---|---|---|---|")
for n, g, s, t in rows[b:e + 1]:
    print("| `%s` | %d | %.1f | %.1f | %.1f |" % (n, g, s - t0, t - t0, t - s))
print("\nbuild, first start to last end: %.1f us\n" % (max(r[3] for r in rows[b:e + 1]) - t0))


def find(prefix, grid=None):
    return [r for r in rows[b:e + 1] if r[0].startswith(prefix) and (grid is None or r[1] == grid)]


def overlap(a, c):
    return max(0.0, min(a[3], c[3]) - max(a[2], c[2]))


if onesided:
    pairs = ((("k_cf_chain", 64), ("k_cf_forward<2>", None)), (("k_cf_forward<1>", None), ("k_cf_T_onesided", None)),
             (("k_cf_sep_rhs", None), ("k_cf_seg_back", None)), (("k_chol_update_v", None), ("k_cf_T_onesided", None)))
else:
    pairs = ((("k_cf_chain", 64), ("k_cf_forward<2>", None)), (("k_cf_forward<1>", None), ("k_cf_seg_syrk", None)),
             (("k_chol_update_v", None), ("k_cf_seg_syrk", None)), (("k_chol_update_v", None), ("k_cf_T_gather", None)))
for (pa, ga), (pc, gc) in pairs:
    for a in find(pa, ga):
        for c in find(pc, gc):
            print("%s [%.1f, %.1f] against %s [%.1f, %.1f]: %.1f us side by side" % (
                a[0], a[2] - t0, a[3] - t0, c[0], c[2] - t0, c[3] - t0, overlap(a, c)))
```

Baseline: 18.48.

## Merge repeated one-sided slot runs and split forward chunks into eighths

Consecutive edge entries that map to the same camera slot get their V blocks pre-summed into a merged buffer, so the one-sided T assembly processes far fewer pairs. The pair list also now picks the shorter side per segment pair, swapping A/B sources via a sign bit. The forward kernel's mode-2 chunk split becomes a template parameter, defaulting to eighths, which shrinks its shared-memory staging. The cost is an extra merge kernel, an Vm buffer and more host planning.

```diff
diff --git a/include/esl.h b/include/esl.h
--- a/include/esl.h
+++ b/include/esl.h
@@ -176,6 +176,8 @@
 int esl_lm_solver_used(esl_ctx* ctx, int32_t* solver_out);
 #define ESL_SOLVER_STATS 10
 int esl_lm_solver_stats(esl_ctx* ctx, double stats[ESL_SOLVER_STATS]);
+#define ESL_OS_COUNTS 6
+int esl_lm_os_counts(esl_ctx* ctx, double counts[ESL_OS_COUNTS]);
 
 int esl_lm_download(esl_ctx* ctx, int32_t which, double* dst, int64_t count);
 
diff --git a/object-oriented-slam_amd/abi.py b/object-oriented-slam_amd/abi.py
--- a/object-oriented-slam_amd/abi.py
+++ b/object-oriented-slam_amd/abi.py
@@ -3,6 +3,7 @@
 import numpy as np
 
 ESL_MAX_TRACE = 32
+ESL_OS_COUNTS = 6
 
 c_double_p = C.POINTER(C.c_double)
 c_int32_p = C.POINTER(C.c_int32)
diff --git a/object-oriented-slam_amd/csrc/esl_capi.hip b/object-oriented-slam_amd/csrc/esl_capi.hip
--- a/object-oriented-slam_amd/csrc/esl_capi.hip
+++ b/object-oriented-slam_amd/csrc/esl_capi.hip
@@ -124,6 +124,8 @@
   c->device = device_id;
   { const char* ov = std::getenv("ESL_CF_OVERLAP"); c->sw_cf_overlap = (ov && ov[0] >= '0' && ov[0] <= '4') ? ov[0] - '0' : 4; }
   { const char* ok = std::getenv("ESL_CF_OS_KERNEL"); c->sw_cf_os_kernel = (ok && ok[0] == '0') ? 0 : 1; }
+  { const char* ol = std::getenv("ESL_CF_OS_LIST"); c->sw_cf_os_list = (ol && ol[0] == '0') ? 0 : 1; }
+  { const char* fp = std::getenv("ESL_CF_FWD_PARTS"); const int v = fp ? std::atoi(fp) : 0; if (v == 2 || v == 4 || v == 8) c->sw_cf_fwd_parts = v; }
   { const char* sd = std::getenv("ESL_CF_STRIDE"); const int v = sd ? std::atoi(sd) : 0; c->sw_cf_stride = (v == 16 || v == 32 || v == 48) ? v : 0; }
   auto init = [&]() -> int {
     ESL_HIP_TRY(hipStreamCreateWithFlags(&c->stream, hipStreamNonBlocking));
diff --git a/object-oriented-slam_amd/csrc/esl_cf.hpp b/object-oriented-slam_amd/csrc/esl_cf.hpp
--- a/object-oriented-slam_amd/csrc/esl_cf.hpp
+++ b/object-oriented-slam_amd/csrc/esl_cf.hpp
@@ -221,7 +221,7 @@
   const int* fwork; const int* seg_start; const int* seg_obj; const long long* xoff; const int* xld;
   const int* rank; const int* unrank;
 };
-template <int MODE>
+template <int MODE, int PARTS = 2>
 static __global__ __launch_bounds__(64) void k_cf_forward(int nf_all, int n_o, int n_chunks, const int* __restrict__ oe_cst ,
                                                           const int* __restrict__ oe_slot, const double* __restrict__ V,
                                                           const double* __restrict__ vy, const double* __restrict__ Mm,
@@ -230,7 +230,8 @@
   constexpr bool SEP = MODE == 1;
   __shared__ double sM[kCfFwdCh * 36];
   __shared__ double sZ[kCfFwdCh * 36];
-  constexpr int CH = MODE == 2 ? kCfFwdCh / 2 : kCfFwdCh;
+  static_assert(PARTS == 2 || (MODE == 2 && (PARTS == 4 || PARTS == 8)), "halves, quarters or eighths of a chunk");
+  constexpr int CH = MODE == 2 ? kCfFwdCh / PARTS : kCfFwdCh;
   __shared__ double sv[CH * 6 * 64];
   __shared__ double svy[kCfFwdCh * 6];
   const int lane = threadIdx.x;
@@ -940,7 +941,8 @@
                                                            const int* __restrict__ cmap, const int* __restrict__ seg_start,
                                                            const int* __restrict__ oe_cst, const int* __restrict__ oe_slot,
                                                            const int* __restrict__ unrank, const long long* __restrict__ bstart,
-                                                           int* __restrict__ bcnt, int2* __restrict__ pairs, int offsets) {
+                                                           int* __restrict__ bcnt, int2* __restrict__ pairs, int offsets,
+                                                           const int* __restrict__ run, const int* __restrict__ heads) {
   const int lane = threadIdx.x & 63, wave = __builtin_amdgcn_readfirstlane(threadIdx.x >> 6);
   const int t1 = blockIdx.x;
   const int o1 = (t1 == N || !unrank) ? t1 : unrank[t1];
@@ -953,7 +955,6 @@
     if (t2 > t1 || t2 >= N) continue;
     const int o2 = unrank ? unrank[t2] : t2;
     const long b = rhs ? (long)N * (N + 1) / 2 + t2 : (long)t1 * (t1 + 1) / 2 + t2;
-    const int* cst = oe_cst + (size_t)(rhs ? o2 : o1) * (n_chunks + 1);
     const long long w0 = FILL ? bstart[b] : 0;
     int cnt = 0;
     for (int wd = 0; wd < nw; ++wd) {
@@ -962,21 +963,28 @@
       const int pl = wd * 64 + lane;
       const bool mine = (mk >> lane) & 1ull;
       const int che = seg_chunks * (pl + 1) < n_chunks ? seg_chunks * (pl + 1) : n_chunks;
+      const int q2 = mine ? seg_start[pl] + (cmap[(size_t)pl * N1 + o2] & 0xFFFFFF) : 0;
+      const int q1 = (mine && !rhs) ? seg_start[pl] + (cmap[(size_t)pl * N1 + o1] & 0xFFFFFF) : 0;
+      const bool swl = mine && !rhs && heads && heads[q2] < heads[q1];
+      const int* cst = oe_cst + (size_t)((rhs || swl) ? o2 : o1) * (n_chunks + 1);
       const int kal = mine ? cst[seg_chunks * pl] : 0, kbl = mine ? cst[che] : 0;
-      const int yrl = (mine && !rhs) ? (seg_start[pl] + (cmap[(size_t)pl * N1 + o2] & 0xFFFFFF)) * (stride - 1) : 0;
+      const int yrl = (swl ? q1 : q2) * (stride - 1);
       while (mk) {
         const int bit = __builtin_ctzll(mk);
         mk &= mk - 1;
         const int p = wd * 64 + bit;
         const int ka = __builtin_amdgcn_readlane(kal, bit), kb = __builtin_amdgcn_readlane(kbl, bit), yr = __builtin_amdgcn_readlane(yrl, bit);
+        const int sw = __builtin_amdgcn_readlane((int)swl, bit) ? (int)0x80000000u : 0;
         for (int k0 = ka; k0 < kb; k0 += 64) {
           const int ent = k0 + lane;
           const int pos = ent < kb ? oe_slot[ent] - p * stride : stride - 1;
-          const bool valid = pos != stride - 1;
+          const bool valid = pos != stride - 1 && (!run || run[ent] != 0);
           const unsigned long long vb = __ballot(valid);
           if (FILL && valid) {
             const int at = cnt + __builtin_popcountll(vb & ((1ull << lane) - 1ull));
-            pairs[w0 + at] = rhs ? make_int2((p * stride + pos) * m6, ent * m54) : make_int2(ent * m54, (yr + pos) * m54);
+            pairs[w0 + at] = rhs  ? make_int2((p * stride + pos) * m6, ent * m54)
+                             : sw ? make_int2(((yr + pos) * m54) | sw, ent * m54)
+                                  : make_int2(ent * m54, (yr + pos) * m54);
           }
           cnt += __builtin_popcountll(vb);
         }
@@ -984,6 +992,23 @@
     }
     if (!FILL && lane == 0) bcnt[b] = cnt;
   }
+}
+
+static __global__ __launch_bounds__(256) void k_cf_v_merge(int n_list, const int* __restrict__ run, const double* __restrict__ V, double* __restrict__ Vm) {
+  const long t = (long)blockIdx.x * 256 + threadIdx.x;
+  if (t >= (long)n_list * 9) return;
+  const long k = t / 9;
+  const int n = run[k];
+  if (n == 0) return;
+  double s[6];
+#pragma unroll
+  for (int a = 0; a < 6; ++a) s[a] = V[t * 6 + a];
+  for (int j = 1; j < n; ++j) {
+#pragma unroll
+    for (int a = 0; a < 6; ++a) s[a] += V[(t + 9L * j) * 6 + a];
+  }
+#pragma unroll
+  for (int a = 0; a < 6; ++a) Vm[t * 6 + a] = s[a];
 }
 
 constexpr int kCfOsBatch = 12;
@@ -1050,8 +1075,10 @@
           const int a = kidx - 6 * (hi ? e1 : e0);
           const bool ok = (hi ? e1 : e0) < m && kidx < 6 * m;
           const bool oka = ok && alane, okb = ok && blane;
-          const size_t ia = oka ? (size_t)(hi ? x1 : x0) * astep + aoff + a : 0, ib = okb ? (size_t)(hi ? y1 : y0) * 54 + r * 6 + a : 0;
-          const double va = Asrc[ia], vb = Bsrc[ib];
+          const int xs = hi ? x1 : x0;
+          const bool swp = xs < 0;
+          const size_t ia = oka ? (size_t)(xs & 0x7FFFFFFF) * astep + aoff + a : 0, ib = okb ? (size_t)(hi ? y1 : y0) * 54 + r * 6 + a : 0;
+          const double va = (swp ? Y : Asrc)[ia], vb = (swp ? V : Bsrc)[ib];
           av[j] = oka ? va : 0.0; bv[j] = okb ? vb : 0.0;
         }
 #pragma unroll
@@ -1145,8 +1172,10 @@
 #pragma unroll
     for (int e = 0; e < E; ++e)
       if (full || e < m) {
-        const unsigned x = (unsigned)__builtin_amdgcn_readlane(px, e0 + e), y = (unsigned)__builtin_amdgcn_readlane(py, e0 + e);
-        unsigned long long pa = (unsigned long long)(Asrc + x), pb = (unsigned long long)(Bsrc + y);
+        const int xs = __builtin_amdgcn_readlane(px, e0 + e);
+        const bool swp = xs < 0;
+        const unsigned x = (unsigned)xs & 0x7FFFFFFFu, y = (unsigned)__builtin_amdgcn_readlane(py, e0 + e);
+        unsigned long long pa = (unsigned long long)((swp ? Y : Asrc) + x), pb = (unsigned long long)((swp ? V : Bsrc) + y);
         unsigned oa = la8, ob = lb8;
 #if defined(__HIP_DEVICE_COMPILE__)
         asm("" : "+s"(pa)); asm("" : "+s"(pb)); asm("" : "+v"(oa)); asm("" : "+v"(ob));
diff --git a/object-oriented-slam_amd/csrc/esl_cf_plan.hpp b/object-oriented-slam_amd/csrc/esl_cf_plan.hpp
--- a/object-oriented-slam_amd/csrc/esl_cf_plan.hpp
+++ b/object-oriented-slam_amd/csrc/esl_cf_plan.hpp
@@ -4,6 +4,7 @@
 #include <cmath>
 #include <cstddef>
 #include <cstdint>
+#include <utility>
 #include <vector>
 
 namespace esl {
@@ -41,6 +42,7 @@
   int nd_min = 48;
   int stride = 0;
   int os_kernel = 1;
+  int os_list = 1;
 };
 
 struct CfSegTables {
@@ -64,6 +66,10 @@
   size_t os_npairs = 0;
   bool os_offsets = false;
   double os_flops = 0;
+  bool os_list = false;
+  std::vector<int> os_run, os_heads;
+  size_t osm_npairs = 0, osm_row_npairs = 0, os_list_npairs = 0;
+  double osm_flops = 0;
   bool tperm = false;
   std::vector<int> rank, unrank, kfirst;
   double upd_flops = 0;
@@ -157,6 +163,40 @@
     n.prod += (double)inc3[q][2] * (double)(q - q0 + 1);
   }
   return n;
+}
+
+inline void cf_os_sides(CfPlan& pl, const std::vector<int>& start) {
+  const int S = pl.S;
+  const size_t n_inc = pl.p.size();
+  pl.os_run.assign(pl.os.size(), 0); pl.os_heads.assign(n_inc, 0);
+  std::vector<int> cur(start.begin(), start.end() - 1);
+  for (size_t q = 0; q < n_inc; ++q) {
+    const int o = pl.o[q], p = pl.p[q], end = start[(size_t)o + 1];
+    int k = cur[(size_t)o];
+    while (k < end && pl.os[(size_t)k] / S < p) ++k;
+    for (int head = -1; k < end && pl.os[(size_t)k] / S == p; ++k) {
+      const int sl = pl.os[(size_t)k];
+      if (sl % S == S - 1) continue;
+      if (head < 0 || pl.os[(size_t)head] != sl) { head = k; ++pl.os_heads[q]; }
+      ++pl.os_run[(size_t)head];
+    }
+    cur[(size_t)o] = k;
+  }
+  double both = 0, row = 0, brow = 0;
+  std::vector<int> v;
+  std::vector<std::pair<int, int>> byrank;
+  for (int p = 0; p < pl.nseg; ++p) {
+    const int q0 = pl.seg_start[(size_t)p], n = pl.seg_start[(size_t)p + 1] - q0;
+    v.assign(pl.os_heads.begin() + q0, pl.os_heads.begin() + q0 + n);
+    std::sort(v.begin(), v.end());
+    for (int i = 0; i < n; ++i) { both += (double)v[(size_t)i] * (double)(n - i); brow += v[(size_t)i]; }
+    byrank.clear();
+    for (int i = 0; i < n; ++i) { const int o = pl.o[(size_t)(q0 + i)]; byrank.push_back({pl.rank.empty() ? o : pl.rank[(size_t)o], pl.os_heads[(size_t)(q0 + i)]}); }
+    std::sort(byrank.begin(), byrank.end());
+    for (int i = 0; i < n; ++i) row += (double)byrank[(size_t)i].second * (double)(i + 1);
+  }
+  pl.osm_npairs = (size_t)(both + brow); pl.osm_row_npairs = (size_t)(row + brow);
+  pl.osm_flops = 2.0 * 6.0 * (81.0 * both + 9.0 * brow);
 }
 
 inline bool cf_plan_build(int N, int nf, size_t EU, const std::vector<int>& start, const int* cu_start, const int* cu_obj, const int* cu_id, bool chain_ok,
@@ -229,6 +269,9 @@
     pl.os_npairs = (size_t)(n.prod + n.rhs_entries);
     pl.y_len = y_recs * 54 + std::max<size_t>(nfz, 1) * 6;
     pl.os_offsets = sw.os_kernel != 0 && 54 * std::max(EU, y_recs) <= (size_t)INT32_MAX;
+    cf_os_sides(pl, start);
+    pl.os_list = sw.os_list != 0;
+    pl.os_list_npairs = pl.os_list ? pl.osm_npairs : pl.os_npairs;
   }
   return true;
 }
diff --git a/object-oriented-slam_amd/csrc/esl_ctx.hpp b/object-oriented-slam_amd/csrc/esl_ctx.hpp
--- a/object-oriented-slam_amd/csrc/esl_ctx.hpp
+++ b/object-oriented-slam_amd/csrc/esl_ctx.hpp
@@ -248,6 +248,8 @@
   double *cf_Xc = nullptr, *cf_Xs = nullptr, *cf_P = nullptr, *cf_Prhs = nullptr, *cf_Y = nullptr, *cf_Yr = nullptr;
   long long* cf_os_start = nullptr;
   int *cf_os_cnt = nullptr, *cf_os_pairs = nullptr;
+  int *cf_os_run = nullptr, *cf_os_heads = nullptr;
+  double* cf_Vm = nullptr;
   int *cf_rank = nullptr, *cf_unrank = nullptr, *cf_kfirst = nullptr;
   double* cf_xo_t = nullptr;
   int lm_solver_used = 0;
@@ -278,5 +280,7 @@
   bool sw_chol_overlap = true;
   int sw_cf_overlap = 4;
   int sw_cf_os_kernel = 1;
+  int sw_cf_os_list = 1;
+  int sw_cf_fwd_parts = 8;
   int sw_cf_stride = 0;
 };
diff --git a/object-oriented-slam_amd/csrc/esl_slam.hip b/object-oriented-slam_amd/csrc/esl_slam.hip
--- a/object-oriented-slam_amd/csrc/esl_slam.hip
+++ b/object-oriented-slam_amd/csrc/esl_slam.hip
@@ -262,7 +262,7 @@
   c->cf_T = c->cf_Linv_ws = c->cf_part = nullptr;
   c->cf_Zt = c->cf_Hs = c->cf_Bs = c->cf_LfacS = c->cf_GS = c->cf_LiS = c->cf_MS = c->cf_NS = c->cf_R = nullptr;
   c->cf_Xc = c->cf_Xs = c->cf_P = c->cf_Prhs = c->cf_Xt = c->cf_Y = c->cf_Yr = nullptr;
-  c->cf_os_start = nullptr; c->cf_os_cnt = c->cf_os_pairs = nullptr;
+  c->cf_os_start = nullptr; c->cf_os_cnt = c->cf_os_pairs = c->cf_os_run = c->cf_os_heads = nullptr; c->cf_Vm = nullptr;
   c->cf_rank = c->cf_unrank = c->cf_kfirst = nullptr; c->cf_xo_t = nullptr;
   c->cf_plan = CfPlan{};
   c->cf_ready = false;
@@ -287,7 +287,7 @@
   { const char* e = std::getenv("ESL_CF_TPERM"); sw.tperm_off = e && e[0] == '0'; }
   sw.no_nd = std::getenv("ESL_CF_NO_ND") != nullptr;
   static const int nd_min = [] { const char* e = std::getenv("ESL_CF_ND_MIN"); return e ? std::atoi(e) : 48; }();
-  sw.nd_min = nd_min; sw.stride = c->sw_cf_stride; sw.os_kernel = c->sw_cf_os_kernel;
+  sw.nd_min = nd_min; sw.stride = c->sw_cf_stride; sw.os_kernel = c->sw_cf_os_kernel; sw.os_list = c->sw_cf_os_list;
   size_t free_b = 0, total_b = 0;
   if (nfi >= kCfSparseMinCams) ESL_HIP_TRY(hipMemGetInfo(&free_b, &total_b));
   CfPlan& pl = c->cf_plan;
@@ -295,7 +295,7 @@
     set_error("camera-first elimination: the (ellipsoid, camera chunk) range table of this graph exceeds 1 GB");
     return ESL_ERR_ALLOC;
   }
-  const bool sp = pl.sparse, os3 = sp && pl.form == 3;
+  const bool sp = pl.sparse, os3 = sp && pl.form == 3, osm = os3 && pl.os_list;
   const int nch = pl.n_chunks, nseg = pl.nseg, nw = pl.nw, N1 = N + 1;
   const size_t n_inc = pl.p.size();
   const size_t y_recs = std::max<size_t>(n_inc, 1) * (size_t)(pl.S - 1), nb = (size_t)N * (N + 1) / 2 + N;
@@ -312,6 +312,7 @@
     i_inc = st.up(&d_inc, 4 * n_inc); ship(&c->cf_seg_start, pl.seg_start); ship(&c->cf_xld, pl.xld);
     ship(&c->cf_xoff, pl.xoff); ship(&c->cf_boff, pl.boff); ship(&c->cf_roff, pl.roff); ship(&d_fw_off, pl.fw_off); ship(&d_tw_off, pl.tw_off);
   }
+  if (osm) { ship(&c->cf_os_run, pl.os_run); ship(&c->cf_os_heads, pl.os_heads); }
   st.work(&c->cf_oe_cst, (size_t)std::max(N, 1) * (nch + 1));
   if (sp) {
     st.work(&c->cf_cmap, (size_t)nseg * N1); st.work(&c->cf_mask, (size_t)N1 * nw); st.work(&c->cf_seg_obj, n_inc); st.work(&c->cf_seg_first, n_inc);
@@ -333,7 +334,8 @@
     if (pl.form == 1) { st.work(&c->cf_P, pl.p_blocks * 81); st.work(&c->cf_Prhs, pl.prhs_len); }
     if (pl.form == 3) {
       st.work(&c->cf_Y, y_recs * 54); st.work(&c->cf_Yr, std::max<size_t>(nf, 1) * 6);
-      st.work(&c->cf_os_start, nb + 1); st.work(&c->cf_os_cnt, nb); st.work(&c->cf_os_pairs, 2 * std::max<size_t>(pl.os_npairs, 1));
+      st.work(&c->cf_os_start, nb + 1); st.work(&c->cf_os_cnt, nb); st.work(&c->cf_os_pairs, 2 * std::max<size_t>(pl.os_list_npairs, 1));
+      if (osm) st.work(&c->cf_Vm, EU * 54);
     }
   } else {
     st.work(&c->cf_Xt, (size_t)pl.ldx * (size_t)pl.kpad);
@@ -364,20 +366,21 @@
     const dim3 grid((unsigned)(N + 1), (unsigned)((N + kCfTPer - 1) / kCfTPer));
     ESL_HIP_TRY(hipMemsetAsync(c->cf_os_cnt, 0, nb * sizeof(int), c->stream));
     hipLaunchKernelGGL(k_cf_os_list<false>, grid, dim3(256), 0, c->stream, N, nw, nch, pl.S / kCfFwdCh, c->cf_mask, c->cf_cmap, c->cf_seg_start, c->cf_oe_cst, c->cf_oe_slot,
-                       (const int*)c->cf_unrank, (const long long*)nullptr, c->cf_os_cnt, (int2*)nullptr, 0);
+                       (const int*)c->cf_unrank, (const long long*)nullptr, c->cf_os_cnt, (int2*)nullptr, 0, (const int*)c->cf_os_run, (const int*)c->cf_os_heads);
     std::vector<int> h_cnt(nb);
     std::vector<long long> h_start(nb + 1);
     ESL_HIP_TRY(hipMemcpyAsync(h_cnt.data(), c->cf_os_cnt, nb * sizeof(int), hipMemcpyDeviceToHost, c->stream));
     ESL_HIP_TRY(hipStreamSynchronize(c->stream));
     h_start[0] = 0;
     for (size_t b = 0; b < nb; ++b) h_start[b + 1] = h_start[b] + h_cnt[b];
-    if ((size_t)h_start[nb] != pl.os_npairs) {
+    if ((size_t)h_start[nb] != pl.os_list_npairs) {
       set_error("camera-first elimination: the one-sided assembly's pair list does not have the length the host counted");
       return ESL_ERR_STATE;
     }
     ESL_HIP_TRY(hipMemcpyAsync(c->cf_os_start, h_start.data(), (nb + 1) * sizeof(long long), hipMemcpyHostToDevice, c->stream));
     hipLaunchKernelGGL(k_cf_os_list<true>, grid, dim3(256), 0, c->stream, N, nw, nch, pl.S / kCfFwdCh, c->cf_mask, c->cf_cmap, c->cf_seg_start, c->cf_oe_cst, c->cf_oe_slot,
-                       (const int*)c->cf_unrank, (const long long*)c->cf_os_start, c->cf_os_cnt, (int2*)c->cf_os_pairs, pl.os_offsets ? 1 : 0);
+                       (const int*)c->cf_unrank, (const long long*)c->cf_os_start, c->cf_os_cnt, (int2*)c->cf_os_pairs, pl.os_offsets ? 1 : 0,
+                       (const int*)c->cf_os_run, (const int*)c->cf_os_heads);
     ESL_HIP_TRY(hipStreamSynchronize(c->stream));
   }
   if (pl.nd) ESL_HIP_TRY(hipMemsetAsync(c->cf_Zt, 0, nf * 36 * sizeof(double), c->stream));
@@ -457,8 +460,13 @@
     sep_chain(beside ? rt.cf_side : main);
     if (beside) ESL_HIP_TRY(hipEventRecord(rt.cf_ev_s, rt.cf_side));
     edge_scale(beside ? 1 : 0, main);
-    hipLaunchKernelGGL(k_cf_forward<2>, dim3((unsigned)pl.n_fwork), dim3(64), 0, main, nf, n_o, pl.n_chunks, c->cf_oe_cst, c->cf_oe_slot, c->cf_V,
-                       c->cf_vy, c->cf_M, c->cf_Xc, ldx, st, st - 1, (const double*)c->cf_Zt, c->cf_R, st, segs());
+    auto forward = [&](auto parts) {
+      hipLaunchKernelGGL((k_cf_forward<2, decltype(parts)::value>), dim3((unsigned)pl.n_fwork), dim3(64), 0, main, nf, n_o, pl.n_chunks, c->cf_oe_cst, c->cf_oe_slot,
+                         c->cf_V, c->cf_vy, c->cf_M, c->cf_Xc, ldx, st, st - 1, (const double*)c->cf_Zt, c->cf_R, st, segs());
+    };
+    if (c->sw_cf_fwd_parts == 8) forward(std::integral_constant<int, 8>{});
+    else if (c->sw_cf_fwd_parts == 4) forward(std::integral_constant<int, 4>{});
+    else forward(std::integral_constant<int, 2>{});
     return ESL_OK;
   }
   void sep_rhs(hipStream_t s, bool sp = true) const {
@@ -592,9 +600,11 @@
       if (st == 3 * kCfFwdCh) seg_back(std::integral_constant<int, 3>{});
       else if (st == 2 * kCfFwdCh) seg_back(std::integral_constant<int, 2>{});
       else seg_back(std::integral_constant<int, 1>{});
+      if (pl.os_list && pl.n_list > 0)
+        hipLaunchKernelGGL(k_cf_v_merge, dim3((unsigned)(((long)pl.n_list * 9 + 255) / 256)), dim3(256), 0, main, pl.n_list, (const int*)c->cf_os_run, c->cf_V, c->cf_Vm);
       const dim3 grid((unsigned)(N + 1), (unsigned)((N + kCfTPer - 1) / kCfTPer));
       hipLaunchKernelGGL(pl.os_offsets ? k_cf_T_onesided_lds : k_cf_T_onesided, grid, dim3(256), 0, main, N, (const int2*)c->cf_os_pairs,
-                         (const long long*)c->cf_os_start, (const int*)c->cf_os_cnt, c->cf_V, c->cf_Y, c->cf_Yr, c->Hoo, c->bo, lambda, c->cf_T, ldt, 0, N,
+                         (const long long*)c->cf_os_start, (const int*)c->cf_os_cnt, pl.os_list ? c->cf_Vm : c->cf_V, c->cf_Y, c->cf_Yr, c->Hoo, c->bo, lambda, c->cf_T, ldt, 0, N,
                          (const int*)c->cf_unrank, 0);
     }
     ESL_HIP_TRY(hipGetLastError());
@@ -1202,6 +1212,16 @@
   st[9] = pl.tperm ? 1.0 : 0.0;
   return ESL_OK;
 }
+extern "C" int esl_lm_os_counts(esl_ctx* c, double* n) {
+  if (!c || !n) return ESL_ERR_INVALID;
+  for (int k = 0; k < ESL_OS_COUNTS; ++k) n[k] = 0;
+  if (c->lm_solver_used != ESL_SOLVER_REDUCED_ELLIPSOID || !c->cf_ready) return ESL_OK;
+  const esl::CfPlan& pl = c->cf_plan;
+  if (!pl.sparse || pl.form != 3) return ESL_OK;
+  n[0] = (double)pl.os_npairs; n[1] = (double)pl.osm_row_npairs; n[2] = (double)pl.osm_npairs;
+  n[3] = (double)pl.os_list_npairs; n[4] = pl.os_list ? pl.osm_flops : pl.os_flops; n[5] = 8.0 * (double)pl.os_list_npairs;
+  return ESL_OK;
+}
 extern "C" int esl_lm_pcg_stats(esl_ctx* c, double* st) {
   if (!c || !st) return ESL_ERR_INVALID;
   for (int k = 0; k < ESL_PCG_STATS; ++k) st[k] = 0;
diff --git a/object-oriented-slam_amd/lib.py b/object-oriented-slam_amd/lib.py
--- a/object-oriented-slam_amd/lib.py
+++ b/object-oriented-slam_amd/lib.py
@@ -15,7 +15,7 @@
     "esl_abi_version", "esl_last_error", "esl_device_count", "esl_ctx_create", "esl_ctx_destroy",
     "esl_ctx_synchronize", "esl_ctx_trim", "esl_lm_params_default", "esl_optimize", "esl_optimize_fixed", "esl_graph_upload", "esl_graph_upload_fixed", "esl_graph_obj_fixed", "esl_graph_append", "esl_graph_sizes", "esl_states_upload",
     "esl_states_download", "esl_optimize_resident", "esl_states_snapshot", "esl_states_restore", "esl_profile_enable", "esl_profile_get", "esl_lm_begin", "esl_lm_linearize", "esl_lm_reduced_system", "esl_lm_reduced_residual",
-    "esl_lm_try_step", "esl_lm_commit", "esl_lm_solver_used", "esl_lm_solver_stats", "esl_lm_download", "esl_lm_set_robust", "esl_edge_chi2", "esl_pcg_params_default", "esl_lm_set_pcg", "esl_lm_pcg_stats", "esl_comm_unique_id", "esl_comm_init", "esl_comm_init_host", "esl_comm_set_replicated", "esl_comm_destroy", "esl_partition_objects", "esl_fit_params_default", "esl_fit_frame", "esl_fit_frame_debug", "esl_fit_frame_ex", "esl_selftest_cholesky", "esl_debug_chol_plan", "esl_debug_update_v_applies", "esl_debug_cf_stride_choose",
+    "esl_lm_try_step", "esl_lm_commit", "esl_lm_solver_used", "esl_lm_solver_stats", "esl_lm_os_counts", "esl_lm_download", "esl_lm_set_robust", "esl_edge_chi2", "esl_pcg_params_default", "esl_lm_set_pcg", "esl_lm_pcg_stats", "esl_comm_unique_id", "esl_comm_init", "esl_comm_init_host", "esl_comm_set_replicated", "esl_comm_destroy", "esl_partition_objects", "esl_fit_params_default", "esl_fit_frame", "esl_fit_frame_debug", "esl_fit_frame_ex", "esl_selftest_cholesky", "esl_debug_chol_plan", "esl_debug_update_v_applies", "esl_debug_cf_stride_choose",
     "esl_init_quadric", "esl_init_from_qstar", "esl_init_plane_error", "esl_init_quadrics", "esl_plane_params_default", "esl_extract_ground_plane", "esl_extract_planes",
     "esl_reloc_params_default", "esl_reloc_set_map", "esl_relocalize",
     "esl_assoc_params_default", "esl_predict_boxes", "esl_associate_boxes",
@@ -225,6 +225,12 @@
                  "dense_update_flops_executed", "t_ordered_by_first_camera"]
         return {n: float(st[i]) for i, n in enumerate(names)}
 
+    def lm_os_counts(self):
+        n = (C.c_double * abi.ESL_OS_COUNTS)()
+        _check(load().esl_lm_os_counts(self._h, n), "esl_lm_os_counts")
+        names = ["row_side_pairs", "merged_pairs", "merged_shorter_side_pairs", "list_pairs", "list_flops", "list_bytes"]
+        return {k: float(n[i]) for i, k in enumerate(names)}
+
     def lm_reduced_system(self, lam):
         ptr, n, lda = C.c_void_p(), C.c_int64(0), C.c_int64(0)
         _check(load().esl_lm_reduced_system(self._h, C.c_double(lam), C.byref(ptr), C.byref(n), C.byref(lda)),
diff --git a/profiles/cf_trial_timeline.py b/profiles/cf_trial_timeline.py
--- a/profiles/cf_trial_timeline.py
+++ b/profiles/cf_trial_timeline.py
@@ -37,10 +37,10 @@
 
 
 if onesided:
-    pairs = ((("k_cf_chain", 64), ("k_cf_forward<2>", None)), (("k_cf_forward<1>", None), ("k_cf_T_onesided", None)),
+    pairs = ((("k_cf_chain", 64), ("k_cf_forward<2", None)), (("k_cf_forward<1", None), ("k_cf_T_onesided", None)),
              (("k_cf_sep_rhs", None), ("k_cf_seg_back", None)), (("k_chol_update_v", None), ("k_cf_T_onesided", None)))
 else:
-    pairs = ((("k_cf_chain", 64), ("k_cf_forward<2>", None)), (("k_cf_forward<1>", None), ("k_cf_seg_syrk", None)),
+    pairs = ((("k_cf_chain", 64), ("k_cf_forward<2", None)), (("k_cf_forward<1", None), ("k_cf_seg_syrk", None)),
              (("k_chol_update_v", None), ("k_cf_seg_syrk", None)), (("k_chol_update_v", None), ("k_cf_T_gather", None)))
 for (pa, ga), (pc, gc) in pairs:
     for a in find(pa, ga):
```

New measurement: 19.23 (median of 6 runs). 1.04x the previous value.
